# gaspardol/MonteCarloPredictiveCoding

Measured on AMD Instinct MI355X. Metric: Langevin inference steps/sec (whole node), MNIST MCPC 784-256-256-30, batch 6000, higher is better.
Workload: dtype f32

## Files before the change

### montecarlopredictivecoding_amd/csrc/mcpc_api.hip

```cpp
#include <hip/hip_runtime.h>
#include <dlfcn.h>
#include <rccl/rccl.h>

#include <algorithm>
#include <cmath>
#include <cstdio>
#include <cstring>
#include <string>
#include <vector>

#include "mcpc_build.h"
#include "mcpc_kernels.h"
#include "mcpc_moments.h"
#include "mcpc_plan.h"

using namespace mcpc;

#define HIP_TRY(expr)                                                                            \
    do {                                                                                         \
        hipError_t _e = (expr);                                                                  \
        if (_e != hipSuccess) return fail(MCPC_EHIP, "%s failed: %s (%s:%d)", #expr, hipGetErrorString(_e), __FILE__, __LINE__); \
    } while (0)

static inline int grid_for(size_t n, int block = 256) { return (int)std::min<size_t>((n + block - 1) / block, 4096); }

struct mcpc_engine : EnginePlan {
    mcpc_net_desc d{};
    ncclComm_t comm = nullptr;
    int comm_ranks = 0;
    float* x[kMaxLatent]{};
    float* m[kMaxLatent]{};
    float* v[kMaxLatent]{};
    float* e0sum = nullptr;
    float* mu1 = nullptr;
    float* ypad = nullptr;
    float* ytile = nullptr;
    uint32_t* ybits = nullptr;
    int* y_binary = nullptr;
    int ywords = 0;
    bool target_bound = false;
    const float* inputs = nullptr;
    hipStream_t aux = nullptr;
    hipEvent_t ev_steps[kMaxRingParts] = {}, ev_flush[kMaxRingParts] = {};
    hipStream_t spacer = nullptr;
    hipStream_t aux3 = nullptr;
    hipEvent_t ev_fork = nullptr, ev_join = nullptr;
    bool flush_pending[kMaxRingParts] = {};
    float* spill_a[kMaxLatent]{};
    float* spill_e[kMaxLatent]{};
    float* spill_eo = nullptr;
    float* slab = nullptr;
    size_t slab_floats = 0;
    double* epart = nullptr;
    size_t epart_rows = 0;
    float* adam_coef = nullptr;
    size_t adam_cap = 0;
    float* adam_host[2] = {nullptr, nullptr};
    size_t adam_host_cap[2] = {0, 0};
    hipEvent_t adam_ev[2] = {nullptr, nullptr};
    int adam_next = 0;
    struct Retired { void* p; hipEvent_t ev; };
    std::vector<Retired> retired;
    bool spill_ready = false;
    int* err = nullptr;
    int* wexp = nullptr;
    unsigned* spillmax = nullptr;
    float* lw_fx[kMaxLatent]{};
    float* lw_err[kMaxLatent]{};
    float* lw_err_o = nullptr;
    LwJob* lw_jobs = nullptr;
    unsigned long long* clk = nullptr;
    float* dummy = nullptr;
    int* rr_tab = nullptr;
    std::string last_step;
    std::string last_flush[kMaxLatent + 1];
    bool profiling = false;
    std::vector<std::pair<hipEvent_t, hipEvent_t>> events;
    size_t events_used = 0;
    double prof_steps = 0;
#ifdef MCPC_STAMPS
    unsigned long long* dbg = nullptr;
#endif
};

namespace {

struct Rccl {
    void* so = nullptr;
    decltype(&ncclGetUniqueId) GetUniqueId = nullptr;
    decltype(&ncclCommInitRank) CommInitRank = nullptr;
    decltype(&ncclAllReduce) AllReduce = nullptr;
    decltype(&ncclCommDestroy) CommDestroy = nullptr;
    decltype(&ncclGetErrorString) GetErrorString = nullptr;
};
Rccl g_rccl;

int rccl_load() {
    if (g_rccl.so) return MCPC_OK;
    void* so = dlopen("librccl.so.1", RTLD_NOW | RTLD_LOCAL);
    if (!so) so = dlopen("librccl.so", RTLD_NOW | RTLD_LOCAL);
    if (!so) return fail(MCPC_EHIP, "librccl.so.1 could not be loaded: %s", dlerror());
    Rccl r;
    r.GetUniqueId = (decltype(r.GetUniqueId))dlsym(so, "ncclGetUniqueId");
    r.CommInitRank = (decltype(r.CommInitRank))dlsym(so, "ncclCommInitRank");
    r.AllReduce = (decltype(r.AllReduce))dlsym(so, "ncclAllReduce");
    r.CommDestroy = (decltype(r.CommDestroy))dlsym(so, "ncclCommDestroy");
    r.GetErrorString = (decltype(r.GetErrorString))dlsym(so, "ncclGetErrorString");
    if (!r.GetUniqueId || !r.CommInitRank || !r.AllReduce || !r.CommDestroy || !r.GetErrorString) {
        dlclose(so);
        return fail(MCPC_EHIP, "librccl.so.1 lacks an entry point this library needs");
    }
    r.so = so;
    g_rccl = r;
    return MCPC_OK;
}

int free_all(mcpc_engine* e) {
    if (e->comm && g_rccl.CommDestroy) { (void)g_rccl.CommDestroy(e->comm); e->comm = nullptr; e->comm_ranks = 0; }
    auto F = [](auto*& p) { if (p) { (void)hipFree((void*)p); p = nullptr; } };
    for (int l = 0; l < kMaxLatent; ++l) { F(e->x[l]); F(e->m[l]); F(e->v[l]); F(e->spill_a[l]); F(e->spill_e[l]); }
    F(e->e0sum); F(e->mu1); F(e->ypad); F(e->ytile); F(e->ybits); F(e->y_binary); F(e->spill_eo); F(e->slab); F(e->epart); F(e->adam_coef); F(e->main.dev); F(e->err); F(e->wexp); F(e->spillmax); F(e->clk); F(e->dummy); F(e->u.plan.dev);
    for (int l = 0; l < kMaxLatent; ++l) { F(e->lw_fx[l]); F(e->lw_err[l]); }
    F(e->lw_err_o); F(e->lw_jobs);
    for (auto& ln : e->lin) { F(ln.Wf); F(ln.Wb); F(ln.bias_pad); F(ln.G); F(ln.Gb); }
    for (auto& ev : e->events) { (void)hipEventDestroy(ev.first); (void)hipEventDestroy(ev.second); }
    for (int h = 0; h < kMaxRingParts; ++h) { if (e->ev_steps[h]) (void)hipEventDestroy(e->ev_steps[h]); if (e->ev_flush[h]) (void)hipEventDestroy(e->ev_flush[h]); e->ev_steps[h] = e->ev_flush[h] = nullptr; }
    if (e->aux) { (void)hipStreamDestroy(e->aux); e->aux = nullptr; }
    if (e->aux3) { (void)hipStreamDestroy(e->aux3); e->aux3 = nullptr; }
    if (e->spacer) { (void)hipStreamDestroy(e->spacer); e->spacer = nullptr; }
    if (e->ev_fork) { (void)hipEventDestroy(e->ev_fork); e->ev_fork = nullptr; }
    if (e->ev_join) { (void)hipEventDestroy(e->ev_join); e->ev_join = nullptr; }
    F(e->rr_tab);
    for (auto& q : e->retired) { (void)hipFree(q.p); if (q.ev) (void)hipEventDestroy(q.ev); }
    e->retired.clear();
    for (int i = 0; i < 2; ++i) {
        if (e->adam_host[i]) { (void)hipHostFree(e->adam_host[i]); e->adam_host[i] = nullptr; }
        if (e->adam_ev[i]) { (void)hipEventDestroy(e->adam_ev[i]); e->adam_ev[i] = nullptr; }
    }
    e->events.clear();
    return 0;
}

template <typename T>
int dmalloc(T*& p, size_t count) {
    void* q = nullptr;
    hipError_t err = hipMalloc(&q, std::max<size_t>(count, 1) * sizeof(T));
    if (err != hipSuccess) return fail(MCPC_ENOMEM, "hipMalloc of %zu bytes failed: %s", count * sizeof(T), hipGetErrorString(err));
#ifdef MCPC_POISON_ALLOC
    if (hipMemset(q, 0xFF, std::max<size_t>(count, 1) * sizeof(T)) != hipSuccess) return fail(MCPC_EHIP, "hipMemset (poison) failed");
#endif
    p = (T*)q;
    return 0;
}

void retire(mcpc_engine* e, void* p, hipStream_t stream) {
    hipEvent_t ev = nullptr;
    if (hipEventCreateWithFlags(&ev, hipEventDisableTiming) != hipSuccess || hipEventRecord(ev, stream) != hipSuccess) {
        if (ev) (void)hipEventDestroy(ev);
        ev = nullptr;
    }
    e->retired.push_back({p, ev});
}
void free_completed_retired(mcpc_engine* e) {
    size_t keep = 0;
    for (size_t i = 0; i < e->retired.size(); ++i) {
        auto& q = e->retired[i];
        if (q.ev && hipEventQuery(q.ev) == hipSuccess) { (void)hipFree(q.p); (void)hipEventDestroy(q.ev); }
        else e->retired[keep++] = q;
    }
    e->retired.resize(keep);
    (void)hipGetLastError();
}
#ifdef MCPC_STAMPS
void print_u_table(const StepPlan& u) {
    static const char* tn[6] = {"FWD", "HEADF", "HEADB", "BWD", "ENERGY", "NOP"};
    for (int w = 0; w < kUWaves; ++w) {
        fprintf(stderr, "[u-table] wave %d:", w);
        for (int i = 0; i < u.n_phases; ++i) {
            const KPhase& k = u.table[(size_t)w * u.n_phases + i];
            fprintf(stderr, " %s%s(l%d t%d+%d kb%d)", (k.flags & PHF_SYNC) ? "|" : "", tn[k.type], k.layer, k.tile0, k.ntiles, (k.flags & PHF_WS_GEMM) ? k.nkb : 0);
        }
        fprintf(stderr, "\n");
    }
}
#endif

template <typename T>
int upload(T*& dev, const std::vector<T>& host, const char* what) {
    if (const int rc = dmalloc(dev, host.size())) return rc;
    if (hipMemcpy(dev, host.data(), host.size() * sizeof(T), hipMemcpyHostToDevice) != hipSuccess) return fail(MCPC_EHIP, "hipMemcpy of %s failed", what);
    return 0;
}

int upload_table(mcpc_engine* e, StepPlan& p) {
    for (KPhase& k : p.table)
        if (k.a_lin >= 1) k.A = (k.type == PH_FWD || k.type == PH_HEADF) ? e->lin[k.a_lin].Wf : e->lin[k.a_lin].Wb;
    return upload(p.dev, p.table, "the phase table");
}

hipError_t allow_lds(const void* fn, int bytes) { return hipFuncSetAttribute(fn, hipFuncAttributeMaxDynamicSharedMemorySize, bytes); }
int upload_rounds(mcpc_engine* e) {
    if (const int rc = upload(e->rr_tab, e->rr_host, "the round-schedule tables")) return rc;
    if (allow_lds((const void*)mcpc_steps_ws2_kernel<1, true>, e->main.lds_bytes) != hipSuccess) return fail(MCPC_EHIP, "hipFuncSetAttribute failed for the round schedule");
    return 0;
}

void set_window(const mcpc_engine* e, const mcpc_run_desc* r, KParams& P, int t0, int n) {
    P.t0 = t0; P.n_steps = n;
    const size_t s0 = (size_t)(t0 - r->t_begin);
    P.adam_coef = r->xopt_kind == MCPC_XOPT_ADAM ? e->adam_coef + 2 * s0 : nullptr;
    if (r->noise_mode == MCPC_NOISE_EXTERNAL)
        for (int l = 0; l < e->L; ++l) P.layer[l].ext_noise = r->ext_noise[l] + s0 * e->d.batch * e->d.sizes[l];
}

int launch_lw_steps(mcpc_engine* e, const mcpc_run_desc* r, const KParams& P, int t0, int n, hipStream_t stream) {
    LwParams Q{};
    Q.P = P;
    for (int l = 0; l < e->L; ++l) { Q.fx[l] = e->lw_fx[l]; Q.err[l] = e->lw_err[l]; }
    Q.err_o = e->lw_err_o;
    const dim3 gf(e->Bpad / kLwChains, e->lw_nf), gb(e->Bpad / kLwChains, e->lw_nb);
    for (int t = t0; t < t0 + n; ++t) {
        Q.t = t;
        Q.slot = (t >= P.acc_begin && t < P.acc_end) ? t - P.spill_t0 : -1;
        Q.rec_idx = -1;
        if (P.rec_count > 0 && t >= P.rec_begin) {
            const int k = (t - P.rec_begin) / P.rec_stride;
            if (k < P.rec_count && P.rec_begin + k * P.rec_stride == t) Q.rec_idx = k;
        }
        Q.do_energy = (P.energy_mode == MCPC_ENERGY_ALL || (P.energy_mode == MCPC_ENERGY_LAST && t == P.T - 1)) ? 1 : 0;
        Q.erow = P.energy_mode == MCPC_ENERGY_ALL ? t : 0;
        set_window(e, r, Q.P, t, 1);
        Q.jobs = e->lw_jobs;
        hipLaunchKernelGGL(mcpc_lw_fwd_kernel, gf, dim3(kLwThreads), 0, stream, Q);
        Q.jobs = e->lw_jobs + e->lw_nf;
        hipLaunchKernelGGL(mcpc_lw_bwd_kernel, gb, dim3(kLwThreads), 0, stream, Q);
    }
    HIP_TRY(hipGetLastError());
    return 0;
}

}

extern "C" {

int mcpc_abi_version(void) { return MCPC_ABI_VERSION; }

const char* mcpc_build_info(void) {
    static const bool exp = MCPC_TIMING_BUILD != 0 || std::strstr(MCPC_BUILD_FLAGS, "MCPC_EXP") != nullptr ||
                            std::strstr(MCPC_BUILD_FLAGS, "MCPC_HEB_EXP") != nullptr;
    static char buf[1024];
    static const int n = std::snprintf(buf, sizeof buf, "libmcpc abi=%d arch=gfx950 csrc=%s commit=%s exp=%d stamps=%d flags=[%s]",
                                       MCPC_ABI_VERSION, MCPC_BUILD_CSRC_SHA, MCPC_BUILD_COMMIT, exp ? 1 : 0, MCPC_STAMPS_BUILD, MCPC_BUILD_FLAGS);
    (void)n;
    return buf;
}
const char* mcpc_last_error(void) { return g_err.c_str(); }

int mcpc_create(const mcpc_net_desc* d, mcpc_engine** out) {
    if (!d || !out) return fail(MCPC_EINVAL, "null argument");
    *out = nullptr;
    if (const int rc = check_net_desc(d)) return rc;
    int ndev = 0;
    HIP_TRY(hipGetDeviceCount(&ndev));
    if (d->device < 0 || d->device >= ndev) return fail(MCPC_EINVAL, "device %d not present (%d devices)", d->device, ndev);
    HIP_TRY(hipSetDevice(d->device));
    int n_cu = 256;
    if (hipDeviceGetAttribute(&n_cu, hipDeviceAttributeMultiprocessorCount, d->device) != hipSuccess || n_cu <= 0) n_cu = 256;
    size_t free_b = 0, total_b = 0;
    if (d->spill_budget_bytes <= 0 && hipMemGetInfo(&free_b, &total_b) != hipSuccess) total_b = 0;

    mcpc_engine* e = new mcpc_engine();
    e->d = *d;
    e->d.tuning = nullptr;
    int rc = parse_tuning(d->tuning, e->knobs);
    if (!rc) rc = plan_engine(*d, n_cu, total_b, *e);
    if (rc) { delete e; return rc; }
    auto bail = [&](int code) { free_all(e); delete e; return code; };
    auto zeroed = [&](auto*& p, size_t count) -> int {
        if (const int rc2 = dmalloc(p, count)) return rc2;
        return hipMemset(p, 0, count * sizeof(*p)) == hipSuccess ? 0 : fail(MCPC_EHIP, "hipMemset failed");
    };
    for (int l = 0; l < e->L; ++l) {
        const size_t n = (size_t)e->Bpad * e->npad[l];
        if ((rc = zeroed(e->x[l], n)) || (rc = dmalloc(e->m[l], n)) || (rc = dmalloc(e->v[l], n))) return bail(rc);
    }
    if ((rc = zeroed(e->e0sum, (size_t)e->Bpad * e->npad[0])) || (rc = dmalloc(e->mu1, (size_t)e->Bpad * e->npad[0]))) return bail(rc);
    if (e->has_head) {
        if ((rc = zeroed(e->ypad, (size_t)e->Bpad * e->out_pad)) || (rc = dmalloc(e->ytile, (size_t)e->Bpad * e->out_pad))) return bail(rc);
        e->ywords = (e->out_pad + 31) / 32;
        if ((rc = dmalloc(e->ybits, (size_t)e->Bpad * e->ywords)) || (rc = zeroed(e->y_binary, 3))) return bail(rc);
    }
    const int nlin = e->L + (e->has_head ? 1 : 0);
    for (int j = 0; j < nlin; ++j) {
        Lin& ln = e->lin[j];
        if ((rc = zeroed(ln.G, (size_t)ln.out_pad * ln.g_ld)) || (rc = zeroed(ln.Gb, (size_t)ln.out_pad))) return bail(rc);
        if (j >= 1) {
            const size_t pkf = (size_t)(ln.out_pad / 16) * kblocks(ln.in_pad) * kFragBlock * 4;
            const size_t pkb = (size_t)(ln.in_pad / 16) * kblocks(ln.out_pad) * kFragBlock * 4;
            if ((rc = dmalloc(ln.Wf, pkf)) || (rc = dmalloc(ln.Wb, pkb)) || (rc = dmalloc(ln.bias_pad, (size_t)ln.out_pad))) return bail(rc);
        }
    }
    if (e->lw) {
        for (int l = 0; l < e->L; ++l) {
            const size_t n = (size_t)e->Bpad * e->npad[l];
            if ((rc = dmalloc(e->lw_fx[l], n))) return bail(rc);
            if (l >= 1 && (rc = dmalloc(e->lw_err[l], n))) return bail(rc);
        }
        if (e->has_head && (rc = dmalloc(e->lw_err_o, (size_t)e->Bpad * e->out_pad))) return bail(rc);
        if ((rc = upload(e->lw_jobs, e->lw_table, "the layer-wise job table"))) return bail(rc);
    } else if ((rc = upload_table(e, e->main))) return bail(rc);
    if (e->u.on && (rc = upload_table(e, e->u.plan))) return bail(rc);
#ifdef MCPC_STAMPS
    if (e->u.on) print_u_table(e->u.plan);
#endif
    if ((rc = zeroed(e->err, 1)) || (rc = zeroed(e->spillmax, (size_t)kMaxRingParts * kSpillTensors)) || (rc = zeroed(e->wexp, kMaxLatent + 1)) ||
        (rc = zeroed(e->clk, 2)) || (rc = zeroed(e->dummy, 1024)))
        return bail(rc);
    const void* kfn = e->ws == 2 ? (const void*)mcpc_steps_ws2_kernel<1> : (const void*)mcpc_steps_kernel<1, 4>;
    const hipError_t herr = e->lw ? hipSuccess : allow_lds(kfn, e->main.lds_bytes);
    if (herr != hipSuccess) return bail(fail(MCPC_EHIP, "hipFuncSetAttribute(%d bytes LDS) failed: %s", e->main.lds_bytes, hipGetErrorString(herr)));
    if (e->rr && (rc = upload_rounds(e))) return bail(rc);
    if (e->u.on && (allow_lds((const void*)mcpc_steps_u_kernel<false>, e->u.plan.lds_bytes) != hipSuccess ||
                    allow_lds((const void*)mcpc_steps_u_kernel<true>, e->u.plan.lds_bytes) != hipSuccess))
        return bail(fail(MCPC_EHIP, "hipFuncSetAttribute failed for the unified-wave kernel (%d bytes LDS)", e->u.plan.lds_bytes));
    *out = e;
    return MCPC_OK;
}

int mcpc_destroy(mcpc_engine* e) {
    if (!e) return MCPC_OK;
    (void)hipSetDevice(e->d.device);
    (void)hipDeviceSynchronize();
    free_all(e);
    delete e;
    return MCPC_OK;
}

int mcpc_bind_params(mcpc_engine* e, int j, const float* W, const float* bias) {
    if (!e) return fail(MCPC_EINVAL, "null engine");
    const int nlin = e->L + (e->has_head ? 1 : 0);
    if (j < 0 || j >= nlin) return fail(MCPC_EINVAL, "Linear index %d out of range 0..%d", j, nlin - 1);
    if (!W) return fail(MCPC_EINVAL, "null weight pointer for Linear %d", j);
    e->lin[j].W = W;
    e->lin[j].bias = bias;
    e->lin[j].bound = true;
    return MCPC_OK;
}

int mcpc_params_changed(mcpc_engine* e, void* stream_) {
    if (!e) return fail(MCPC_EINVAL, "null engine");
    hipStream_t stream = (hipStream_t)stream_;
    HIP_TRY(hipSetDevice(e->d.device));
    const int nlin = e->L + (e->has_head ? 1 : 0);
    for (int j = 0; j < nlin; ++j)
        if (!e->lin[j].bound) return fail(MCPC_ESTATE, "Linear %d has no bound parameters", j);
    for (int j = 1; j < nlin; ++j) {
        Lin& ln = e->lin[j];
        const size_t total = (size_t)ln.out_pad * ln.in_pad;
        const int grid = std::max(grid_for(total), (ln.out_pad + 255) / 256);
        hipLaunchKernelGGL(mcpc_wexp_kernel, dim3(1), dim3(1024), 0, stream, ln.W, (size_t)ln.n_out * ln.n_in, e->wexp + j);
        hipLaunchKernelGGL(mcpc_pack_kernel, dim3(grid), dim3(256), 0, stream, ln.W, ln.bias, ln.Wf, ln.Wb, ln.bias_pad,
                           ln.n_out, ln.n_in, ln.out_pad / 16, ln.in_pad / 16, (const int*)(e->wexp + j));
    }
    HIP_TRY(hipGetLastError());
    return MCPC_OK;
}

int mcpc_bind_inputs(mcpc_engine* e, const float* inputs, void* ) {
    if (!e) return fail(MCPC_EINVAL, "null engine");
    e->inputs = inputs;
    return MCPC_OK;
}

int mcpc_bind_target(mcpc_engine* e, const float* target, void* stream_) {
    if (!e) return fail(MCPC_EINVAL, "null engine");
    if (!e->has_head) return fail(MCPC_EINVAL, "network has no read-out: no target to bind");
    if (!target) return fail(MCPC_EINVAL, "null target");
    HIP_TRY(hipSetDevice(e->d.device));
    const size_t total = (size_t)e->Bpad * e->out_pad;
    hipLaunchKernelGGL(mcpc_pad_kernel, dim3(grid_for(total)), dim3(256), 0, (hipStream_t)stream_, target, e->ypad,
                       e->d.batch, e->d.n_out, e->Bpad, e->out_pad);
    hipLaunchKernelGGL(mcpc_tile_major_kernel, dim3(grid_for(total / 4)), dim3(256), 0, (hipStream_t)stream_, e->ypad, e->ytile, e->Bpad, e->out_pad);
    HIP_TRY(hipMemsetAsync(e->y_binary, 0xff, sizeof(int), (hipStream_t)stream_));
    HIP_TRY(hipMemsetAsync(e->y_binary + 2, 0xff, sizeof(int), (hipStream_t)stream_));
    hipLaunchKernelGGL(mcpc_pack_target_bits_kernel, dim3(grid_for((size_t)e->Bpad * e->ywords)), dim3(256), 0, (hipStream_t)stream_,
                       e->ypad, e->ybits, e->y_binary, e->Bpad, e->out_pad, e->ywords);
    HIP_TRY(hipGetLastError());
    e->target_bound = true;
    return MCPC_OK;
}

int mcpc_load_state(mcpc_engine* e, const float* const* x, void* stream_) {
    if (!e || !x) return fail(MCPC_EINVAL, "null argument");
    HIP_TRY(hipSetDevice(e->d.device));
    for (int l = 0; l < e->L; ++l) {
        if (!x[l]) return fail(MCPC_EINVAL, "null state pointer for layer %d", l);
        const size_t total = (size_t)e->Bpad * e->npad[l];
        hipLaunchKernelGGL(mcpc_pad_kernel, dim3(grid_for(total)), dim3(256), 0, (hipStream_t)stream_, x[l], e->x[l],
                           e->d.batch, e->d.sizes[l], e->Bpad, e->npad[l]);
    }
    HIP_TRY(hipGetLastError());
    return MCPC_OK;
}

int mcpc_store_state(mcpc_engine* e, float* const* x, void* stream_) {
    if (!e || !x) return fail(MCPC_EINVAL, "null argument");
    HIP_TRY(hipSetDevice(e->d.device));
    for (int l = 0; l < e->L; ++l) {
        if (!x[l]) return fail(MCPC_EINVAL, "null state pointer for layer %d", l);
        const size_t total = (size_t)e->d.batch * e->d.sizes[l];
        hipLaunchKernelGGL(mcpc_unpad_kernel, dim3(grid_for(total)), dim3(256), 0, (hipStream_t)stream_, e->x[l], x[l],
                           e->d.batch, e->d.sizes[l], e->npad[l]);
    }
    HIP_TRY(hipGetLastError());
    return MCPC_OK;
}

int mcpc_store_adam_state(mcpc_engine* e, float* const* m, float* const* v, void* stream_) {
    if (!e || !m || !v) return fail(MCPC_EINVAL, "null argument");
    HIP_TRY(hipSetDevice(e->d.device));
    for (int l = 0; l < e->L; ++l) {
        if (!m[l] || !v[l]) return fail(MCPC_EINVAL, "null Adam state pointer for layer %d", l);
        const size_t total = (size_t)e->d.batch * e->d.sizes[l];
        hipLaunchKernelGGL(mcpc_unpad_adam_kernel, dim3(grid_for(total)), dim3(256), 0, (hipStream_t)stream_, e->m[l], m[l],
                           e->d.batch, e->d.sizes[l], e->npad[l]);
        hipLaunchKernelGGL(mcpc_unpad_adam_kernel, dim3(grid_for(total)), dim3(256), 0, (hipStream_t)stream_, e->v[l], v[l],
                           e->d.batch, e->d.sizes[l], e->npad[l]);
    }
    HIP_TRY(hipGetLastError());
    return MCPC_OK;
}

}

namespace {

struct HebPlan {
    bool tiled = false, swapped = false;
    int ra = 0;
    int te[2] = {0, 0}, n_mt[2] = {0, 0};
    int n_nt = 1;
    int wave_tiles = 0;
    int ksplit = 1, rps = 0;
    int ksplit_cap = 1;
};

HebPlan plan_hebbian(const mcpc_engine* e, int ne, int na, int rows) {
    HebPlan h;
    const int et = ne / 16, at = na / 16;
    const bool wide = heb_wide(et, at);
    const bool narrow_in = heb_narrow_in(et, at);
    h.tiled = wide || narrow_in;
    h.swapped = narrow_in;
    if (wide) {
        h.ra = at >= 16 ? 2 : 1;
        h.n_nt = at / (8 * h.ra);
        if (et <= 8) { h.te[0] = 8; h.n_mt[0] = 1; }
        else if (et <= 16) { h.te[0] = 16; h.n_mt[0] = 1; }
        else {
            const int b17 = et % 16, a16 = (et - 17 * b17) / 16;
            if (et - 17 * b17 >= 0) { h.te[0] = 17; h.n_mt[0] = b17; h.te[1] = 16; h.n_mt[1] = a16; }
            else { h.te[0] = 17; h.n_mt[0] = (et + 16) / 17; }
            if (h.n_mt[0] == 0) { h.te[0] = h.te[1]; h.n_mt[0] = h.n_mt[1]; h.te[1] = 0; h.n_mt[1] = 0; }
        }
    } else if (narrow_in) {
        h.ra = 2; h.n_nt = 1; h.te[0] = at; h.n_mt[0] = 1;
    }
    if (h.tiled) {
        int want = e->knobs.dw_ksplit > 0 ? e->knobs.dw_ksplit : std::max(1, rows / (48 * kHebKB));
        if (e->knobs.dw_ksplit <= 0) {
            const int cols = std::max(1, (h.n_mt[0] + h.n_mt[1]) * h.n_nt);
            want = std::max(want, std::min(rows / (8 * kHebKB), (256 + cols - 1) / cols));
        }
        want = std::min(want, std::max(1, rows / kHebKB));
        h.ksplit_cap = want;
        h.rps = ((rows + want - 1) / want + kHebKB - 1) / kHebKB * kHebKB;
        h.ksplit = (rows + h.rps - 1) / h.rps;
    } else {
        h.wave_tiles = ((ne + 63) / 64) * ((na + 63) / 64);
        int ksplit = std::max(1, std::min(4096 / h.wave_tiles, rows / 64));
        h.ksplit_cap = ksplit;
        h.rps = ((rows + ksplit - 1) / ksplit + 15) / 16 * 16;
        h.ksplit = (rows + h.rps - 1) / h.rps;
    }
    return h;
}

template <int TE, int RA, bool SW = false>
int launch_heb(const HebArgs& a, hipStream_t stream) {
    constexpr int lds_bytes = 2 * kHebKB * (heb_lds_stride(16 * TE) + heb_lds_stride(16 * 8 * RA)) * (int)sizeof(float);
    static bool attr_set[16] = {false};
    int dev = 0;
    (void)hipGetDevice(&dev);
    if (dev >= 0 && dev < 16 && !attr_set[dev]) {
        if (hipFuncSetAttribute((const void*)mcpc_heb_kernel<TE, RA, SW>, hipFuncAttributeMaxDynamicSharedMemorySize, lds_bytes) != hipSuccess)
            return fail(MCPC_EHIP, "hipFuncSetAttribute failed for the Hebbian kernel");
        attr_set[dev] = true;
    }
    hipLaunchKernelGGL((mcpc_heb_kernel<TE, RA, SW>), dim3(a.n_mt * a.n_nt * a.ksplit), dim3(kHebThreads), lds_bytes, stream, a);
    return 0;
}

template <int TE, int RA, bool SW = false>
int launch_heb7(const HebArgs& a, hipStream_t stream) {
    constexpr int lds_bytes = 2 * 2 * 16 * TE * kHeb7LD * 2 + 16 * TE * (int)sizeof(float) + 8 * 2 * 272 * (int)sizeof(float);
    static bool attr_set[16] = {false};
    int dev = 0;
    (void)hipGetDevice(&dev);
    if (dev >= 0 && dev < 16 && !attr_set[dev]) {
        if (hipFuncSetAttribute((const void*)mcpc_heb7_kernel<TE, RA, SW>, hipFuncAttributeMaxDynamicSharedMemorySize, lds_bytes) != hipSuccess)
            return fail(MCPC_EHIP, "hipFuncSetAttribute failed for the Hebbian kernel");
        attr_set[dev] = true;
    }
    hipLaunchKernelGGL((mcpc_heb7_kernel<TE, RA, SW>), dim3(a.n_mt * a.n_nt * a.ksplit), dim3(kHebThreads), lds_bytes, stream, a);
    return 0;
}

int ensure_spill(mcpc_engine* e, hipStream_t stream) {
    if (e->spill_ready) return 0;
    int rc;
    if (e->half_slots < e->slots && !e->aux) {
        int lo = 0, hi = 0;
        (void)hipDeviceGetStreamPriorityRange(&lo, &hi);
        if (!e->spacer) (void)hipStreamCreateWithFlags(&e->spacer, hipStreamNonBlocking);
        if (hipStreamCreateWithPriority(&e->aux, hipStreamNonBlocking, lo) != hipSuccess) return fail(MCPC_EHIP, "hipStreamCreateWithPriority failed");
        if (e->knobs.flush_streams >= 2 &&
            (hipStreamCreateWithPriority(&e->aux3, hipStreamNonBlocking, lo) != hipSuccess ||
             hipEventCreateWithFlags(&e->ev_fork, hipEventDisableTiming) != hipSuccess ||
             hipEventCreateWithFlags(&e->ev_join, hipEventDisableTiming) != hipSuccess))
            return fail(MCPC_EHIP, "second flush stream could not be created");
        for (int h = 0; h < kMaxRingParts; ++h)
            if (hipEventCreateWithFlags(&e->ev_steps[h], hipEventDisableTiming) != hipSuccess ||
                hipEventCreateWithFlags(&e->ev_flush[h], hipEventDisableTiming) != hipSuccess)
                return fail(MCPC_EHIP, "hipEventCreate failed");
    }
    for (int l = 0; l < e->L; ++l) {
        const size_t n = (size_t)e->slots * e->Bpad * e->npad[l];
        if (!e->spill_a[l] && (rc = dmalloc(e->spill_a[l], n))) return rc;
        if (l >= 1 && !e->spill_e[l] && (rc = dmalloc(e->spill_e[l], n))) return rc;
    }
    if (e->has_head && !e->spill_eo && (rc = dmalloc(e->spill_eo, (size_t)e->slots * e->Bpad * e->out_pad))) return rc;
    if (e->nwg_live * e->ct < e->Bpad && e->ws == 2) {
        const size_t live = (size_t)e->nwg_live * 16, dead = (size_t)e->Bpad - live;
        auto zero_tail = [&](float* base, int npad) {
            return hipMemset2DAsync(base + live * npad, (size_t)e->Bpad * npad * sizeof(float), 0, dead * npad * sizeof(float), (size_t)e->slots, stream) == hipSuccess;
        };
        bool ok = true;
        for (int l = 0; l < e->L; ++l) { ok = ok && zero_tail(e->spill_a[l], e->npad[l]); if (l >= 1) ok = ok && zero_tail(e->spill_e[l], e->npad[l]); }
        if (e->has_head) ok = ok && zero_tail(e->spill_eo, e->out_pad);
        if (!ok) return fail(MCPC_EHIP, "hipMemset2D of the spill ring's padding rows failed");
    }
    const int nlin = e->L + (e->has_head ? 1 : 0);
    const int max_rows = e->half_slots * e->Bpad;
    size_t total = 0;
    for (int j = 1; j < nlin; ++j) {
        Lin& ln = e->lin[j];
        const HebPlan h = plan_hebbian(e, ln.out_pad, ln.in_pad, max_rows);
        ln.slab_off = total;
        ln.slab_floats = (size_t)h.ksplit_cap * ((size_t)ln.out_pad * ln.in_pad + ln.out_pad);
        total += ln.slab_floats;
    }
    if (!e->slab && (rc = dmalloc(e->slab, total))) return rc;
    e->slab_floats = total;
    e->spill_ready = true;
    return 0;
}

static inline int spill_id_a_host(int l) { return l; }
int flush_spill(mcpc_engine* e, int n_slots, int slot0, hipStream_t stream, int part) {
    const unsigned* const smax = e->spillmax + (size_t)part * kSpillTensors;
    const int rows = n_slots * e->Bpad;
    const int nlin = e->L + (e->has_head ? 1 : 0);
    ReduceJobs jobs{};
    unsigned max_blocks = 1;
    hipStream_t const main_stream = stream;
    const bool two = e->aux3 != nullptr && stream == e->aux;
    double load[2] = {0.0, 0.0};
    if (two) { HIP_TRY(hipEventRecord(e->ev_fork, main_stream)); HIP_TRY(hipStreamWaitEvent(e->aux3, e->ev_fork, 0)); }
    auto next_stream = [&](double cost) {
        const int k = (two && load[1] < load[0]) ? 1 : 0;
        load[k] += cost;
        return k ? e->aux3 : main_stream;
    };
    for (int j = 1; j < nlin; ++j) {
        Lin& ln = e->lin[j];
        const int ne = ln.out_pad, na = ln.in_pad;
        const float* E = (j < e->L ? e->spill_e[j] : e->spill_eo) + (size_t)slot0 * e->Bpad * ne;
        const float* A = e->spill_a[j - 1] + (size_t)slot0 * e->Bpad * na;
        const HebPlan h = plan_hebbian(e, ne, na, rows);
        std::string plan;
        auto name_launch = [&](const char* kern, int te, int ra, bool sw, int n_mt, int n_nt) {
            char buf[64];
            snprintf(buf, sizeof buf, "%s%s<%d,%d%s>x%d", plan.empty() ? "" : "+", kern, te, ra, sw ? ",T" : "", n_mt);
            plan += buf;
            if (n_nt > 1) plan += "*" + std::to_string(n_nt);
        };
        const char* const heb_name = e->knobs.heb_fp32 ? "heb" : "heb7";
        const int e_id = j < e->L ? kMaxLatent + j : kSpillIdEo;
        float* slab = e->slab + ln.slab_off;
        float* slab_b = slab + (size_t)h.ksplit * ne * na;
        if ((size_t)h.ksplit * ((size_t)ne * na + ne) > ln.slab_floats)
            return fail(MCPC_ESTATE, "internal: Hebbian slabs of Linear %d (%d splits) exceed their allocation", j, h.ksplit);
        if (h.swapped) {
            stream = next_stream((double)ne * na);
            HebArgs a{A, E, slab, slab_b, rows, na, ne, h.rps, 1, 1, h.ksplit, 0, smax + spill_id_a_host(j - 1), smax + e_id};
            name_launch(heb_name, h.te[0], 2, true, 1, 1);
            int rc = 0;
            if (!e->knobs.heb_fp32) {
                if (h.te[0] == 1) rc = launch_heb7<1, 2, true>(a, stream);
                else if (h.te[0] == 2) rc = launch_heb7<2, 2, true>(a, stream);
                else rc = launch_heb7<4, 2, true>(a, stream);
            } else
            if (h.te[0] == 1) rc = launch_heb<1, 2, true>(a, stream);
            else if (h.te[0] == 2) rc = launch_heb<2, 2, true>(a, stream);
            else rc = launch_heb<4, 2, true>(a, stream);
            if (rc) return rc;
        } else if (h.tiled) {
            int col = 0;
            for (int part = 0; part < 2; ++part) {
                if (h.n_mt[part] == 0) continue;
                HebArgs a{E, A, slab, slab_b, rows, ne, na, h.rps, h.n_mt[part], h.n_nt, h.ksplit, col, smax + e_id, smax + spill_id_a_host(j - 1)};
                stream = next_stream((double)h.n_mt[part] * h.te[part] * 16 * na);
                int rc = 0;
                const int te = h.te[part];
                const bool resplit = te == 17 && h.ra == 2 && !e->knobs.heb_fp32 && e->knobs.heb171;
                if (!resplit) name_launch(heb_name, te, h.ra, false, h.n_mt[part], h.n_nt);
                if (!e->knobs.heb_fp32) {
                    if (te == 17 && h.ra == 2 && !e->knobs.heb171) rc = launch_heb7<17, 2>(a, stream);
                    else if (te == 17 && h.ra == 2) {
                        HebArgs a1 = a;
                        a1.n_nt = 2 * a.n_nt;
                        name_launch(heb_name, 17, 1, false, a1.n_mt, a1.n_nt);
                        rc = launch_heb7<17, 1>(a1, stream);
                    }
                    else if (te == 16 && h.ra == 2) rc = launch_heb7<16, 2>(a, stream);
                    else if (te == 8 && h.ra == 2) rc = launch_heb7<8, 2>(a, stream);
                    else if (te == 17) rc = launch_heb7<17, 1>(a, stream);
                    else if (te == 16) rc = launch_heb7<16, 1>(a, stream);
                    else rc = launch_heb7<8, 1>(a, stream);
                } else
                if (te == 17 && h.ra == 2) rc = launch_heb<17, 2>(a, stream);
                else if (te == 16 && h.ra == 2) rc = launch_heb<16, 2>(a, stream);
                else if (te == 8 && h.ra == 2) rc = launch_heb<8, 2>(a, stream);
                else if (te == 17) rc = launch_heb<17, 1>(a, stream);
                else if (te == 16) rc = launch_heb<16, 1>(a, stream);
                else rc = launch_heb<8, 1>(a, stream);
                if (rc) return rc;
                col += h.n_mt[part] * te * 16;
            }
        } else {
            stream = next_stream((double)ne * na);
            hipLaunchKernelGGL(mcpc_dw_kernel, dim3((h.wave_tiles + 3) / 4, h.ksplit), dim3(256), 0, stream, E, A, slab, slab_b,
                               rows, ne, na, h.rps);
            plan = "dw tiles=" + std::to_string(h.wave_tiles);
        }
        e->last_flush[j] = plan + " ksplit=" + std::to_string(h.ksplit) + " rps=" + std::to_string(h.rps) + (ln.spill_tm ? " tm" : " rm");
        const float sign = j < e->L ? -1.0f : 1.0f;
        jobs.job[jobs.n_jobs++] = ReduceJob{slab, ln.G, ne * na, h.ksplit, sign, h.swapped ? ne : 0, h.swapped ? na : 0};
        jobs.job[jobs.n_jobs++] = ReduceJob{slab_b, ln.Gb, ne, h.ksplit, sign, 0, 0};
        max_blocks = std::max(max_blocks, (unsigned)std::min<size_t>(((size_t)ne * na + 255) / 256, 2048));
    }
    stream = main_stream;
    if (two) { HIP_TRY(hipEventRecord(e->ev_join, e->aux3)); HIP_TRY(hipStreamWaitEvent(main_stream, e->ev_join, 0)); }
    if (jobs.n_jobs > 0)
        hipLaunchKernelGGL(mcpc_reduce_jobs_kernel, dim3(max_blocks, jobs.n_jobs), dim3(256), 0, stream, jobs);
    HIP_TRY(hipGetLastError());
    return 0;
}

}

namespace {

int check_run(const mcpc_engine* e, const mcpc_run_desc* r) {
    const int nlin = e->L + (e->has_head ? 1 : 0);
    for (int j = 0; j < nlin; ++j)
        if (!e->lin[j].bound) return fail(MCPC_ESTATE, "Linear %d has no bound parameters (mcpc_bind_params + mcpc_params_changed first)", j);
    if (r->T < 1 || r->t_begin < 0 || r->n_steps < 1 || r->t_begin + r->n_steps > r->T)
        return fail(MCPC_EINVAL, "bad step range: T=%d t_begin=%d n_steps=%d", r->T, r->t_begin, r->n_steps);
    if (r->loss_kind < 0 || r->loss_kind > 2) return fail(MCPC_EINVAL, "loss_kind=%d", r->loss_kind);
    if (r->loss_kind != MCPC_LOSS_NONE) {
        if (!e->has_head) return fail(MCPC_EINVAL, "a loss needs a read-out Linear (n_out > 0)");
        if (!e->target_bound) return fail(MCPC_ESTATE, "loss requested but no target bound");
        if (r->loss_kind == MCPC_LOSS_GAUSSIAN && !(r->loss_var > 0.0)) return fail(MCPC_EINVAL, "loss_var must be positive");
        if (r->mask_start < 0 || r->mask_start >= e->d.n_out) return fail(MCPC_EINVAL, "mask_start=%d outside 0..%d", r->mask_start, e->d.n_out - 1);
    }
    if (r->xopt_kind != MCPC_XOPT_SGD && r->xopt_kind != MCPC_XOPT_ADAM) return fail(MCPC_EINVAL, "xopt_kind=%d", r->xopt_kind);
    if (!(r->lr > 0.0)) return fail(MCPC_EINVAL, "lr must be positive");
    if (r->noise_mode < 0 || r->noise_mode > 2) return fail(MCPC_EINVAL, "noise_mode=%d", r->noise_mode);
    if (r->noise_mode != MCPC_NOISE_NONE && r->xopt_kind != MCPC_XOPT_SGD)
        return fail(MCPC_EINVAL, "the fused Langevin kick is defined for SGD on x only (reference utils/model.py:35-44 steps the same optimizer)");
    if (r->noise_mode != MCPC_NOISE_NONE && !(r->noise_var >= 0.0)) return fail(MCPC_EINVAL, "noise_var must be >= 0");
    if (r->noise_mode == MCPC_NOISE_EXTERNAL)
        for (int l = 0; l < e->L; ++l)
            if (!r->ext_noise[l]) return fail(MCPC_EINVAL, "ext_noise[%d] is null", l);
    if (!r->update_x)
        for (int l = 0; l < e->L; ++l)
            if (!r->xgrad[l]) return fail(MCPC_EINVAL, "update_x=0 needs xgrad[%d]", l);
    if (r->energy_mode < 0 || r->energy_mode > 2) return fail(MCPC_EINVAL, "energy_mode=%d", r->energy_mode);
    if (r->energy_mode != MCPC_ENERGY_NONE && !r->energies_out) return fail(MCPC_EINVAL, "energies_out is null");
    if (r->rec_count < 0 || (r->rec_count > 0 && r->rec_stride < 1)) return fail(MCPC_EINVAL, "bad record schedule");
    return 0;
}

size_t energy_slots(const mcpc_engine* e) { return e->lw ? (size_t)e->nwg_live : e->ws == 2 ? (size_t)e->Bpad / 16 : (size_t)e->nwg; }

int prepare_run(mcpc_engine* e, const mcpc_run_desc* r, bool run_accumulates, hipStream_t stream) {
    if (r->xopt_kind == MCPC_XOPT_ADAM) {
        const size_t need = (size_t)r->n_steps * 2;
        if (need > e->adam_cap) {
            if (e->adam_coef) retire(e, e->adam_coef, stream);
            e->adam_coef = nullptr;
            size_t cap = 1024;
            while (cap < need) cap *= 2;
            int rc = dmalloc(e->adam_coef, cap);
            if (rc) return rc;
            e->adam_cap = cap;
        }
        const int hb = e->adam_next; e->adam_next ^= 1;
        if (!e->adam_ev[hb]) HIP_TRY(hipEventCreateWithFlags(&e->adam_ev[hb], hipEventDisableTiming));
        else HIP_TRY(hipEventSynchronize(e->adam_ev[hb]));
        if (need > e->adam_host_cap[hb]) {
            if (e->adam_host[hb]) HIP_TRY(hipHostFree(e->adam_host[hb]));
            e->adam_host[hb] = nullptr;
            void* q = nullptr;
            HIP_TRY(hipHostMalloc(&q, e->adam_cap * sizeof(float), hipHostMallocDefault));
            e->adam_host[hb] = (float*)q; e->adam_host_cap[hb] = e->adam_cap;
        }
        float* tab = e->adam_host[hb];
        for (int s = 0; s < r->n_steps; ++s) {
            const double step = (double)(r->adam_step0 + s + 1);
            const double bc1 = 1.0 - std::pow(r->beta1, step);
            const double bc2 = 1.0 - std::pow(r->beta2, step);
            tab[2 * s] = (float)(-(r->lr / bc1));
            tab[2 * s + 1] = (float)std::sqrt(bc2);
        }
        HIP_TRY(hipMemcpyAsync(e->adam_coef, tab, need * sizeof(float), hipMemcpyHostToDevice, stream));
        HIP_TRY(hipEventRecord(e->adam_ev[hb], stream));
        if (r->adam_step0 == 0)
            for (int l = 0; l < e->L; ++l) {
                HIP_TRY(hipMemsetAsync(e->m[l], 0, (size_t)e->Bpad * e->npad[l] * 4, stream));
                HIP_TRY(hipMemsetAsync(e->v[l], 0, (size_t)e->Bpad * e->npad[l] * 4, stream));
            }
    }
    const size_t erows = r->energy_mode == MCPC_ENERGY_ALL ? (size_t)r->T : 1, eslots = energy_slots(e);
    if (r->energy_mode != MCPC_ENERGY_NONE && erows > e->epart_rows) {
        if (e->epart) retire(e, e->epart, stream);
        e->epart = nullptr;
        const size_t cap = std::max(erows, e->epart_rows + e->epart_rows / 2);
        int rc = dmalloc(e->epart, cap * eslots * (kMaxLatent + 1));
        if (rc) return rc;
        HIP_TRY(hipMemsetAsync(e->epart, 0, cap * eslots * (kMaxLatent + 1) * sizeof(double), stream));
        e->epart_rows = cap;
    }
    {
        const Lin& l0 = e->lin[0];
        const size_t total = (size_t)e->Bpad * e->npad[0];
        hipLaunchKernelGGL(mcpc_mu1_kernel, dim3(grid_for(total)), dim3(256), 0, stream, e->inputs, l0.W, l0.bias, e->mu1,
                           e->d.batch, e->d.n_in, e->d.sizes[0], e->Bpad, e->npad[0]);
    }
    if (e->lw)
        for (int l = 0; l < e->L; ++l) {
            const size_t total4 = (size_t)e->Bpad * e->npad[l] / 4;
            hipLaunchKernelGGL(mcpc_lw_act_kernel, dim3(grid_for(total4)), dim3(256), 0, stream, (const float*)e->x[l], e->lw_fx[l], total4, e->d.acts[l]);
        }
    if (run_accumulates) { const int rc = ensure_spill(e, stream); if (rc) return rc; }
    if (r->acc_reset && run_accumulates) {
        const int nlin = e->L + (e->has_head ? 1 : 0);
        for (int j = 0; j < nlin; ++j) {
            HIP_TRY(hipMemsetAsync(e->lin[j].G, 0, (size_t)e->lin[j].out_pad * e->lin[j].g_ld * 4, stream));
            HIP_TRY(hipMemsetAsync(e->lin[j].Gb, 0, (size_t)e->lin[j].out_pad * 4, stream));
        }
        HIP_TRY(hipMemsetAsync(e->e0sum, 0, (size_t)e->Bpad * e->npad[0] * 4, stream));
    }
    return 0;
}

bool lean_ok(const mcpc_engine* e) {
    int widest = e->out_pad;
    for (int l = 0; l < e->L; ++l) widest = std::max(widest, e->npad[l]);
    return e->Bpad < (1 << 24) && (uint64_t)e->Bpad * (uint64_t)widest * 4u < (1ull << 32) && !e->knobs.no_lean;
}

bool use_unified(const mcpc_engine* e, const mcpc_run_desc* r) {
    return e->u.on && (e->u.prefer || (e->has_head && r->loss_kind == MCPC_LOSS_NONE)) && e->ws == 2 && r->update_x && lean_ok(e) &&
           ((r->xopt_kind == MCPC_XOPT_SGD && r->noise_mode != MCPC_NOISE_EXTERNAL) ||
            (r->xopt_kind == MCPC_XOPT_ADAM && r->noise_mode == MCPC_NOISE_NONE));
}

KParams run_params(const mcpc_engine* e, const mcpc_run_desc* r, const StepPlan& sp) {
    KParams P{};
    const int nlin = e->L + (e->has_head ? 1 : 0);
    for (int l = 0; l < e->L; ++l) {
        KLayer& K = P.layer[l];
        K.x = e->x[l]; K.m = e->m[l]; K.v = e->v[l];
        K.xgrad = r->update_x ? nullptr : r->xgrad[l];
        K.rec = r->rec_count > 0 ? r->rec_x[l] : nullptr;
        K.spill_e = l == 0 ? e->e0sum : e->spill_e[l];
        K.spill_a = e->spill_a[l];
        K.spill_e_tm = (l >= 1 && e->lin[l].spill_tm) ? 1 : 0;
        K.spill_a_tm = (l + 1 < nlin && e->lin[l + 1].spill_tm) ? 1 : 0;
        K.ext_noise = nullptr;
        if (l >= 1) {
            K.Wf = (const f32x4*)e->lin[l].Wf; K.Wb = (const f32x4*)e->lin[l].Wb; K.bias = e->lin[l].bias_pad;
        }
        K.n = e->d.sizes[l]; K.npad = e->npad[l]; K.ntiles = e->npad[l] / 16;
        K.act = e->d.acts[l]; K.ecoef = e->d.ecoef[l];
        K.lds_a = sp.lds_a[l]; K.lds_e = sp.lds_e[l]; K.ld = e->npad[l] + kLdPad;
        K.lds_x = sp.lds_x[l]; K.lds_bias = sp.lds_bias[l];
    }
    if (e->has_head) {
        KHead& H = P.head;
        const Lin& ln = e->lin[e->L];
        H.Wf = (const f32x4*)ln.Wf; H.Wb = (const f32x4*)ln.Wb; H.bias = ln.bias_pad;
        H.ybits = e->ybits; H.y_binary = e->knobs.no_ybits ? e->y_binary + 1 : e->y_binary; H.y_bounded = e->y_binary + 2; H.ywords = e->ywords;
        H.y = e->ypad; H.ytile = e->ytile; H.rec_out = r->rec_count > 0 ? r->rec_out : nullptr; H.spill_e = e->spill_eo;
        H.spill_tm = e->lin[e->L].spill_tm ? 1 : 0;
        H.n = e->d.n_out; H.npad = e->out_pad; H.ntiles = e->out_pad / 16;
        H.loss_kind = r->loss_kind;
        H.inv_var = r->loss_kind == MCPC_LOSS_GAUSSIAN ? (float)(1.0 / r->loss_var) : 1.0f;
        H.mask_start = r->loss_kind == MCPC_LOSS_NONE ? 0 : r->mask_start;
        H.lds_eo = sp.lds_eo; H.ld = sp.head_ld;
        H.lds_bias = sp.lds_hbias; H.lds_yw = sp.lds_yw;
    }
    P.mu1 = e->mu1; P.epart = e->epart; P.epart_slots = (int)energy_slots(e);
    P.phases = sp.dev; P.n_phases = sp.n_phases; P.wexp = e->wexp; P.spillmax = nullptr; P.lds_spillmax = sp.lds_spillmax; P.lds_rowexp = sp.lds_rowexp; P.g_first = sp.g_first;
    P.stagger_cycles = e->knobs.stagger;
    P.L = e->L; P.has_head = e->has_head; P.B = e->d.batch; P.Bpad = e->Bpad; P.T = r->T;
    P.xopt = r->xopt_kind; P.update_x = r->update_x ? 1 : 0;
    P.lr = (float)r->lr; P.beta2 = (float)r->beta2;
    P.omb1 = (float)(1.0 - r->beta1); P.omb2 = (float)(1.0 - r->beta2); P.eps = (float)r->eps;
    P.noise_mode = r->update_x ? r->noise_mode : MCPC_NOISE_NONE;
    P.noise_scale = (float)std::sqrt(r->noise_var * r->lr);
    P.seed = r->seed; P.step_base = r->step_base; P.chain_base = r->chain_base;
    P.acc_begin = std::max(r->acc_begin, 0); P.acc_end = std::min(r->acc_end, r->T);
    P.energy_mode = r->energy_mode;
    P.rec_begin = r->rec_begin; P.rec_stride = std::max(r->rec_stride, 1); P.rec_count = r->rec_count;
    P.lds_red = sp.lds_red;
    P.lds_ws_sync = sp.lds_ws_sync;
    P.ws_prio = e->knobs.ws_prio;
    P.lean_ok = lean_ok(e);
    P.err = e->err; P.dummy = e->dummy; P.lds_floats = sp.lds_bytes / 4; P.lds_zero = sp.lds_zero;
    P.clk = e->profiling ? e->clk : nullptr;
    P.xl = sp.xl ? 1 : 0;
    P.spill_sys = e->slot_bytes > ((size_t)8 << 20) ? 1 : 0;
    return P;
}

#ifdef MCPC_STAMPS
int report_stamps(mcpc_engine* e, bool use_u, int t, int n, hipStream_t stream) {
    static const char* names_ws2[16] = {"G top", "G wait deps", "G HEADB gemm", "G gemm", "G prefetch next", "G store+publish",
                                        "(launch, s_memtime)", "(launch, 100 MHz)", "E other", "E loads", "E wait block", "E epilogue FWD", "E epilogue HEADF", "E epilogue BWD", "-", "-"};
    static const char* names[16] = {"FWD prologue", "FWD gemm", "FWD epilogue", "HEADF prologue", "HEADF gemm", "HEADF epilogue",
                                    "HEADB prologue", "HEADB gemm", "HEADB (acc->b)", "BWD prologue", "BWD gemm", "BWD epilogue",
                                    "energy", "barrier", "-", "-"};
    HIP_TRY(hipStreamSynchronize(stream));
    std::vector<unsigned long long> h((size_t)e->nwg * e->nw * 16);
    HIP_TRY(hipMemcpy(h.data(), e->dbg, h.size() * 8, hipMemcpyDeviceToHost));
#ifdef MCPC_STAMPS_ENTRY
    static const char* what[5] = {"", "G wait (deps)", "G total", "E wait for block", "E total"};
    static const char* tname[5] = {"FWD", "HEADF", "HEADB", "BWD", "ENERGY"};
    const std::vector<KPhase>& tab = e->main.table;
    const bool want_g = MCPC_STAMPS_ENTRY <= 2;
    fprintf(stderr, "[stamps] launch t0=%d n=%d: %s per table entry, cycles per step (mean / max over the %s waves)\n", t, n,
            what[MCPC_STAMPS_ENTRY], want_g ? "G" : "E");
    double tot = 0;
    for (int i = 0; i < 16 && i < e->main.n_phases; ++i) {
        double sum = 0, mx = 0; size_t cnt = 0;
        for (size_t w = 0; w < (size_t)e->nwg * e->nw; ++w) {
            const bool is_g = (int)(w % e->nw) < e->nw / 2;
            if (is_g != want_g) continue;
            const double v = (double)h[w * 16 + i];
            sum += v; mx = std::max(mx, v); ++cnt;
        }
        tot += sum / cnt / n;
        fprintf(stderr, "[stamps]   entry %2d %-6s layer %d tiles %2d nkb %2d  mean %8.0f  max %8.0f\n", i, tname[tab[i].type], tab[i].layer,
                tab[i].ntiles, tab[i].nkb, sum / cnt / n, mx / n);
    }
    fprintf(stderr, "[stamps]   sum over entries: %.0f cycles per step\n", tot);
#else
    double tot = 0, sum[16] = {0}, mx[16] = {0};
    for (size_t w = 0; w < (size_t)e->nwg * e->nw; ++w)
        for (int i = 0; i < 16; ++i) { sum[i] += (double)h[w * 16 + i]; mx[i] = std::max(mx[i], (double)h[w * 16 + i]); }
    static const char* names_u[16] = {"top of entry", "barrier", "gemm", "prefetch next", "epilogue", "-", "-", "presplit", "gemm fwd nt=1", "gemm fwd nt=2", "gemm fwd nt=3", "gemm fwd nt=4", "gemm bwd nt=1", "gemm bwd nt=2", "gemm bwd nt=3", "gemm bwd nt=4"};
    if (e->ws == 2 && !use_u) {
        fprintf(stderr, "[stamps] shader clock during the launch = %.3f GHz (s_memtime ticks per 100 MHz wall-clock tick)\n", sum[6] / sum[7] * 0.1);
        sum[6] = sum[7] = 0;
    }
    for (int i = 0; i < 16; ++i) tot += sum[i];
    fprintf(stderr, "[stamps] launch t0=%d n=%d: mean cycles/step/wave = %.0f\n", t, n, tot / (e->nwg * e->nw) / n);
    for (int i = 0; i < 16; ++i)
        fprintf(stderr, "[stamps]   %-18s %5.1f%%  mean %8.0f  max %8.0f cycles/step\n", (use_u ? names_u : e->ws == 2 ? names_ws2 : names)[i], 100.0 * sum[i] / tot,
                sum[i] / (e->nwg * e->nw) / n, mx[i] / n);
#endif
    return 0;
}
#endif

}

extern "C" {

int mcpc_run(mcpc_engine* e, const mcpc_run_desc* r, void* stream_) {
    if (!e || !r) return fail(MCPC_EINVAL, "null argument");
    hipStream_t stream = (hipStream_t)stream_;
    HIP_TRY(hipSetDevice(e->d.device));
    if (const int rc = check_run(e, r)) return rc;
    const int acc_b = std::max(r->acc_begin, 0), acc_e = std::min(r->acc_end, r->T);
    if (!e->retired.empty()) free_completed_retired(e);
    const bool run_accumulates = acc_b < acc_e && r->t_begin < acc_e && r->t_begin + r->n_steps > acc_b;
    if (const int rc = prepare_run(e, r, run_accumulates, stream)) return rc;
    const size_t eslots = energy_slots(e);
    const bool use_u = use_unified(e, r);
    const StepPlan& sp = use_u ? e->u.plan : e->main;
    KParams P = run_params(e, r, sp);
#ifdef MCPC_STAMPS
    if (!e->dbg) { int rc = dmalloc(e->dbg, (size_t)e->nwg * 2 * kMaxWaves * 16); if (rc) return rc; }
    P.dbg = e->dbg;
#endif

    int t = r->t_begin;
    const int end = r->t_begin + r->n_steps;
    const bool overlap = e->aux != nullptr;
    int half = 0;
    const int n_parts = std::max(1, e->slots / std::max(1, e->half_slots));
    constexpr size_t kMaxProfBrackets = 1 << 16;
    bool bracket_open = false;
    auto prof_begin = [&]() -> int {
        bracket_open = false;
        if (!e->profiling) return 0;
        if (e->events_used >= kMaxProfBrackets) return 0;
        bracket_open = true;
        if (e->events_used == e->events.size()) {
            hipEvent_t a, b;
            if (hipEventCreate(&a) != hipSuccess || hipEventCreate(&b) != hipSuccess) return fail(MCPC_EHIP, "hipEventCreate failed");
            e->events.emplace_back(a, b);
        }
        return hipEventRecord(e->events[e->events_used].first, stream) == hipSuccess ? 0 : fail(MCPC_EHIP, "hipEventRecord failed");
    };
    auto prof_end = [&](double steps) -> int {
        if (!e->profiling || !bracket_open) return 0;
        if (hipEventRecord(e->events[e->events_used].second, stream) != hipSuccess) return fail(MCPC_EHIP, "hipEventRecord failed");
        ++e->events_used; e->prof_steps += steps;
        return 0;
    };
    bool rr_ok = e->rr && r->update_x;
#ifdef MCPC_STAMPS
    rr_ok = false;
#endif
    unsigned launched = 0;
    auto run_round_cycle = [&](const KParams& base, int t0, int q) -> int {
        launched |= 2u;
        KParams Q = base;
        set_window(e, r, Q, t0, q);
        Q.spill_t0 = t0; Q.rr_q = q;
        for (int i = 0; i < e->rr_k; ++i) {
            Q.wg_list = e->rr_tab + e->rr_off[i]; Q.wg_rel = Q.wg_list + e->rr_count[i];
            { const int rc = prof_begin(); if (rc) return rc; }
            if (use_u) hipLaunchKernelGGL((mcpc_steps_u_kernel<true>), dim3(e->rr_count[i]), dim3(kUThreads), sp.lds_bytes, stream, Q);
            else hipLaunchKernelGGL((mcpc_steps_ws2_kernel<1, true>), dim3(e->rr_count[i]), dim3(kWs2Threads), sp.lds_bytes, stream, Q);
            { const int rc = prof_end((double)q * e->rr_count[i] / e->nwg_live); if (rc) return rc; }
        }
        HIP_TRY(hipGetLastError());
        return 0;
    };
    while (t < end) {
        const bool in_acc = t >= acc_b && t < acc_e;
        int n;
        if (in_acc) {
            const int rem = std::min(end, acc_e) - t;
            n = std::min(rem, e->half_slots);
            const int tail = e->knobs.flush_tail;
            if (overlap && tail > 0 && rem <= e->half_slots && rem >= 2 * tail && std::min(end, acc_e) == acc_e) n = rem - tail;
        }
        else n = (t < acc_b ? std::min(end, acc_b) : end) - t;
        n = std::min(n, ((1 << 24) - 2) / std::max(std::max(e->main.n_phases, e->u.plan.n_phases), 1));
        int rr_q = 0;
        if (rr_ok && in_acc) {
            rr_q = n / e->rr_m;
            if (rr_q >= 1) n = rr_q * e->rr_m;
        } else if (rr_ok) {
            while (n >= e->rr_m) {
                const int q = std::min(std::max(1, e->knobs.rr_qmax), n / e->rr_m);
                const int rc = run_round_cycle(P, t, q);
                if (rc) return rc;
                t += q * e->rr_m; n -= q * e->rr_m;
            }
            if (n == 0) continue;
        }
        const int slot0 = in_acc && overlap ? half * e->half_slots : 0;
        set_window(e, r, P, t, n);
        P.spill_t0 = t;
        if (in_acc) {
            for (int l = 0; l < e->L; ++l) {
                const size_t off = (size_t)slot0 * e->Bpad * e->npad[l];
                P.layer[l].spill_a = e->spill_a[l] + off;
                if (l >= 1) P.layer[l].spill_e = e->spill_e[l] + off;
            }
            if (e->has_head) P.head.spill_e = e->spill_eo + (size_t)slot0 * e->Bpad * e->out_pad;
            if (overlap && e->flush_pending[half]) { HIP_TRY(hipStreamWaitEvent(stream, e->ev_flush[half], 0)); e->flush_pending[half] = false; }
            P.spillmax = e->spillmax + (size_t)(overlap ? half : 0) * kSpillTensors;
            HIP_TRY(hipMemsetAsync(P.spillmax, 0, kSpillTensors * sizeof(unsigned), stream));
        } else {
            P.spillmax = nullptr;
        }
        if (rr_q >= 1) {
            const int rc = run_round_cycle(P, t, rr_q);
            if (rc) return rc;
        } else {
            { const int rc = prof_begin(); if (rc) return rc; }
            launched |= 1u;
            if (e->lw) { const int rc = launch_lw_steps(e, r, P, t, n, stream); if (rc) return rc; }
            else if (use_u) hipLaunchKernelGGL((mcpc_steps_u_kernel<false>), dim3(e->nwg_live), dim3(kUThreads), sp.lds_bytes, stream, P);
            else if (e->ws == 2) hipLaunchKernelGGL((mcpc_steps_ws2_kernel<1>), dim3(e->nwg_live), dim3(kWs2Threads), sp.lds_bytes, stream, P);
            else hipLaunchKernelGGL((mcpc_steps_kernel<1, 4>), dim3(e->nwg), dim3(256), sp.lds_bytes, stream, P);
            { const int rc = prof_end((double)n); if (rc) return rc; }
        }
        HIP_TRY(hipGetLastError());
#ifdef MCPC_STAMPS
        if (const int rc = report_stamps(e, use_u, t, n, stream)) return rc;
#endif
        if (in_acc) {
            if (overlap) {
                HIP_TRY(hipEventRecord(e->ev_steps[half], stream));
                HIP_TRY(hipStreamWaitEvent(e->aux, e->ev_steps[half], 0));
                int rc = flush_spill(e, n, slot0, e->aux, half);
                if (rc) return rc;
                HIP_TRY(hipEventRecord(e->ev_flush[half], e->aux));
                e->flush_pending[half] = true;
                half = (half + 1) % n_parts;
            } else {
                int rc = flush_spill(e, n, 0, stream, 0);
                if (rc) return rc;
            }
        }
        t += n;
    }
    {
        std::string name;
        if (launched & 2u) name = use_u ? e->u_rr_name : e->rr_name;
        if (launched & 1u) {
            if (!name.empty()) name += " + ";
            name += plain_kernel_name(*e, use_u);
        }
        e->last_step = name;
    }
    for (int h = 0; h < kMaxRingParts; ++h)
        if (overlap && e->flush_pending[h]) { HIP_TRY(hipStreamWaitEvent(stream, e->ev_flush[h], 0)); e->flush_pending[h] = false; }
    if (run_accumulates) {
        Lin& l0 = e->lin[0];
        hipLaunchKernelGGL(mcpc_dw0_kernel, dim3(l0.n_out, e->inputs != nullptr ? l0.n_in + 1 : 1), dim3(256), 0, stream, e->e0sum,
                           e->inputs, l0.G, l0.Gb, e->d.batch, l0.n_out, e->npad[0], l0.n_in, l0.g_ld);
        HIP_TRY(hipMemsetAsync(e->e0sum, 0, (size_t)e->Bpad * e->npad[0] * 4, stream));
    }
    if (r->energy_mode == MCPC_ENERGY_ALL) {
        hipLaunchKernelGGL(mcpc_energy_reduce_kernel, dim3((r->n_steps + 3) / 4), dim3(256), 0, stream,
                           e->epart + (size_t)r->t_begin * eslots * (kMaxLatent + 1),
                           r->energies_out + (size_t)r->t_begin * kEnergyCols, r->n_steps, (int)eslots, e->L);
    } else if (r->energy_mode == MCPC_ENERGY_LAST && end == r->T) {
        hipLaunchKernelGGL(mcpc_energy_reduce_kernel, dim3(1), dim3(256), 0, stream, e->epart, r->energies_out, 1, (int)eslots, e->L);
    }
    HIP_TRY(hipGetLastError());
    return MCPC_OK;
}

int mcpc_read_param_grads(mcpc_engine* e, int j, float* dW, float* db, float scale, int accumulate, void* stream_) {
    if (!e) return fail(MCPC_EINVAL, "null engine");
    const int nlin = e->L + (e->has_head ? 1 : 0);
    if (j < 0 || j >= nlin) return fail(MCPC_EINVAL, "Linear index %d out of range", j);
    if (!dW) return fail(MCPC_EINVAL, "null dW");
    HIP_TRY(hipSetDevice(e->d.device));
    const Lin& ln = e->lin[j];
    hipStream_t stream = (hipStream_t)stream_;
    hipLaunchKernelGGL(mcpc_export_grad_kernel, dim3(grid_for((size_t)ln.n_out * ln.n_in)), dim3(256), 0, stream, ln.G, dW,
                       ln.n_out, ln.n_in, ln.g_ld, scale, accumulate);
    if (db)
        hipLaunchKernelGGL(mcpc_export_grad_kernel, dim3(grid_for((size_t)ln.n_out)), dim3(256), 0, stream, ln.Gb, db,
                           ln.n_out, 1, 1, scale, accumulate);
    HIP_TRY(hipGetLastError());
    return MCPC_OK;
}

int mcpc_comm_unique_id(void* id_out) {
    static_assert(sizeof(ncclUniqueId) == MCPC_COMM_ID_BYTES, "ncclUniqueId is 128 bytes");
    if (!id_out) return fail(MCPC_EINVAL, "null id buffer");
    if (const int rc = rccl_load()) return rc;
    ncclUniqueId id;
    const ncclResult_t r = g_rccl.GetUniqueId(&id);
    if (r != ncclSuccess) return fail(MCPC_EHIP, "ncclGetUniqueId: %s", g_rccl.GetErrorString(r));
    std::memcpy(id_out, &id, sizeof(id));
    return MCPC_OK;
}

int mcpc_comm_init(mcpc_engine* e, int n_ranks, int rank, const void* id_in) {
    if (!e || !id_in) return fail(MCPC_EINVAL, "null argument");
    if (n_ranks < 1 || rank < 0 || rank >= n_ranks) return fail(MCPC_EINVAL, "rank %d of %d", rank, n_ranks);
    if (e->comm) return fail(MCPC_ESTATE, "the engine already has a communicator (mcpc_comm_destroy first)");
    if (const int rc = rccl_load()) return rc;
    HIP_TRY(hipSetDevice(e->d.device));
    ncclUniqueId id;
    std::memcpy(&id, id_in, sizeof(id));
    const ncclResult_t r = g_rccl.CommInitRank(&e->comm, n_ranks, id, rank);
    if (r != ncclSuccess) { e->comm = nullptr; return fail(MCPC_EHIP, "ncclCommInitRank(%d of %d): %s", rank, n_ranks, g_rccl.GetErrorString(r)); }
    e->comm_ranks = n_ranks;
    return MCPC_OK;
}

int mcpc_allreduce_grads(mcpc_engine* e, float* flat, int64_t n_floats, void* stream_) {
    if (!e || !flat) return fail(MCPC_EINVAL, "null argument");
    if (!e->comm) return fail(MCPC_ESTATE, "mcpc_allreduce_grads before mcpc_comm_init");
    if (n_floats != mcpc_param_count(e)) return fail(MCPC_EINVAL, "bucket of %lld floats, the engine's parameters have %lld", (long long)n_floats, (long long)mcpc_param_count(e));
    HIP_TRY(hipSetDevice(e->d.device));
    const ncclResult_t r = g_rccl.AllReduce(flat, flat, (size_t)n_floats, ncclFloat, ncclSum, e->comm, (hipStream_t)stream_);
    if (r != ncclSuccess) return fail(MCPC_EHIP, "ncclAllReduce: %s", g_rccl.GetErrorString(r));
    return MCPC_OK;
}

int mcpc_comm_destroy(mcpc_engine* e) {
    if (!e) return fail(MCPC_EINVAL, "null engine");
    if (e->comm) {
        (void)hipSetDevice(e->d.device);
        const ncclResult_t r = g_rccl.CommDestroy(e->comm);
        e->comm = nullptr; e->comm_ranks = 0;
        if (r != ncclSuccess) return fail(MCPC_EHIP, "ncclCommDestroy: %s", g_rccl.GetErrorString(r));
    }
    return MCPC_OK;
}

int64_t mcpc_param_count(const mcpc_engine* e) {
    if (!e) return 0;
    const int nlin = e->L + (e->has_head ? 1 : 0);
    int64_t n = 0;
    for (int j = 0; j < nlin; ++j) n += (int64_t)e->lin[j].n_out * e->lin[j].n_in + (e->lin[j].bias ? e->lin[j].n_out : 0);
    return n;
}

int mcpc_read_param_grads_flat(mcpc_engine* e, float* flat, int64_t n_floats, float scale, void* stream_) {
    if (!e || !flat) return fail(MCPC_EINVAL, "null argument");
    if (n_floats != mcpc_param_count(e)) return fail(MCPC_EINVAL, "flat buffer holds %lld floats, parameters need %lld", (long long)n_floats, (long long)mcpc_param_count(e));
    const int nlin = e->L + (e->has_head ? 1 : 0);
    int64_t off = 0;
    for (int j = 0; j < nlin; ++j) {
        const Lin& ln = e->lin[j];
        float* dW = flat + off; off += (int64_t)ln.n_out * ln.n_in;
        float* db = nullptr;
        if (ln.bias) { db = flat + off; off += ln.n_out; }
        int rc = mcpc_read_param_grads(e, j, dW, db, scale, 0, stream_);
        if (rc) return rc;
    }
    return MCPC_OK;
}

int mcpc_philox_normals(int device, uint64_t seed, uint64_t step, int layer, uint64_t chain_base, int batch, int n_units,
                        float* out, int raw, void* stream_) {
    if (!out || batch < 1 || n_units < 1 || layer < 0 || layer > 255) return fail(MCPC_EINVAL, "bad argument");
    HIP_TRY(hipSetDevice(device));
    const size_t total = (size_t)batch * ((n_units + 3) / 4);
    hipLaunchKernelGGL(mcpc_philox_kernel, dim3(grid_for(total)), dim3(256), 0, (hipStream_t)stream_, seed, step, layer, chain_base,
                       batch, n_units, out, raw);
    HIP_TRY(hipGetLastError());
    return MCPC_OK;
}

int mcpc_moments_accumulate(int device, const float* rec, int64_t row_elems, int32_t first, int32_t stride, int32_t n, int32_t transform,
                            double* sum, double* sumsq, int accumulate, void* stream_) {
    if (!sum) return fail(MCPC_EINVAL, "moments: sum is null");
    if (row_elems < 1) return fail(MCPC_EINVAL, "moments: row_elems=%lld, must be at least 1", (long long)row_elems);
    if (stride < 1) return fail(MCPC_EINVAL, "moments: stride=%d, must be at least 1", stride);
    if (first < 0) return fail(MCPC_EINVAL, "moments: first=%d, must not be negative", first);
    if (n < 0) return fail(MCPC_EINVAL, "moments: n=%d, must not be negative", n);
    if (transform != MCPC_MOM_IDENTITY && transform != MCPC_MOM_SIGMOID) return fail(MCPC_EINVAL, "moments: unknown transform %d", transform);
    if (n > 0 && !rec) return fail(MCPC_EINVAL, "moments: rec is null with n=%d", n);
    if (n == 0 && accumulate) return MCPC_OK;
    HIP_TRY(hipSetDevice(device));
    const float* r0 = n > 0 ? rec + (int64_t)first * row_elems : rec;
    const int64_t row_step = (int64_t)stride * row_elems;
    const uintptr_t align = (uintptr_t)r0 | (uintptr_t)sum | (uintptr_t)sumsq;
    if (row_elems % 4 == 0 && align % 16 == 0)
        mom_dispatch<4>(transform, r0, row_elems, row_step, n, sum, sumsq, accumulate, (hipStream_t)stream_);
    else
        mom_dispatch<1>(transform, r0, row_elems, row_step, n, sum, sumsq, accumulate, (hipStream_t)stream_);
    HIP_TRY(hipGetLastError());
    return MCPC_OK;
}

int mcpc_query(const mcpc_engine* e, int32_t* lds_bytes, int32_t* chains_per_wg, int32_t* n_workgroups, int32_t* spill_slots) {
    if (!e) return fail(MCPC_EINVAL, "null engine");
    if (lds_bytes) *lds_bytes = e->main.lds_bytes;
    if (chains_per_wg) *chains_per_wg = e->lw ? kLwChains : e->ct;
    if (n_workgroups) *n_workgroups = e->nwg_live;
    if (spill_slots) *spill_slots = e->slots;
    return MCPC_OK;
}

const char* mcpc_step_kernel_name(const mcpc_engine* e) { return e ? step_kernel_name(*e) : ""; }

const char* mcpc_last_step_kernel_name(const mcpc_engine* e) {
    return e ? e->last_step.c_str() : "";
}

const char* mcpc_last_flush_plan(const mcpc_engine* e, int j) {
    if (!e || j < 0 || j >= e->L + (e->has_head ? 1 : 0)) return "";
    return e->last_flush[j].c_str();
}

int mcpc_sync_check(mcpc_engine* e, void* stream_) {
    if (!e) return fail(MCPC_EINVAL, "null engine");
    HIP_TRY(hipSetDevice(e->d.device));
    HIP_TRY(hipStreamSynchronize((hipStream_t)stream_));
    int flag = 0;
    HIP_TRY(hipMemcpy(&flag, e->err, sizeof(int), hipMemcpyDeviceToHost));
    if (flag != 0) {
        (void)hipMemset(e->err, 0, sizeof(int));
        return fail(MCPC_ESTATE, "the step kernel reported error word 0x%x (a workgroup-internal progress wait ran out): results of the last run are invalid", flag);
    }
    return MCPC_OK;
}

int mcpc_last_shader_clock_ghz(mcpc_engine* e, float* ghz) {
    if (!e || !ghz) return fail(MCPC_EINVAL, "null argument");
    HIP_TRY(hipSetDevice(e->d.device));
    unsigned long long h[2] = {0, 0};
    HIP_TRY(hipMemcpy(h, e->clk, sizeof h, hipMemcpyDeviceToHost));
    *ghz = h[1] ? (float)((double)h[0] / (double)h[1] * 0.1) : 0.f;
    return MCPC_OK;
}

}
namespace {
__global__ __launch_bounds__(256) void mcpc_poison_lds_kernel(uint32_t word, int* seen) {
    extern __shared__ uint32_t poison_lds[];
    for (int i = threadIdx.x; i < 160 * 1024 / 4; i += 256) poison_lds[i] = word;
    __syncthreads();
    if (threadIdx.x == 0) {
        uint32_t hw, xcc;
        asm volatile("s_getreg_b32 %0, hwreg(HW_REG_HW_ID)" : "=s"(hw));
        asm volatile("s_getreg_b32 %0, hwreg(HW_REG_XCC_ID)" : "=s"(xcc));
        const int cu = (int)((hw >> 8) & 0xff);
        atomicAdd(&seen[(xcc & 7) * 256 + cu], 1);
        const unsigned long long t_end = wall_clock64() + 2000;
        while (wall_clock64() < t_end) __builtin_amdgcn_s_sleep(32);
    }
    __syncthreads();
    if (poison_lds[(threadIdx.x * 97) % (160 * 1024 / 4)] != word) atomicAdd(&seen[8 * 256], 1);
}
}
extern "C" {

int mcpc_debug_poison_lds(int device, uint32_t word, void* stream_) {
    HIP_TRY(hipSetDevice(device));
    int n_cu = 256;
    if (hipDeviceGetAttribute(&n_cu, hipDeviceAttributeMultiprocessorCount, device) != hipSuccess || n_cu <= 0) n_cu = 256;
    static bool attr_set[16] = {false};
    if (device >= 0 && device < 16 && !attr_set[device]) {
        HIP_TRY(hipFuncSetAttribute((const void*)mcpc_poison_lds_kernel, hipFuncAttributeMaxDynamicSharedMemorySize, 160 * 1024));
        attr_set[device] = true;
    }
    int* seen = nullptr;
    HIP_TRY(hipMalloc((void**)&seen, (8 * 256 + 1) * sizeof(int)));
    hipStream_t stream = (hipStream_t)stream_;
    int rc = MCPC_OK;
    for (int pass = 0; pass < 2 && rc == MCPC_OK; ++pass) {
        if (hipMemsetAsync(seen, 0, (8 * 256 + 1) * sizeof(int), stream) != hipSuccess) { rc = fail(MCPC_EHIP, "hipMemsetAsync failed"); break; }
        hipLaunchKernelGGL(mcpc_poison_lds_kernel, dim3(4 * n_cu), dim3(256), 160 * 1024, stream, word, seen);
        if (hipGetLastError() != hipSuccess || hipStreamSynchronize(stream) != hipSuccess) rc = fail(MCPC_EHIP, "the LDS poison kernel failed");
    }
    if (rc == MCPC_OK) {
        std::vector<int> h(8 * 256 + 1);
        if (hipMemcpy(h.data(), seen, h.size() * sizeof(int), hipMemcpyDeviceToHost) != hipSuccess) rc = fail(MCPC_EHIP, "hipMemcpy failed");
        else {
            int visited = 0;
            for (int i = 0; i < 8 * 256; ++i) visited += h[i] > 0;
            if (visited < n_cu) rc = fail(MCPC_ESTATE, "LDS poison reached %d of %d compute units", visited, n_cu);
            else if (h[8 * 256] != 0) rc = fail(MCPC_ESTATE, "LDS poison read-back mismatch");
        }
    }
    (void)hipFree(seen);
    return rc;
}

int mcpc_debug_lw_jobs(int32_t n_latent, const int32_t* sizes, int32_t n_out, int32_t* fwd, int32_t* bwd, int32_t cap,
                       int32_t* n_fwd, int32_t* n_bwd, int32_t* tile) {
    if (n_latent < 1 || n_latent > kMaxLatent || !sizes || n_out < 0) return fail(MCPC_EINVAL, "bad network");
    int npad[kMaxLatent];
    for (int l = 0; l < n_latent; ++l) { if (sizes[l] < 1) return fail(MCPC_EINVAL, "sizes[%d]=%d", l, sizes[l]); npad[l] = pad16(sizes[l]); }
    std::vector<LwJob> f, b;
    lw_job_table(n_latent, npad, pad16(n_out), f, b);
    for (int i = 0; i < (int)f.size() && i < cap && fwd; ++i) { fwd[2 * i] = f[i].layer; fwd[2 * i + 1] = f[i].ut0; }
    for (int i = 0; i < (int)b.size() && i < cap && bwd; ++i) { bwd[2 * i] = b[i].layer; bwd[2 * i + 1] = b[i].ut0; }
    if (n_fwd) *n_fwd = (int32_t)f.size();
    if (n_bwd) *n_bwd = (int32_t)b.size();
    if (tile) { tile[0] = kLwChains; tile[1] = kLwUnitTiles; }
    return MCPC_OK;
}

int mcpc_debug_plan(const mcpc_net_desc* d, int32_t n_cu, int64_t total_mem, char* out, int64_t cap, int64_t* needed) {
    if (!d || n_cu < 1 || total_mem < 0 || cap < 0 || (cap > 0 && !out)) return fail(MCPC_EINVAL, "bad argument");
    if (const int rc = check_net_desc(d)) return rc;
    EnginePlan plan;
    if (const int rc = parse_tuning(d->tuning, plan.knobs)) return rc;
    if (const int rc = plan_engine(*d, n_cu, (size_t)total_mem, plan)) return rc;
    const std::string s = plan_json(plan);
    if (needed) *needed = (int64_t)s.size() + 1;
    if (cap > 0) { const size_t n = std::min<size_t>(s.size(), (size_t)cap - 1); std::memcpy(out, s.data(), n); out[n] = 0; }
    return MCPC_OK;
}

int mcpc_set_profiling(mcpc_engine* e, int enable) {
    if (!e) return fail(MCPC_EINVAL, "null engine");
    HIP_TRY(hipSetDevice(e->d.device));
    e->profiling = enable != 0;
    e->events_used = 0;
    e->prof_steps = 0;
    if (enable) HIP_TRY(hipMemset(e->clk, 0, 2 * sizeof(unsigned long long)));
    return MCPC_OK;
}

namespace {
int sum_events(const std::vector<std::pair<hipEvent_t, hipEvent_t>>& ev, size_t used, float* total) {
    *total = 0.f;
    for (size_t i = 0; i < used; ++i) {
        HIP_TRY(hipEventSynchronize(ev[i].second));
        float t = 0.f;
        HIP_TRY(hipEventElapsedTime(&t, ev[i].first, ev[i].second));
        *total += t;
    }
    return 0;
}
}

int mcpc_last_step_kernel_ms(mcpc_engine* e, float* ms, int32_t* n_launches, int64_t* n_steps) {
    if (!e || !ms) return fail(MCPC_EINVAL, "null argument");
    HIP_TRY(hipSetDevice(e->d.device));
    const int rc = sum_events(e->events, e->events_used, ms);
    if (rc) return rc;
    if (n_launches) *n_launches = (int32_t)e->events_used;
    if (n_steps) *n_steps = (int64_t)std::llround(e->prof_steps);
    return MCPC_OK;
}

}
```

### montecarlopredictivecoding_amd/csrc/mcpc_plan.h

```cpp
#pragma once

#include <algorithm>
#include <cstdarg>
#include <cstdio>
#include <cstdlib>
#include <string>
#include <vector>

#include "mcpc_kernels.h"

namespace mcpc {

inline thread_local std::string g_err;

inline int fail(int code, const char* fmt, ...) {
    char buf[1024];
    va_list ap;
    va_start(ap, fmt);
    vsnprintf(buf, sizeof buf, fmt, ap);
    va_end(ap);
    g_err = buf;
    return code;
}

inline int pad16(int n) { return (n + 15) / 16 * 16; }
inline int kblocks(int k_pad) { return (k_pad + kKB - 1) / kKB; }
inline bool heb_wide(int et, int at) { return et >= 8 && at % 8 == 0 && (at <= 16 || at % 16 == 0); }
inline bool heb_narrow_in(int et, int at) { return !heb_wide(et, at) && et == 16 && (at == 1 || at == 2 || at == 4); }
constexpr int kLdsLimit = 160 * 1024;

struct Lin {
    const float* W = nullptr;
    const float* bias = nullptr;
    bool bound = false;
    int n_out = 0, n_in = 0, out_pad = 0, in_pad = 0;
    float* Wf = nullptr;
    float* Wb = nullptr;
    float* bias_pad = nullptr;
    float* G = nullptr;
    float* Gb = nullptr;
    int g_ld = 0;
    bool spill_tm = false;
    size_t slab_off = 0;
    size_t slab_floats = 0;
};

constexpr int kMaxRingParts = 8;
struct Knobs {
    int ws = -1;
    int wide = 0;
    int no_overlap = 0;
    int slot_cap = 384;
    int spill_gb = 0;
    int cu_slack = 0;
    int flush_streams = 2;
    int flush_tail = 0;
    int ring_parts = 3;
    int dw_ksplit = 0;
    int ws_prio = 0;
    int stagger = 0;
    int no_lean = 0;
    int no_ybits = 0;
    int overlay16 = 0;
    int no_xl = 0;
    int rr = 1;
    int rr_qmax = 100;
    int heb171 = 0;
    int heb_fp32 = 0;
    int u_row = 5000;
    int u_gemm0 = 1200;
    int u_kb = 200;
    int u_kbt = 68;
    int u_eh = 3000, u_eb = 1300, u_ef = 500;
};

inline int parse_tuning(const char* str, Knobs& k) {
    if (!str) return 0;
    std::string s(str);
    size_t pos = 0;
    while (pos < s.size()) {
        size_t end = s.find_first_of(",;", pos);
        if (end == std::string::npos) end = s.size();
        std::string item = s.substr(pos, end - pos);
        pos = end + 1;
        while (!item.empty() && item.front() == ' ') item.erase(item.begin());
        while (!item.empty() && item.back() == ' ') item.pop_back();
        if (item.empty()) continue;
        const size_t eq = item.find('=');
        const std::string key = item.substr(0, eq);
        const int val = eq == std::string::npos ? 1 : atoi(item.c_str() + eq + 1);
        struct { const char* name; int* dst; } table[] = {
            {"ws", &k.ws}, {"wide", &k.wide}, {"no_overlap", &k.no_overlap},
            {"slot_cap", &k.slot_cap}, {"spill_gb", &k.spill_gb}, {"cu_slack", &k.cu_slack}, {"ring_parts", &k.ring_parts}, {"flush_tail", &k.flush_tail}, {"flush_streams", &k.flush_streams}, {"dw_ksplit", &k.dw_ksplit},
            {"ws_prio", &k.ws_prio}, {"stagger", &k.stagger}, {"no_lean", &k.no_lean}, {"no_ybits", &k.no_ybits}, {"overlay16", &k.overlay16}, {"heb_fp32", &k.heb_fp32}, {"heb171", &k.heb171}, {"rr", &k.rr}, {"rr_qmax", &k.rr_qmax}, {"no_xl", &k.no_xl},
            {"u_row", &k.u_row}, {"u_gemm0", &k.u_gemm0}, {"u_kb", &k.u_kb}, {"u_kbt", &k.u_kbt}, {"u_eh", &k.u_eh}, {"u_eb", &k.u_eb}, {"u_ef", &k.u_ef}};
        bool found = false;
        for (auto& t : table)
            if (key == t.name) { *t.dst = val; found = true; }
        if (!found) return fail(MCPC_EINVAL, "unknown tuning key '%s' in mcpc_net_desc::tuning", key.c_str());
    }
    if (k.ws != -1 && k.ws != 0 && k.ws != 2 && k.ws != 3 && k.ws != 4)
        return fail(MCPC_EINVAL, "tuning ws=%d: 0 (barrier kernel), 2 (in-place kernel), 3 (unified-wave kernel) or 4 (layer-wise kernels)", k.ws);
    if (k.ws == 4) {
        const Knobs dflt;
        const struct { const char* name; bool set; } lds_only[] = {
            {"no_lean", k.no_lean != 0}, {"no_xl", k.no_xl != 0}, {"overlay16", k.overlay16 != 0}, {"rr", k.rr != dflt.rr},
            {"u_row", k.u_row != dflt.u_row}, {"u_gemm0", k.u_gemm0 != dflt.u_gemm0}, {"u_kb", k.u_kb != dflt.u_kb}, {"u_kbt", k.u_kbt != dflt.u_kbt},
            {"u_eh", k.u_eh != dflt.u_eh}, {"u_eb", k.u_eb != dflt.u_eb}, {"u_ef", k.u_ef != dflt.u_ef}};
        for (auto& t : lds_only)
            if (t.set) return fail(MCPC_EINVAL, "tuning ws=4 (layer-wise kernels) together with %s, a knob of the LDS-resident kernels", t.name);
    }
    if (k.slot_cap < 2) k.slot_cap = 2;
    if (k.cu_slack < 0) k.cu_slack = 0;
    if (k.ring_parts < 2 || k.ring_parts > kMaxRingParts) return fail(MCPC_EINVAL, "tuning ring_parts=%d: 2..%d", k.ring_parts, kMaxRingParts);
    return 0;
}

struct LdsRegion { const char* name; int layer; int off, floats; };
struct StepPlan {
    int lds_a[kMaxLatent]{}, lds_e[kMaxLatent]{}, lds_x[kMaxLatent]{}, lds_bias[kMaxLatent]{};
    int lds_eo = 0, lds_red = 0, lds_ws_sync = 0, lds_spillmax = 0, lds_rowexp = 0, lds_hbias = 0, lds_yw = 0, lds_bytes = 0;
    int lds_zero = 0;
    int head_ld = kChunkTiles * 16 + kLdPad;
    bool xl = false;
    int g_first = -1;
    int ws2_chunk = 0, ws2_ring = 0;
    bool ws2_overlay = true;
    std::vector<LdsRegion> regions;
    std::vector<KPhase> table;
    int n_phases = 0;
    KPhase* dev = nullptr;
    int take(const char* name, int layer, int& off, int floats) { regions.push_back({name, layer, off, floats}); off += floats; return off - floats; }
};

struct UPlan {
    bool ok = false;
    bool on = false;
    bool prefer = false;
    StepPlan plan;
};

struct EnginePlan {
    Knobs knobs;
    int L = 0, Bpad = 0, nwg = 0, has_head = 0;
    int nwg_live = 0;
    static constexpr int ct = 16;
    int nw = kWaves;
    int ws = 0;
    bool lw = false;
    int npad[kMaxLatent]{};
    int out_pad = 0;
    Lin lin[kMaxLatent + 1];
    StepPlan main;
    UPlan u;
    std::vector<LwJob> lw_table;
    int lw_nf = 0, lw_nb = 0;
    bool rr = false;
    int rr_k = 0, rr_m = 0;
    std::vector<int> rr_count, rr_off;
    std::vector<int> rr_host;
    std::string rr_name;
    std::string u_rr_name;
    int slots = 0, half_slots = 0;
    size_t slot_bytes = 0;
};

static const char* const kLwName = "mcpc::mcpc_lw_fwd_kernel + mcpc::mcpc_lw_bwd_kernel";

inline KPhase blank_phase() { KPhase k{}; k.dep_e = -1; k.dep_g = -1; k.dep_se = -1; k.b_row = -1; k.o_row = -1; return k; }
inline void set_gemm(KPhase& k, int a_lin, int kw) { k.a_lin = a_lin; k.kw = kw; k.nkb = kblocks(kw); k.a_tile_stride = k.nkb * kFragBlock; }

inline int plan_lds(const EnginePlan& e, StepPlan& p) {
    p = StepPlan{};
    int buf[2] = {0, 0};
    const int CT = e.ct;
    for (int l = 0; l < e.L; ++l) buf[l & 1] = std::max(buf[l & 1], CT * (e.npad[l] + kLdPad));
    const int eo_floats = e.has_head ? CT * (kChunkTiles * 16 + kLdPad) : 0;
    const int eo_buf = ((e.L - 1) & 1) ^ 1;
    buf[eo_buf] = std::max(buf[eo_buf], eo_floats);
    int off = 0;
    const int base[2] = {p.take("buf", 0, off, buf[0]), p.take("buf", 1, off, buf[1])};
    for (int l = 0; l < e.L; ++l) p.lds_a[l] = base[l & 1];
    p.lds_eo = base[eo_buf];
    for (int l = 1; l < e.L; ++l) p.lds_e[l] = p.take("e", l, off, CT * (e.npad[l] + kLdPad));
    p.lds_red = p.take("red", -1, off, 2 * (kMaxLatent + 1) * kMaxWaves);
    p.lds_zero = p.take("zero", -1, off, 16);
    p.lds_spillmax = p.take("spillmax", -1, off, kSpillTensors);
    p.lds_bytes = off * (int)sizeof(float);
    if (p.lds_bytes > kLdsLimit)
        return fail(MCPC_ENOMEM, "network needs %d bytes of LDS per workgroup (> 163840): latent widths too large for the fused kernel", p.lds_bytes);
    return 0;
}

inline void take_xl(const EnginePlan& e, StepPlan& p, int& off, bool with_yw) {
    for (int l = 0; l < e.L; ++l) p.lds_x[l] = p.take("x", l, off, e.ct * (e.npad[l] + kLdPad));
    for (int l = 0; l < e.L; ++l) p.lds_bias[l] = p.take("bias", l, off, l >= 1 ? e.npad[l] : e.ct * (e.npad[0] + kLdPad));
    if (e.has_head) p.lds_hbias = p.take("hbias", -1, off, e.out_pad);
    if (e.has_head && with_yw) p.lds_yw = p.take("yw", -1, off, (e.ct * ((e.out_pad + 31) / 32) + 3) / 4 * 4);
    p.xl = true;
}

inline int plan_lds_ws2(const EnginePlan& e, StepPlan& p) {
    p = StepPlan{};
    const int CT = e.ct, L = e.L;
    int off = 0;
    for (int l = 0; l < L; ++l) p.lds_a[l] = p.take("fx", l, off, CT * (e.npad[l] + kLdPad));
    p.lds_red = p.take("red", -1, off, 2 * (kMaxLatent + 1) * kMaxWaves);
    p.lds_ws_sync = p.take("ws_sync", -1, off, 16);
    int e_sum = 0;
    for (int l = 1; l < L; ++l) e_sum += CT * (e.npad[l] + kLdPad);
    int ring_floats = 0;
    if (e.has_head) {
        const int ht = std::max(e.out_pad / 16, 1);
        const int span = kWs2Pairs * ws2_nt<1>();
        auto ring_of = [&](int hc, int nb) { return nb * CT * (hc * 16 + kLdPad); };
        constexpr int tail = 16 + kSpillTensors + kRowExpFloats;
        auto fits = [&](int hc, int nb) { return (off + tail + std::max(ring_of(hc, nb), e_sum)) * (int)sizeof(float) <= kLdsLimit; };
        auto fits_apart = [&](int hc, int nb) { return (off + tail + ring_of(hc, nb) + e_sum) * (int)sizeof(float) <= kLdsLimit; };
        const int tq = kKB / 16, hb = (ht + tq - 1) / tq;
        int hcb_fit = 0;
        for (int hcb = std::min(span / tq, hb); hcb >= 1; --hcb)
            if (fits(hcb * tq, 2)) { hcb_fit = hcb; break; }
        if (!hcb_fit) return fail(MCPC_ENOMEM, "in-place schedule does not fit the LDS");
        const int nch = (hb + hcb_fit - 1) / hcb_fit;
        const int hc = tq * ((hb + nch - 1) / nch);
        const int nb = (nch >= 3 && fits(hc, 3)) ? 3 : 2;
        p.ws2_chunk = hc; p.ws2_ring = nb; ring_floats = ring_of(hc, nb);
        if (L >= 2 && fits_apart(hc, nb) && !e.knobs.overlay16) p.ws2_overlay = false;
    }
    int e_off = off;
    for (int l = 1; l < L; ++l) p.lds_e[l] = p.take("e", l, e_off, CT * (e.npad[l] + kLdPad));
    p.lds_eo = p.ws2_overlay ? off : e_off;
    if (ring_floats) p.regions.push_back({"ring", -1, p.lds_eo, ring_floats});
    off += p.ws2_overlay ? std::max(ring_floats, e_sum) : ring_floats + e_sum;
    p.lds_zero = p.take("zero", -1, off, 16);
    p.lds_spillmax = p.take("spillmax", -1, off, kSpillTensors);
    p.lds_rowexp = p.take("rowexp", -1, off, kRowExpFloats);
    if (!e.knobs.no_xl) {
        StepPlan with = p;
        int end = off;
        take_xl(e, with, end, true);
        if (end * (int)sizeof(float) <= kLdsLimit) { p = with; off = end; }
    }
    p.lds_bytes = off * (int)sizeof(float);
    if (p.lds_bytes > kLdsLimit) return fail(MCPC_ENOMEM, "in-place schedule does not fit the LDS (%d bytes)", p.lds_bytes);
    return 0;
}

inline void build_phases_ws2(const EnginePlan& e, StepPlan& p) {
    const int L = e.L;
    const int span = kWs2Pairs * ws2_nt<1>();
    auto tiles = [&](int l) { return e.npad[l] / 16; };
    enum { REF_LAST_BWD = -1000, REF_LAST_FWD = -2000, REF_LAST_HB = -3000, REF_LAST_BWD_GEMM = -4000, REF_LAST_BWD_ANY = -5000 };
    auto fwd_entries = [&](int l, std::vector<KPhase>& out) {
        for (int base = 0; base < tiles(l); base += span) {
            KPhase k = blank_phase();
            k.type = PH_FWD; k.layer = l; k.tile0 = base; k.ntiles = std::min(span, tiles(l) - base);
            if (l == 0) {
                k.flags = PHF_MU1 | PHF_WS_EPI;
            } else {
                set_gemm(k, l, 16 * tiles(l - 1));
                k.b_lds = p.lds_a[l - 1]; k.ldb = e.npad[l - 1] + kLdPad;
                k.out_lds = p.lds_e[l]; k.out_ld = e.npad[l] + kLdPad;
                k.b_row = rowexp_fx(l - 1); k.o_row = rowexp_e(l);
                k.flags = PHF_WS_GEMM | PHF_WS_EPI; k.dep_e = REF_LAST_BWD - (l - 1);
                if (e.has_head && p.ws2_overlay) k.dep_g = REF_LAST_HB;
                else if (e.has_head) {
                    k.dep_g = REF_LAST_BWD_GEMM; k.dep_se = REF_LAST_BWD_ANY;
                }
            }
            out.push_back(k);
        }
    };
    std::vector<KPhase> fill, after;
    if (e.has_head && !p.ws2_overlay) {
        if (L >= 2) fwd_entries(1, fill);
        fwd_entries(0, fill);
        for (int l = 2; l < L; ++l) fwd_entries(l, fill);
    } else {
        for (int l = L - 1; l >= 0; --l) fwd_entries(l, (l >= 1 && e.has_head) ? after : fill);
    }
    std::vector<KPhase>& ph = p.table;
    size_t nf = 0;
    if (e.has_head) {
        const int hc = p.ws2_chunk, R = p.ws2_ring;
        const int ht = e.out_pad / 16;
        const int nch = (ht + hc - 1) / hc;
        const int tq = kKB / 16, hb = (ht + tq - 1) / tq;
        std::vector<int> c_start(nch + 1, 0);
        for (int c = 0; c < nch; ++c) c_start[c + 1] = std::min(ht, c_start[c] + tq * (hb / nch + (c < hb % nch ? 1 : 0)));
        const int chunk_floats = e.ct * (hc * 16 + kLdPad);
        int e_sum = 0;
        for (int l = 1; l < L; ++l) e_sum += e.ct * (e.npad[l] + kLdPad);
        std::vector<int> idx_f(nch, -1), idx_b(nch, -1);
        auto add_f = [&](int c) {
            KPhase f = blank_phase();
            f.type = PH_HEADF; f.layer = L - 1; f.tile0 = c_start[c]; f.ntiles = c_start[c + 1] - c_start[c]; f.rot = c & (kWs2Pairs - 1);
            set_gemm(f, L, 16 * tiles(L - 1));
            f.b_lds = p.lds_a[L - 1]; f.ldb = e.npad[L - 1] + kLdPad;
            f.out_lds = p.lds_eo + (c % R) * chunk_floats; f.out_ld = hc * 16 + kLdPad;
            f.b_row = rowexp_fx(L - 1); f.o_row = rowexp_ring(c % R);
            f.flags = PHF_WS_GEMM | PHF_WS_EPI; f.dep_e = REF_LAST_BWD - (L - 1);
            if (c >= R) f.dep_g = idx_b[c - R];
            else if (p.ws2_overlay && (c % R) * chunk_floats < e_sum) { f.dep_g = REF_LAST_BWD_GEMM; f.dep_se = REF_LAST_BWD_ANY; }
            idx_f[c] = (int)ph.size(); ph.push_back(f);
        };
        auto add_b = [&](int c) {
            KPhase b = blank_phase();
            b.type = PH_HEADB; b.layer = L - 1; b.tile0 = 0; b.ntiles = tiles(L - 1);
            b.a_lin = L; b.a_tile_stride = kblocks(e.out_pad) * kFragBlock; b.a_off0 = (c_start[c] / tq) * kFragBlock;
            b.kw = 16 * (c_start[c + 1] - c_start[c]); b.nkb = (c_start[c + 1] - c_start[c] + tq - 1) / tq;
            b.b_lds = p.lds_eo + (c % R) * chunk_floats; b.ldb = hc * 16 + kLdPad;
            b.b_row = rowexp_ring(c % R);
            b.flags = PHF_WS_GEMM; b.dep_e = idx_f[c];
            idx_b[c] = (int)ph.size(); ph.push_back(b);
            if (nf < fill.size()) ph.push_back(fill[nf++]);
        };
        for (int c = 0; c < nch; ++c) {
            add_f(c);
            if (c >= R - 1) add_b(c - (R - 1));
        }
        for (int c = std::max(nch - (R - 1), 0); c < nch; ++c) add_b(c);
    }
    while (nf < fill.size()) ph.push_back(fill[nf++]);
    for (auto it = after.rbegin(); it != after.rend(); ++it) ph.push_back(*it);
    for (int base = 0; base < tiles(L - 1); base += span) {
        KPhase k = blank_phase();
        k.type = PH_BWD; k.layer = L - 1; k.tile0 = base; k.ntiles = std::min(span, tiles(L - 1) - base);
        k.flags = PHF_WS_EPI | (e.has_head ? PHF_WS2_HANDOFF : 0);
        k.sign = e.has_head ? 1.0f : 0.0f;
        k.out_lds = p.lds_a[L - 1]; k.out_ld = e.npad[L - 1] + kLdPad;
        k.o_row = rowexp_fx(L - 1);
        ph.push_back(k);
    }
    for (int l = 1; l <= L - 1; ++l)
        for (int base = 0; base < tiles(l - 1); base += span) {
            KPhase k = blank_phase();
            k.type = PH_BWD; k.layer = l - 1; k.tile0 = base; k.ntiles = std::min(span, tiles(l - 1) - base);
            set_gemm(k, l, 16 * tiles(l));
            k.b_lds = p.lds_e[l]; k.ldb = e.npad[l] + kLdPad; k.sign = -1.0f;
            k.out_lds = p.lds_a[l - 1]; k.out_ld = e.npad[l - 1] + kLdPad;
            k.b_row = rowexp_e(l); k.o_row = rowexp_fx(l - 1);
            k.flags = PHF_WS_GEMM | PHF_WS_EPI; k.dep_e = REF_LAST_FWD - l;
            ph.push_back(k);
        }
    { KPhase k = blank_phase(); k.type = PH_ENERGY; k.flags = PHF_WS_EPI; ph.push_back(k); }
    std::vector<int> last_fwd(L, -1), last_bwd(L, -1);
    int last_hb = -1, last_bwd_gemm = -1, last_bwd_any = -1;
    for (size_t i = 0; i < ph.size(); ++i) {
        if (ph[i].type == PH_FWD) last_fwd[ph[i].layer] = (int)i;
        if (ph[i].type == PH_BWD) { last_bwd[ph[i].layer] = (int)i; last_bwd_any = (int)i; if (ph[i].flags & PHF_WS_GEMM) last_bwd_gemm = (int)i; }
        if (ph[i].type == PH_HEADB) last_hb = (int)i;
    }
    auto resolve = [&](int d) {
        if (d == REF_LAST_BWD_ANY) return last_bwd_any;
        if (d == REF_LAST_BWD_GEMM) return last_bwd_gemm;
        if (d == REF_LAST_HB) return last_hb;
        if (d <= REF_LAST_FWD && d > REF_LAST_HB) return last_fwd[REF_LAST_FWD - d];
        if (d <= REF_LAST_BWD && d > REF_LAST_FWD) return last_bwd[REF_LAST_BWD - d];
        return d;
    };
    for (auto& k : ph) { k.dep_e = resolve(k.dep_e); k.dep_g = resolve(k.dep_g); k.dep_se = resolve(k.dep_se); }
    auto g_works = [&](const KPhase& k) { return (k.flags & (PHF_WS_GEMM | PHF_WS2_HANDOFF)) != 0; };
    p.g_first = -1;
    for (size_t i = 0; i < ph.size(); ++i) if (g_works(ph[i])) { p.g_first = (int)i; break; }
    for (size_t i = 0; i < ph.size(); ++i) {
        ph[i].next_g = p.g_first;
        for (size_t d = 1; d <= ph.size(); ++d) {
            const size_t j = (i + d) % ph.size();
            if (g_works(ph[j])) { ph[i].next_g = (int)j; break; }
        }
    }
    p.n_phases = (int)ph.size();
}

inline void plan_lds_u(const EnginePlan& e, UPlan& u) {
    u.ok = false;
    const int CT = e.ct, L = e.L;
    for (int yw_in_lds = 1; yw_in_lds >= 0 && !u.ok; --yw_in_lds) {
        StepPlan& p = u.plan = StepPlan{};
        int off = 0;
        for (int l = 0; l < L; ++l) p.lds_a[l] = p.take("fx", l, off, CT * (e.npad[l] + kLdPad));
        for (int l = 1; l < L; ++l) p.lds_e[l] = p.take("e", l, off, CT * (e.npad[l] + kLdPad));
        p.lds_red = p.take("red", -1, off, 2 * (kMaxLatent + 1) * kMaxWaves);
        p.lds_ws_sync = off;
        p.lds_eo = p.take("eo", -1, off, e.has_head ? CT * (e.out_pad + kLdPad) : 0);
        p.head_ld = e.out_pad + kLdPad;
        p.lds_zero = p.take("zero", -1, off, 16);
        p.lds_spillmax = p.take("spillmax", -1, off, kSpillTensors);
        p.lds_rowexp = p.take("rowexp", -1, off, (rowexp_ring(0) + 1) * 16);
        p.lds_yw = -1;
        take_xl(e, p, off, yw_in_lds != 0);
        p.g_first = 0;
        p.lds_bytes = off * (int)sizeof(float);
        u.ok = p.lds_bytes <= kLdsLimit;
    }
}
// ... 404 lines not shown
```

### montecarlopredictivecoding_amd/csrc/mcpc_steps_ws2.h

```cpp
#pragma once

namespace mcpc {

#ifdef MCPC_EXP_NOGEMM
#define MCPC_EXP_GEMM_GATE && P.n_steps < 0
#else
#define MCPC_EXP_GEMM_GATE
#endif

#ifndef MCPC_WS2_PAIRS
#define MCPC_WS2_PAIRS 4
#endif
constexpr int kWs2Pairs = MCPC_WS2_PAIRS;
#ifndef MCPC_WS2_SPAN
#define MCPC_WS2_SPAN 16
#endif
#ifndef MCPC_WS2_WAVES_PER_EU
#define MCPC_WS2_WAVES_PER_EU 2
#endif
constexpr int kWs2NT = MCPC_WS2_SPAN / kWs2Pairs;
#ifndef MCPC_WS2_NT16
#define MCPC_WS2_NT16 kWs2NT
#endif
template <int CTT> constexpr int ws2_nt() { return MCPC_WS2_NT16; }
constexpr int kWs2Threads = 2 * kWs2Pairs * 64;
static_assert(kWs2Pairs == 4 || kWs2Pairs == 8, "4 or 8 pairs");

#ifdef MCPC_STAMPS_ENTRY
#define STAMP_ENTRY_ADD(p_, d_)                                                                      \
    do {                                                                                             \
        const unsigned long long dd_ = (d_);                                                         \
        switch (p_) {                                                                                \
            case 0: st_sum[0] += dd_; break; case 1: st_sum[1] += dd_; break; case 2: st_sum[2] += dd_; break;     \
            case 3: st_sum[3] += dd_; break; case 4: st_sum[4] += dd_; break; case 5: st_sum[5] += dd_; break;     \
            case 6: st_sum[6] += dd_; break; case 7: st_sum[7] += dd_; break; case 8: st_sum[8] += dd_; break;     \
            case 9: st_sum[9] += dd_; break; case 10: st_sum[10] += dd_; break; case 11: st_sum[11] += dd_; break; \
            case 12: st_sum[12] += dd_; break; case 13: st_sum[13] += dd_; break; case 14: st_sum[14] += dd_; break; \
            default: st_sum[15] += dd_; break;                                                       \
        }                                                                                            \
    } while (0)
#undef STAMP
#define STAMP(i) do {} while (0)
#endif

struct alignas(16) Ws2Sync {
    int prog_e[kWs2Pairs];
    int prog_g[kWs2Pairs];
};

typedef int i32x4_t __attribute__((ext_vector_type(4)));
__device__ __forceinline__ int ws2_min_all(const int* p) {
    if constexpr (kWs2Pairs == 4) {
        const i32x4_t v = *reinterpret_cast<const volatile i32x4_t*>(p);
        return min(min(v.x, v.y), min(v.z, v.w));
    } else {
        int m = ws_ld(p);
#pragma unroll
        for (int i = 1; i < kWs2Pairs; ++i) m = min(m, ws_ld(p + i));
        return m;
    }
}
__device__ __forceinline__ void ws2_wait_all(const int* p, int need, int* err, int& dead) {
    if (__builtin_expect(ws2_min_all(p) < need, 0)) {
        if (!dead) {
            int spin = 0;
            bool ok = false;
#pragma clang loop unroll(disable)
            do {
                if (MCPC_WS_SLEEP > 0) __builtin_amdgcn_s_sleep(MCPC_WS_SLEEP);
                ok = ws2_min_all(p) >= need;
            } while (!ok && ++spin < kWsSpinLimit);
            if (!ok) { if ((threadIdx.x & 63) == 0) atomicOr(err, 1); dead = 1; }
        }
    }
    MCPC_WS_FENCE(__ATOMIC_ACQUIRE);
}

__device__ __forceinline__ int ws2_need(int base, int n_ent, int p, int dep) {
    return (dep > p ? base - n_ent : base) + dep + 1;
}

template <int NT>
__device__ __forceinline__ void ws2_prefetch(const KPhase& ph, int k, int lane, const void* dummy, int& nt_out, int (&aoff)[NT],
                                             frag_t (&pre0)[NT]) {
    const int kk = (k + ph.rot) & (kWs2Pairs - 1);
    int nt = (ph.ntiles - kk + kWs2Pairs - 1) / kWs2Pairs;
    nt = nt < 0 ? 0 : (nt > NT ? NT : nt);
    if (!(ph.flags & PHF_WS_GEMM) || ph.nkb <= 0) nt = 0;
    nt_out = nt;
    const bool valid = nt > 0;
    const gu32x4* const A = valid ? (const gu32x4*)ph.A : (const gu32x4*)dummy;
#pragma unroll
    for (int i = 0; i < NT; ++i) {
        const int ii = i < nt ? i : 0;
        const int off = valid ? (ph.tile0 + kk + kWs2Pairs * ii) * ph.a_tile_stride + ph.a_off0 : 0;
        aoff[i] = off;
        pre0[i] = load_frag(A, off, lane);
    }
}

template <int ACT>
__device__ __forceinline__ void ws2_fill_fx(const KLayer& Ly, float* lds, int chain0, int tid, int ct_rows, bool keep_x,
                                            float* lds_rowexp = nullptr, int row_id = 0) {
    const int qpr = Ly.npad / 4;
    for (int idx = tid; idx < ct_rows * qpr; idx += kWs2Threads) {
        const int r = idx / qpr, u0 = 4 * (idx - r * qpr);
        const f32x4 x = ld4s(Ly.x + (size_t)(chain0 + r) * Ly.npad + u0);
        f32x4 fx;
        fx.x = actf<ACT>(x.x); fx.y = actf<ACT>(x.y); fx.z = actf<ACT>(x.z); fx.w = actf<ACT>(x.w);
        st4(lds + Ly.lds_a + r * Ly.ld + u0, fx);
        if (keep_x) st4(lds + Ly.lds_x + r * Ly.ld + u0, x);
        if (lds_rowexp != nullptr && r < 16) rowexp_track(lds_rowexp, row_id, r, absmax4(0.f, fx), 0u);
    }
}

__device__ __forceinline__ void ws2_fill_constants(const KParams& P, float* lds, int chain0, int tid, int ct_rows) {
    for (int l = 1; l < P.L; ++l) {
        const KLayer& Ly = P.layer[l];
        for (int i = tid; i < Ly.npad / 4; i += kWs2Threads) st4(lds + Ly.lds_bias + 4 * i, ld4(Ly.bias + 4 * i));
    }
    {
        const KLayer& Ly = P.layer[0];
        const int qpr = Ly.npad / 4;
        for (int idx = tid; idx < ct_rows * qpr; idx += kWs2Threads) {
            const int r = idx / qpr, u0 = 4 * (idx - r * qpr);
            st4(lds + Ly.lds_bias + r * Ly.ld + u0, ld4(P.mu1 + (size_t)(chain0 + r) * Ly.npad + u0));
        }
    }
    if (P.has_head) {
        const KHead& H = P.head;
        for (int i = tid; i < H.npad / 4; i += kWs2Threads) st4(lds + H.lds_bias + 4 * i, ld4(H.bias + 4 * i));
        if (H.lds_yw >= 0) {
            uint32_t* const yw = reinterpret_cast<uint32_t*>(lds + H.lds_yw);
            for (int idx = tid; idx < ct_rows * H.ywords; idx += kWs2Threads) {
                const int r = idx / H.ywords, w = idx - r * H.ywords;
                yw[idx] = H.ybits[(size_t)(chain0 + r) * H.ywords + w];
            }
        }
    }
}

__device__ __forceinline__ int vreg(int s) { int v; asm volatile("v_mov_b32 %0, %1" : "=v"(v) : "s"(s)); return v; }
__device__ __forceinline__ float vreg(float s) { float v; asm volatile("v_mov_b32 %0, %1" : "=v"(v) : "s"(s)); return v; }
__device__ __forceinline__ float* vreg(float* s) {
    const uint64_t u = (uint64_t)s;
    const uint32_t lo = (uint32_t)vreg((int)(uint32_t)u), hi = (uint32_t)vreg((int)(uint32_t)(u >> 32));
    return (float*)(((uint64_t)hi << 32) | lo);
}

template <int CTT, int NW, int NTW>
__device__ __forceinline__ float ws2_headf_epilogue(const KParams& P, const KPhase& ph, float* lds, int nt, int wave, int lane,
                                                    int chain0, const f32x4 (&acc)[NTW][CTT], const f32x4 (&pa)[NTW][CTT],
                                                    const f32x4 (&pb)[NTW][CTT], int slot, int rec_idx, bool do_energy) {
    const KHead& H = P.head;
    const int c = lane & 15, q = lane >> 4;
    const int kind = H.loss_kind;
    const int npad = vreg(H.npad), n = vreg(H.n), ld = vreg(ph.out_ld), B = vreg(P.B), mask_start = vreg(H.mask_start);
    const float inv_var = vreg(H.inv_var);
    const int eo_off = vreg(ph.out_lds), tile0x16 = vreg(16 * ph.tile0);
    float* const spill = slot >= 0 ? vreg(H.spill_e + (size_t)slot * P.Bpad * H.npad) : nullptr;
    const int spill_tm = vreg(H.spill_tm);
    float* const rec = (rec_idx >= 0 && H.rec_out != nullptr) ? H.rec_out + (size_t)rec_idx * P.B * H.n : nullptr;
    float lsum = 0.f;
    float omx = 0.f;
#pragma unroll
    for (int i = 0; i < NTW; ++i) {
        if (i >= nt) continue;
        const int u0 = tile0x16 + 16 * (wave + NW * i) + 4 * q;
#pragma unroll
        for (int ct = 0; ct < CTT; ++ct) {
            const int cl = 16 * ct + c, chain = chain0 + cl;
            const bool live = chain < B;
            const f32x4 o = acc[i][ct] + pb[i][ct];
            f32x4 e = splat(0.f);
            if (kind != MCPC_LOSS_NONE) {
                const f32x4 y = pa[i][ct];
                const float ov[4] = {o.x, o.y, o.z, o.w}, yv[4] = {y.x, y.y, y.z, y.w};
                float ev[4];
                if (kind == MCPC_LOSS_GAUSSIAN) {
#pragma unroll
                    for (int r = 0; r < 4; ++r) {
                        const bool on = live && (u0 + r) >= mask_start && (u0 + r) < n;
                        const float dlt = ov[r] - yv[r];
                        ev[r] = on ? inv_var * dlt : 0.f;
                        lsum += on ? 0.5f * inv_var * dlt * dlt : 0.f;
                    }
                } else if (do_energy) {
#pragma unroll
                    for (int r = 0; r < 4; ++r) {
                        const bool on = live && (u0 + r) >= mask_start && (u0 + r) < n;
                        float sg, bc;
                        sigmoid_bce_f(ov[r], yv[r], sg, bc);
                        ev[r] = on ? sg - yv[r] : 0.f;
                        lsum += on ? bc : 0.f;
                    }
                } else {
#pragma unroll
                    for (int r = 0; r < 4; ++r) {
                        const bool on = live && (u0 + r) >= mask_start && (u0 + r) < n;
                        ev[r] = on ? sigmoid_f(ov[r]) - yv[r] : 0.f;
                    }
                }
                e.x = ev[0]; e.y = ev[1]; e.z = ev[2]; e.w = ev[3];
            }
            st4(lds + eo_off + cl * ld + (u0 - tile0x16), e);
            if (slot >= 0) { st4s(spill + spill_offset(spill_tm, (size_t)chain, u0, npad), e); omx = absmax4(omx, e); }
            if (rec != nullptr && live) st_unpadded(rec, chain, H.n, u0, o);
        }
    }
    if (slot >= 0) spill_track(lds + P.lds_spillmax, kSpillIdEo, omx, lane);
    return lsum;
}

template <int CTT, bool MIX = false>
__global__ __launch_bounds__(kWs2Threads, MCPC_WS2_WAVES_PER_EU) void mcpc_steps_ws2_kernel(const KParams P) {
    extern __shared__ __attribute__((aligned(16))) float lds[];
#define WS2_BLOCK blockIdx.x
#define WS2_NBLOCKS gridDim.x
#include "mcpc_steps_ws2_body.inc"
#undef WS2_BLOCK
#undef WS2_NBLOCKS
}

}
```

### montecarlopredictivecoding_amd/csrc/mcpc_steps_ws2_body.inc

```
    constexpr int NW = kWs2Pairs, NTW = ws2_nt<CTT>();
    const int tid = threadIdx.x;
    const int lane = tid & 63;
    const int wave8 = __builtin_amdgcn_readfirstlane(tid >> 6);
    const bool is_g = wave8 < kWs2Pairs;
    const int k = wave8 & (kWs2Pairs - 1);
    const int c = lane & 15, q = lane >> 4;
    const int unit = MIX ? P.wg_list[WS2_BLOCK] : (int)WS2_BLOCK;
    const int chain0 = unit * (16 * CTT);
    const int t_first = MIX ? P.t0 + P.wg_rel[WS2_BLOCK] * P.rr_q : P.t0;
    const int L = P.L;
    const int n_ent = P.n_phases;
    Ws2Sync* sync = reinterpret_cast<Ws2Sync*>(lds + P.lds_ws_sync);
    int dead = 0;
    for (int i = tid; i < P.lds_floats / 4; i += kWs2Threads) st4(lds + 4 * i, splat(0.f));
    __syncthreads();
    if (tid < 2 * kWs2Pairs) reinterpret_cast<int*>(sync)[tid] = 0;
    const int upd_mode = (P.update_x && P.xopt == MCPC_XOPT_SGD)
                             ? (P.noise_mode == MCPC_NOISE_PHILOX ? 2 : (P.noise_mode == MCPC_NOISE_NONE ? 1 : 0)) : 0;
    const bool lean_adam = P.update_x && P.xopt == MCPC_XOPT_ADAM && P.noise_mode == MCPC_NOISE_NONE;
    const bool lean = (upd_mode != 0 || lean_adam) && chain0 < P.B && P.lean_ok;
    const bool xl = CTT == 1 && lean && P.xl != 0;
#ifdef MCPC_EXP_NOLEAN
    const bool rowexp = false;
#else
    const bool rowexp = CTT == 1 && lean;
#endif
    float* const rx = rowexp ? lds + P.lds_rowexp : nullptr;
    for (int l = 0; l < L; ++l) {
        const KLayer& Ly = P.layer[l];
        if (Ly.act == MCPC_ACT_RELU) ws2_fill_fx<MCPC_ACT_RELU>(Ly, lds, chain0, tid, 16 * CTT, xl, rx, rowexp_fx(l));
        else if (Ly.act == MCPC_ACT_TANH) ws2_fill_fx<MCPC_ACT_TANH>(Ly, lds, chain0, tid, 16 * CTT, xl, rx, rowexp_fx(l));
        else ws2_fill_fx<MCPC_ACT_IDENTITY>(Ly, lds, chain0, tid, 16 * CTT, xl, rx, rowexp_fx(l));
    }
    if (xl) ws2_fill_constants(P, lds, chain0, tid, 16 * CTT);
    __syncthreads();

    if (is_g) {
        if (P.ws_prio == 2) __builtin_amdgcn_s_setprio(2);
        int p = P.g_first;
        if (p < 0) return;
        const bool y_bounded = P.has_head && *P.head.y_bounded != 0;
        KPhase ph_next = load_phase(P.phases, p);
        int nt_next, aoff[NTW];
        frag_t pre0[NTW];
#pragma unroll
        for (int i = 0; i < NTW; ++i) { pre0[i] = frag_zero(); aoff[i] = 0; }
        ws2_prefetch(ph_next, k, lane, P.dummy, nt_next, aoff, pre0);
        STAMP_DECL
#ifdef MCPC_STAMPS
        const unsigned long long clk_m0 = mcpc_stamp(), clk_r0 = wall_clock64();
#endif
        for (int s = 0; s < P.n_steps; ++s) {
            const int base = s * n_ent;
            f32x4 accb[NTW][CTT];
#pragma unroll
            for (int i = 0; i < NTW; ++i)
#pragma unroll
                for (int ct = 0; ct < CTT; ++ct) accb[i][ct] = splat(0.f);
            int accb_run = kRunNone, accb_aexp = 0;
#pragma unroll 1
            for (;;) {
                const KPhase ph = ph_next;
                const int nt = nt_next;
                const int p_next = ph.next_g;
                const bool wraps = p_next <= p;
                const bool has_next = !wraps || (s + 1 < P.n_steps);
                if (has_next) ph_next = load_phase(P.phases, p_next);
                const bool handoff = (ph.flags & PHF_WS2_HANDOFF) != 0;
                const bool is_headb = ph.type == PH_HEADB;
                const bool works = true;
                const bool stores = !is_headb;
                f32x4 acc[NTW][CTT];
#pragma unroll
                for (int i = 0; i < NTW; ++i)
#pragma unroll
                    for (int ct = 0; ct < CTT; ++ct) acc[i][ct] = splat(0.f);
                STAMP(0);
#ifdef MCPC_STAMPS_ENTRY
                const unsigned long long ge0 = mcpc_stamp();
                unsigned long long gwait = 0;
#endif
                if (works) {
                    if (ph.dep_e >= 0) ws2_wait_all(sync->prog_e, ws2_need(base, n_ent, p, ph.dep_e), P.err, dead);
#ifdef MCPC_STAMPS_ENTRY
                    gwait = mcpc_stamp() - ge0;
#endif
                    STAMP(1);
                    if (is_headb) {
                        if (nt > 0 MCPC_EXP_GEMM_GATE) {
                            const int hb_exp = headb_fixed_exp(P.head.loss_kind, y_bounded);
                            const bool hb_word = hb_exp == kScaleAuto && rowexp && ph.b_row >= 0;
                            const int fixed_b = hb_word ? rowexp_read(rx, ph.b_row, c) : hb_exp;
                            GemmScale gs{load_wexp(P.wexp, ph.a_lin), GS_ACCUM, fixed_b, accb_run,
                                         P.head.npad <= kShortK * kKB ? 1 : 0, (hb_exp == kScaleAuto && !hb_word) ? 1 : 0};
                            gemm_tiles<NTW, CTT, NW>(accb, ph.A, aoff, nt, ph.nkb, ph.kw, lds + ph.b_lds, ph.ldb, lane, pre0, lds + P.lds_zero, gs);
                            accb_run = gs.run; accb_aexp = gs.a_exp;
                        }
                        STAMP(2);
                    } else {
                        if (handoff) {
#pragma unroll
                            for (int i = 0; i < NTW; ++i)
#pragma unroll
                                for (int ct = 0; ct < CTT; ++ct) acc[i][ct] = accb[i][ct];
                            if (accb_run != kRunNone) gemm_unscale<NTW, CTT>(acc, accb_aexp, accb_run);
                        }
                        if (nt > 0 && ph.nkb > 0 MCPC_EXP_GEMM_GATE) {
                            const bool has_word = rowexp && ph.b_row >= 0;
                            const int fixed_b = has_word ? rowexp_read(rx, ph.b_row, c) : kScaleAuto;
                            GemmScale gs{load_wexp(P.wexp, ph.a_lin), GS_FRESH, fixed_b, kRunNone, -1, has_word ? 0 : 1};
                            gemm_tiles<NTW, CTT, NW>(acc, ph.A, aoff, nt, ph.nkb, ph.kw, lds + ph.b_lds, ph.ldb, lane, pre0, lds + P.lds_zero, gs);
                        }
                        STAMP(3);
                    }
                }
                ws2_prefetch(ph_next, k, lane, P.dummy, nt_next, aoff, pre0);
                STAMP(4);
                if (stores) {
#ifdef MCPC_STAMPS_ENTRY
                    const unsigned long long gw0 = mcpc_stamp();
#endif
                    if (ph.dep_g >= 0) ws2_wait_all(sync->prog_g, ws2_need(base, n_ent, p, ph.dep_g), P.err, dead);
                    if (ph.dep_se >= 0) ws2_wait_all(sync->prog_e, ws2_need(base, n_ent, p, ph.dep_se), P.err, dead);
#ifdef MCPC_STAMPS_ENTRY
                    gwait += mcpc_stamp() - gw0;
#endif
                    const int kk = (k + ph.rot) & (NW - 1);
                    int ntw = (ph.ntiles - kk + NW - 1) / NW;
                    ntw = ntw < 0 ? 0 : (ntw > NTW ? NTW : ntw);
                    float* const out = lds + ph.out_lds;
                    const int col0 = (ph.type == PH_HEADF) ? 0 : 16 * ph.tile0;
#pragma unroll
                    for (int i = 0; i < NTW; ++i) {
                        if (i >= ntw) continue;
                        const int col = col0 + 16 * (kk + NW * i) + 4 * q;
#pragma unroll
                        for (int ct = 0; ct < CTT; ++ct) st4(out + (16 * ct + c) * ph.out_ld + col, acc[i][ct]);
                    }
                }
                if (lane == 0) ws_publish(&sync->prog_g[k], base + p + 1);
                STAMP(5);
#ifdef MCPC_STAMPS_ENTRY
                if (MCPC_STAMPS_ENTRY == 1) STAMP_ENTRY_ADD(p, gwait);
                else if (MCPC_STAMPS_ENTRY == 2) STAMP_ENTRY_ADD(p, mcpc_stamp() - ge0);
#endif
                p = p_next;
                if (wraps) break;
            }
        }
#if defined(MCPC_STAMPS) && !defined(MCPC_STAMPS_ENTRY)
        st_sum[6] = mcpc_stamp() - clk_m0;
        st_sum[7] = wall_clock64() - clk_r0;
#endif
#ifdef MCPC_STAMPS
        if (lane == 0 && P.dbg != nullptr)
            for (int i = 0; i < 16; ++i) P.dbg[((size_t)WS2_BLOCK * (2 * kWs2Pairs) + wave8) * 16 + i] = st_sum[i];
#endif
        return;
    }

    if (P.ws_prio == 1) __builtin_amdgcn_s_setprio(2);
    const bool clk_wave = P.clk != nullptr && WS2_BLOCK == 0 && k == 0;
    unsigned long long clk_c0 = 0, clk_w0 = 0;
    if (clk_wave) { clk_c0 = __builtin_amdgcn_s_memtime(); clk_w0 = __builtin_amdgcn_s_memrealtime(); }
    LeanLane<CTT> LL;
    LL.c = c; LL.q = q;
#pragma unroll
    for (int ct = 0; ct < CTT; ++ct) {
        LL.chain[ct] = (uint32_t)(chain0 + 16 * ct + c); LL.lrow[ct] = (uint32_t)(16 * ct + c);
        const bool live = chain0 + 16 * ct + c < P.B;
        LL.livem[ct] = live ? ~0u : 0u;
    }
    const bool ybin = lean && P.has_head && *P.head.y_binary != 0;
    const bool e0_in_regs = lean && P.layer[0].ntiles <= NW;
    bool e0_dirty = false;
    f32x4 e0acc[CTT];
#pragma unroll
    for (int ct = 0; ct < CTT; ++ct) e0acc[ct] = splat(0.f);
    if (e0_in_regs && t_first + P.n_steps > P.acc_begin && t_first < P.acc_end) lean_load_e0<CTT>(P, k, LL, e0acc);
    STAMP_DECL
    for (int s = 0; s < P.n_steps; ++s) {
        const int t = t_first + s;
        const int s_tab = MIX ? t - P.t0 : s;
        const int base = s * n_ent;
        const bool do_energy = (P.energy_mode == MCPC_ENERGY_ALL) || (P.energy_mode == MCPC_ENERGY_LAST && t == P.T - 1);
        const int slot = (t >= P.acc_begin && t < P.acc_end) ? (t - P.spill_t0) : -1;
        int rec_idx = -1;
        if (P.rec_count > 0 && t >= P.rec_begin) {
            const int kk = (t - P.rec_begin) / P.rec_stride;
            if (kk < P.rec_count && P.rec_begin + kk * P.rec_stride == t) rec_idx = kk;
        }
        float* red = lds + P.lds_red + (s & 1) * (kMaxLatent + 1) * kMaxWaves;
        float en_acc = 0.f;
#pragma unroll 1
        for (int p = 0; p < n_ent; ++p) {
            const KPhase ph = load_phase(P.phases, p);
#ifdef MCPC_STAMPS_ENTRY
            const unsigned long long ee0 = mcpc_stamp();
            unsigned long long ewait = 0;
#endif
            if (ph.type == PH_ENERGY) {
                if (do_energy && lane <= kMaxLatent) red[lane * kMaxWaves + k] = en_acc;
                if (lane == 0) ws_publish(&sync->prog_e[k], base + p + 1);
                if (do_energy && k == 0) {
                    ws2_wait_all(sync->prog_e + 0, base + p + 1, P.err, dead);
                    if (lane <= kMaxLatent) {
                        double v = 0.0;
                        const bool used = (lane < L) || (lane == kMaxLatent && P.has_head);
                        if (used) {
#pragma unroll
                            for (int w = 0; w < kWs2Pairs; ++w) v += (double)red[lane * kMaxWaves + w];
                        }
                        const int erow = (P.energy_mode == MCPC_ENERGY_ALL) ? t : 0;
                        double* const ep = P.epart + ((size_t)erow * P.epart_slots + (size_t)unit * CTT) * (kMaxLatent + 1) + lane;
                        ep[0] = v;
                        if (CTT == 2) ep[kMaxLatent + 1] = 0.0;
                    }
                }
                continue;
            }
            if (!(ph.flags & PHF_WS_EPI)) {
                if (lane == 0) ws_publish(&sync->prog_e[k], base + p + 1);
                continue;
            }
            const int kk = (k + ph.rot) & (NW - 1);
            int nt = (ph.ntiles - kk + NW - 1) / NW;
            nt = nt < 0 ? 0 : (nt > NTW ? NTW : nt);
#ifndef MCPC_EXP_NOLEAN
            if (lean) {
                const int act = P.layer[ph.layer].act;
                const int* const pg = &sync->prog_g[k];
                const int need = base + p + 1;
#ifdef MCPC_STAMPS_ENTRY
                if (((ph.flags & PHF_WS_GEMM) && ph.nkb > 0) || (ph.flags & PHF_WS2_HANDOFF)) {
                    const unsigned long long ew0 = mcpc_stamp();
                    ws_wait_one(pg, need, P.err, dead);
                    ewait = mcpc_stamp() - ew0;
                }
#endif
#ifdef MCPC_EXP_NOEPI
                if (P.n_steps < 0)
#endif
                if (ph.type == PH_FWD) {
                    float esum;
                    if (ph.layer == 0 && slot >= 0) e0_dirty = true;
                    if constexpr (CTT == 1) {
                        if (xl) {
                            if (act == MCPC_ACT_RELU) esum = lean_fwd<CTT, NW, NTW, MCPC_ACT_RELU, true>(P, ph, lds, nt, kk, LL, slot, rec_idx, pg, need, P.err, dead, e0acc, e0_in_regs, rx, (unsigned)(s + 1));
                            else if (act == MCPC_ACT_TANH) esum = lean_fwd<CTT, NW, NTW, MCPC_ACT_TANH, true>(P, ph, lds, nt, kk, LL, slot, rec_idx, pg, need, P.err, dead, e0acc, e0_in_regs, rx, (unsigned)(s + 1));
                            else esum = lean_fwd<CTT, NW, NTW, MCPC_ACT_IDENTITY, true>(P, ph, lds, nt, kk, LL, slot, rec_idx, pg, need, P.err, dead, e0acc, e0_in_regs, rx, (unsigned)(s + 1));
                        }
                    }
                    if (!xl) {
                    if (act == MCPC_ACT_RELU) esum = lean_fwd<CTT, NW, NTW, MCPC_ACT_RELU>(P, ph, lds, nt, kk, LL, slot, rec_idx, pg, need, P.err, dead, e0acc, e0_in_regs, rx, (unsigned)(s + 1));
                    else if (act == MCPC_ACT_TANH) esum = lean_fwd<CTT, NW, NTW, MCPC_ACT_TANH>(P, ph, lds, nt, kk, LL, slot, rec_idx, pg, need, P.err, dead, e0acc, e0_in_regs, rx, (unsigned)(s + 1));
                    else esum = lean_fwd<CTT, NW, NTW, MCPC_ACT_IDENTITY>(P, ph, lds, nt, kk, LL, slot, rec_idx, pg, need, P.err, dead, e0acc, e0_in_regs, rx, (unsigned)(s + 1));
                    }
                    if (do_energy) { esum = wave_sum(esum); if (lane == ph.layer) en_acc += esum; }
                } else if (ph.type == PH_HEADF) {
                    float lsum;
                    bool done = false;
                    if constexpr (CTT == 1) {
                        if (xl) {
                            if (ybin) lsum = lean_headf<CTT, NW, NTW, true, true>(P, ph, lds, nt, kk, LL, slot, rec_idx, do_energy, pg, need, P.err, dead, true, rx);
                            else lsum = lean_headf<CTT, NW, NTW, true, false>(P, ph, lds, nt, kk, LL, slot, rec_idx, do_energy, pg, need, P.err, dead, false, rx);
                            done = true;
                        }
                    }
                    if (!done) lsum = lean_headf<CTT, NW, NTW>(P, ph, lds, nt, kk, LL, slot, rec_idx, do_energy, pg, need, P.err, dead, ybin, rx);
                    if (do_energy) { lsum = wave_sum(lsum); if (lane == kMaxLatent) en_acc += lsum; }
                } else if (ph.type == PH_BWD) {
                    bool done = false;
                    if constexpr (CTT == 1) {
                        if (xl) {
                            done = true;
                            if (lean_adam) {
                                if (act == MCPC_ACT_RELU) lean_bwd<CTT, NW, NTW, MCPC_ACT_RELU, false, true, true>(P, ph, lds, nt, kk, LL, t, pg, need, P.err, dead, s_tab, rx, (unsigned)(s + 1));
                                else if (act == MCPC_ACT_TANH) lean_bwd<CTT, NW, NTW, MCPC_ACT_TANH, false, true, true>(P, ph, lds, nt, kk, LL, t, pg, need, P.err, dead, s_tab, rx, (unsigned)(s + 1));
                                else lean_bwd<CTT, NW, NTW, MCPC_ACT_IDENTITY, false, true, true>(P, ph, lds, nt, kk, LL, t, pg, need, P.err, dead, s_tab, rx, (unsigned)(s + 1));
                            } else if (upd_mode == 2) {
                                if (act == MCPC_ACT_RELU) lean_bwd<CTT, NW, NTW, MCPC_ACT_RELU, true, false, true>(P, ph, lds, nt, kk, LL, t, pg, need, P.err, dead, 0, rx, (unsigned)(s + 1));
                                else if (act == MCPC_ACT_TANH) lean_bwd<CTT, NW, NTW, MCPC_ACT_TANH, true, false, true>(P, ph, lds, nt, kk, LL, t, pg, need, P.err, dead, 0, rx, (unsigned)(s + 1));
                                else lean_bwd<CTT, NW, NTW, MCPC_ACT_IDENTITY, true, false, true>(P, ph, lds, nt, kk, LL, t, pg, need, P.err, dead, 0, rx, (unsigned)(s + 1));
                            } else {
                                if (act == MCPC_ACT_RELU) lean_bwd<CTT, NW, NTW, MCPC_ACT_RELU, false, false, true>(P, ph, lds, nt, kk, LL, t, pg, need, P.err, dead, 0, rx, (unsigned)(s + 1));
                                else if (act == MCPC_ACT_TANH) lean_bwd<CTT, NW, NTW, MCPC_ACT_TANH, false, false, true>(P, ph, lds, nt, kk, LL, t, pg, need, P.err, dead, 0, rx, (unsigned)(s + 1));
                                else lean_bwd<CTT, NW, NTW, MCPC_ACT_IDENTITY, false, false, true>(P, ph, lds, nt, kk, LL, t, pg, need, P.err, dead, 0, rx, (unsigned)(s + 1));
                            }
                        }
                    }
                    if (done) {
                    } else if (lean_adam) {
                        if (act == MCPC_ACT_RELU) lean_bwd<CTT, NW, NTW, MCPC_ACT_RELU, false, true>(P, ph, lds, nt, kk, LL, t, pg, need, P.err, dead, s_tab, rx, (unsigned)(s + 1));
                        else if (act == MCPC_ACT_TANH) lean_bwd<CTT, NW, NTW, MCPC_ACT_TANH, false, true>(P, ph, lds, nt, kk, LL, t, pg, need, P.err, dead, s_tab, rx, (unsigned)(s + 1));
                        else lean_bwd<CTT, NW, NTW, MCPC_ACT_IDENTITY, false, true>(P, ph, lds, nt, kk, LL, t, pg, need, P.err, dead, s_tab, rx, (unsigned)(s + 1));
                    } else if (upd_mode == 2) {
                        if (act == MCPC_ACT_RELU) lean_bwd<CTT, NW, NTW, MCPC_ACT_RELU, true>(P, ph, lds, nt, kk, LL, t, pg, need, P.err, dead, 0, rx, (unsigned)(s + 1));
                        else if (act == MCPC_ACT_TANH) lean_bwd<CTT, NW, NTW, MCPC_ACT_TANH, true>(P, ph, lds, nt, kk, LL, t, pg, need, P.err, dead, 0, rx, (unsigned)(s + 1));
                        else lean_bwd<CTT, NW, NTW, MCPC_ACT_IDENTITY, true>(P, ph, lds, nt, kk, LL, t, pg, need, P.err, dead, 0, rx, (unsigned)(s + 1));
                    } else {
                        if (act == MCPC_ACT_RELU) lean_bwd<CTT, NW, NTW, MCPC_ACT_RELU, false>(P, ph, lds, nt, kk, LL, t, pg, need, P.err, dead, 0, rx, (unsigned)(s + 1));
                        else if (act == MCPC_ACT_TANH) lean_bwd<CTT, NW, NTW, MCPC_ACT_TANH, false>(P, ph, lds, nt, kk, LL, t, pg, need, P.err, dead, 0, rx, (unsigned)(s + 1));
                        else lean_bwd<CTT, NW, NTW, MCPC_ACT_IDENTITY, false>(P, ph, lds, nt, kk, LL, t, pg, need, P.err, dead, 0, rx, (unsigned)(s + 1));
                    }
                }
                if (lane == 0) ws_publish(&sync->prog_e[k], base + p + 1);
#ifdef MCPC_STAMPS_ENTRY
                if (MCPC_STAMPS_ENTRY == 3) STAMP_ENTRY_ADD(p, ewait);
                else if (MCPC_STAMPS_ENTRY == 4) STAMP_ENTRY_ADD(p, mcpc_stamp() - ee0);
#endif
                continue;
            }
#endif
            f32x4 acc[NTW][CTT], pa[NTW][CTT], pb[NTW][CTT];
#pragma unroll
            for (int i = 0; i < NTW; ++i)
#pragma unroll
                for (int ct = 0; ct < CTT; ++ct) { acc[i][ct] = splat(0.f); pa[i][ct] = splat(0.f); pb[i][ct] = splat(0.f); }
            const KLayer& Ly = P.layer[ph.layer];
            STAMP(8);
            issue_epilogue_loads<CTT, NW, NTW>(P, ph, lds, nt, kk, lane, chain0, pa, pb);
            STAMP(9);
            const bool from_g = ((ph.flags & PHF_WS_GEMM) && ph.nkb > 0) || (ph.flags & PHF_WS2_HANDOFF);
            if (from_g) {
#ifdef MCPC_STAMPS_ENTRY
                const unsigned long long ew0 = mcpc_stamp();
#endif
                ws_wait_one(&sync->prog_g[k], base + p + 1, P.err, dead);
#ifdef MCPC_STAMPS_ENTRY
                ewait = mcpc_stamp() - ew0;
#endif
                STAMP(10);
                const float* const src = lds + ph.out_lds;
                const int col0 = (ph.type == PH_HEADF) ? 0 : 16 * ph.tile0;
#pragma unroll
                for (int i = 0; i < NTW; ++i) {
                    const int col = col0 + 16 * (kk + NW * (i < nt ? i : 0)) + 4 * q;
#pragma unroll
                    for (int ct = 0; ct < CTT; ++ct) acc[i][ct] = ld4(src + (16 * ct + c) * ph.out_ld + col);
                }
            }
#ifdef MCPC_EXP_NOEPI
            if (P.n_steps < 0)
#endif
            if (ph.type == PH_FWD) {
                float esum;
                if (Ly.act == MCPC_ACT_RELU) esum = fwd_epilogue<CTT, NW, NTW, MCPC_ACT_RELU, false>(P, ph, lds, nt, kk, lane, chain0, acc, pa, pb, slot, rec_idx);
                else if (Ly.act == MCPC_ACT_TANH) esum = fwd_epilogue<CTT, NW, NTW, MCPC_ACT_TANH, false>(P, ph, lds, nt, kk, lane, chain0, acc, pa, pb, slot, rec_idx);
                else esum = fwd_epilogue<CTT, NW, NTW, MCPC_ACT_IDENTITY, false>(P, ph, lds, nt, kk, lane, chain0, acc, pa, pb, slot, rec_idx);
                if (do_energy) { esum = wave_sum(esum); if (lane == ph.layer) en_acc += esum; }
            } else if (ph.type == PH_HEADF) {
                float lsum = ws2_headf_epilogue<CTT, NW, NTW>(P, ph, lds, nt, kk, lane, chain0, acc, pa, pb, slot, rec_idx, do_energy);
                if (do_energy) { lsum = wave_sum(lsum); if (lane == kMaxLatent) en_acc += lsum; }
            } else if (ph.type == PH_BWD) {
                if (Ly.act == MCPC_ACT_RELU) bwd_epilogue_mode<CTT, NW, NTW, MCPC_ACT_RELU, true>(P, ph, nt, kk, lane, chain0, acc, pa, pb, s_tab, t, upd_mode, lds);
                else if (Ly.act == MCPC_ACT_TANH) bwd_epilogue_mode<CTT, NW, NTW, MCPC_ACT_TANH, true>(P, ph, nt, kk, lane, chain0, acc, pa, pb, s_tab, t, upd_mode, lds);
                else bwd_epilogue_mode<CTT, NW, NTW, MCPC_ACT_IDENTITY, true>(P, ph, nt, kk, lane, chain0, acc, pa, pb, s_tab, t, upd_mode, lds);
            }
            if (lane == 0) ws_publish(&sync->prog_e[k], base + p + 1);
            if (ph.type == PH_FWD) STAMP(11); else if (ph.type == PH_HEADF) STAMP(12); else STAMP(13);
#ifdef MCPC_STAMPS_ENTRY
            if (MCPC_STAMPS_ENTRY == 3) STAMP_ENTRY_ADD(p, ewait);
            else if (MCPC_STAMPS_ENTRY == 4) STAMP_ENTRY_ADD(p, mcpc_stamp() - ee0);
#endif
        }
    }
    if constexpr (CTT == 1) {
        if (xl) lean_store_x<CTT, NW>(P, lds, k, LL);
    }
    spill_max_publish(P.spillmax, lds + P.lds_spillmax, lane);
    if (clk_wave && lane == 0) {
        atomicAdd(P.clk, __builtin_amdgcn_s_memtime() - clk_c0);
        atomicAdd(P.clk + 1, __builtin_amdgcn_s_memrealtime() - clk_w0);
    }
    if (e0_in_regs && e0_dirty) lean_flush_e0<CTT>(P, k, LL, e0acc);
#ifdef MCPC_STAMPS
    if (lane == 0 && P.dbg != nullptr)
        for (int i = 0; i < 16; ++i) P.dbg[((size_t)WS2_BLOCK * 8 + wave8) * 16 + i] = st_sum[i];
#endif
```

### montecarlopredictivecoding_amd/csrc/mcpc_ws2_lean.h

```cpp
#pragma once

namespace mcpc {

typedef const char __attribute__((address_space(1)))* gbytes_t;
typedef char __attribute__((address_space(1)))* gbytes_w_t;

__device__ __forceinline__ f32x4 gld4(const float* base, uint32_t boff) {
    return *reinterpret_cast<const gf32x4*>((gbytes_t)base + boff);
}
__device__ __forceinline__ f32x4 gld4s(const float* base, uint32_t boff) {
    return __builtin_nontemporal_load(reinterpret_cast<const gf32x4*>((gbytes_t)base + boff));
}
__device__ __forceinline__ void gst4s(float* base, uint32_t boff, f32x4 v) {
    __builtin_nontemporal_store(v, reinterpret_cast<gf32x4*>((gbytes_w_t)base + boff));
}
__device__ __forceinline__ uint32_t mul24(uint32_t a, uint32_t b) { return __umul24(a, b); }

#ifndef MCPC_SPILL_AUX
#define MCPC_SPILL_AUX -1
#endif
typedef unsigned int u32x4_t __attribute__((ext_vector_type(4)));
__device__ __forceinline__ void spill_st4(float* base, uint32_t image_bytes, uint32_t boff, f32x4 v, bool sys = true) {
#ifdef MCPC_EXP_NOSPILL
    (void)base; (void)image_bytes; (void)boff; (void)v; (void)sys;
#elif MCPC_SPILL_AUX < 0
    if (sys) {
        gst4s(base, boff, v); (void)image_bytes;
    } else {
        const __amdgpu_buffer_rsrc_t rsrc = __builtin_amdgcn_make_buffer_rsrc(base, 0, (int)image_bytes, 0x00020000);
        __builtin_amdgcn_raw_buffer_store_b128(__builtin_bit_cast(u32x4_t, v), rsrc, (int)boff, 0, 0);
    }
#else
    const __amdgpu_buffer_rsrc_t rsrc = __builtin_amdgcn_make_buffer_rsrc(base, 0, (int)image_bytes, 0x00020000);
    if (sys) __builtin_amdgcn_raw_buffer_store_b128(__builtin_bit_cast(u32x4_t, v), rsrc, (int)boff, 0, MCPC_SPILL_AUX);
    else __builtin_amdgcn_raw_buffer_store_b128(__builtin_bit_cast(u32x4_t, v), rsrc, (int)boff, 0, 0);
#endif
}

template <int CTT>
struct LeanLane {
    int c, q;
    uint32_t chain[CTT];
    uint32_t lrow[CTT];
    uint32_t livem[CTT];
};
__device__ __forceinline__ f32x4 mask4(f32x4 v, uint32_t m) {
    f32x4 r;
    r.x = __uint_as_float(__float_as_uint(v.x) & m); r.y = __uint_as_float(__float_as_uint(v.y) & m);
    r.z = __uint_as_float(__float_as_uint(v.z) & m); r.w = __uint_as_float(__float_as_uint(v.w) & m);
    return r;
}

template <int ACT> __device__ __forceinline__ f32x4 act4(f32x4 x) {
    f32x4 r;
    r.x = actf<ACT>(x.x); r.y = actf<ACT>(x.y); r.z = actf<ACT>(x.z); r.w = actf<ACT>(x.w);
    return r;
}

template <int CTT, int NW, int NTW, int ACT, bool XL = false, bool REG = false>
__device__ __forceinline__ float lean_fwd(const KParams& P, const KPhase& ph, float* lds, int nt, int kk, const LeanLane<CTT>& L,
                                          int slot, int rec_idx, const int* prog_g, int need, int* err, int& dead,
                                          f32x4 (&e0acc)[CTT], bool e0_in_regs, float* rx = nullptr, unsigned row_gen = 0u,
                                          const f32x4 (*racc)[CTT] = nullptr) {
    if (nt <= 0) return 0.f;
    const int tstep = REG ? ph.rot : NW;
    const KLayer& Ly = P.layer[ph.layer];
    const int l = ph.layer;
    const bool has_gemm = (ph.flags & PHF_WS_GEMM) && ph.nkb > 0;
    const uint32_t npad4 = 4u * (uint32_t)Ly.npad;
    uint32_t rowb[CTT], lrowb[CTT], orowb[CTT];
#pragma unroll
    for (int ct = 0; ct < CTT; ++ct) {
        rowb[ct] = mul24(L.chain[ct], npad4) + 16u * L.q;
        lrowb[ct] = mul24(L.lrow[ct], 4u * (uint32_t)Ly.ld) + 16u * L.q;
        orowb[ct] = mul24(L.lrow[ct], 4u * (uint32_t)ph.out_ld) + 16u * L.q;
    }
    f32x4 xv[NTW][CTT], bv[NTW][CTT];
    const float* const bsrc = l == 0 ? P.mu1 : Ly.bias;
#pragma unroll
    for (int i = 0; i < NTW; ++i) {
        const uint32_t tb = 64u * (uint32_t)(ph.tile0 + kk + tstep * (i < nt ? i : 0));
#pragma unroll
        for (int ct = 0; ct < CTT; ++ct) {
            if constexpr (XL) {
                xv[i][ct] = *reinterpret_cast<const f32x4*>(reinterpret_cast<const char*>(lds + Ly.lds_x) + lrowb[ct] + tb);
                bv[i][ct] = *reinterpret_cast<const f32x4*>(reinterpret_cast<const char*>(lds + Ly.lds_bias) + (l == 0 ? lrowb[ct] : 16u * L.q) + tb);
                (void)bsrc;
            } else {
#if defined(MCPC_EXP_NOX) || defined(MCPC_EXP_NOELOAD)
            xv[i][ct] = splat(0.5f);
#else
            xv[i][ct] = gld4s(Ly.x, rowb[ct] + tb);
#endif
#ifdef MCPC_EXP_NOELOAD
            bv[i][ct] = splat(0.25f); (void)bsrc;
#else
            bv[i][ct] = gld4(bsrc, (l == 0 ? rowb[ct] : 16u * L.q) + tb);
#endif
            }
        }
    }
    f32x4 av[NTW][CTT];
    if constexpr (REG) {
#pragma unroll
        for (int i = 0; i < NTW; ++i)
#pragma unroll
            for (int ct = 0; ct < CTT; ++ct) av[i][ct] = racc[i][ct];
        (void)has_gemm; (void)prog_g; (void)need; (void)err; (void)dead; (void)orowb;
    } else if (has_gemm) {
        ws_wait_one(prog_g, need, err, dead);
        const char* const src = reinterpret_cast<const char*>(lds + ph.out_lds);
#pragma unroll
        for (int i = 0; i < NTW; ++i) {
            const uint32_t tb = 64u * (uint32_t)(ph.tile0 + kk + tstep * (i < nt ? i : 0));
#pragma unroll
            for (int ct = 0; ct < CTT; ++ct) av[i][ct] = *reinterpret_cast<const f32x4*>(src + orowb[ct] + tb);
        }
    } else {
#pragma unroll
        for (int i = 0; i < NTW; ++i)
#pragma unroll
            for (int ct = 0; ct < CTT; ++ct) av[i][ct] = splat(0.f);
    }
    const float ecoef = Ly.ecoef;
    char* const e_lds = reinterpret_cast<char*>(lds + Ly.lds_e);
    float* const spill_a = slot >= 0 ? Ly.spill_a + (size_t)slot * P.Bpad * Ly.npad : nullptr;
    float* const spill_e = slot >= 0 ? (l > 0 ? Ly.spill_e + (size_t)slot * P.Bpad * Ly.npad : Ly.spill_e) : nullptr;
    float* const rec = (rec_idx >= 0 && Ly.rec != nullptr) ? Ly.rec + (size_t)rec_idx * P.B * Ly.n : nullptr;
    const uint32_t img_bytes = (uint32_t)P.Bpad * npad4;
    const bool sys = P.spill_sys != 0;
    float esum = 0.f;
    float amx = 0.f, emx = 0.f;
    float rmx = 0.f;
#pragma unroll
    for (int i = 0; i < NTW; ++i) {
        if (i >= nt) continue;
        const int tile = ph.tile0 + kk + tstep * i;
        const uint32_t tb = 64u * (uint32_t)tile;
#pragma unroll
        for (int ct = 0; ct < CTT; ++ct) {
            const f32x4 x = xv[i][ct];
            const f32x4 d = x - (av[i][ct] + bv[i][ct]);
            const f32x4 e = d * ecoef;
            if (l > 0) { *reinterpret_cast<f32x4*>(e_lds + lrowb[ct] + tb) = e; rmx = absmax4(rmx, e); }
            if (slot >= 0) {
#ifdef MCPC_EXP_SPILL_LINEAR
                const uint32_t sb = mul24(L.chain[ct] - (uint32_t)L.c, npad4) + 1024u * (uint32_t)tile + 16u * (uint32_t)(L.c + 16 * L.q);
#else
                const uint32_t sb = rowb[ct] + tb;
#endif
                const uint32_t sb_tm = mul24(L.chain[ct] - (uint32_t)L.c, npad4) + 1024u * (uint32_t)tile + 16u * (uint32_t)(L.c + 16 * L.q);
                spill_st4(spill_a, img_bytes, Ly.spill_a_tm ? sb_tm : sb, mask4(act4<ACT>(x), L.livem[ct]), sys);
                amx = absmax4(amx, mask4(act4<ACT>(x), L.livem[ct]));
                if (l > 0) { spill_st4(spill_e, img_bytes, Ly.spill_e_tm ? sb_tm : sb, mask4(e, L.livem[ct]), sys); emx = absmax4(emx, mask4(e, L.livem[ct])); }
                else if (e0_in_regs) e0acc[ct] = e0acc[ct] + e;
                else gst4s(spill_e, rowb[ct] + tb, gld4s(spill_e, rowb[ct] + tb) + e);
            }
            if (rec != nullptr && L.livem[ct]) st_unpadded(rec, (int)L.chain[ct], Ly.n, 16 * tile + 4 * L.q, x);
            const f32x4 dd = d * d;
            esum += L.livem[ct] ? 0.5f * ecoef * (dd.x + dd.y + dd.z + dd.w) : 0.f;
        }
    }
    if (slot >= 0) {
        spill_track(lds + P.lds_spillmax, spill_id_a(l), amx, L.c + 16 * L.q);
        if (l > 0) spill_track(lds + P.lds_spillmax, spill_id_e(l), emx, L.c + 16 * L.q);
    }
    if (CTT == 1 && rx != nullptr && ph.o_row >= 0) rowexp_track(rx, ph.o_row, L.c, rmx, row_gen);
    return esum;
}

template <int CTT>
__device__ __forceinline__ void lean_load_e0(const KParams& P, int kk, const LeanLane<CTT>& L, f32x4 (&e0acc)[CTT]) {
    const KLayer& Ly = P.layer[0];
    if (kk >= Ly.ntiles) return;
    const uint32_t npad4 = 4u * (uint32_t)Ly.npad;
#pragma unroll
    for (int ct = 0; ct < CTT; ++ct) e0acc[ct] = gld4s(Ly.spill_e, mul24(L.chain[ct], npad4) + 16u * L.q + 64u * (uint32_t)kk);
}
template <int CTT>
__device__ __forceinline__ void lean_flush_e0(const KParams& P, int kk, const LeanLane<CTT>& L, const f32x4 (&e0acc)[CTT]) {
    const KLayer& Ly = P.layer[0];
    if (kk >= Ly.ntiles) return;
    const uint32_t npad4 = 4u * (uint32_t)Ly.npad;
#pragma unroll
    for (int ct = 0; ct < CTT; ++ct) gst4s(Ly.spill_e, mul24(L.chain[ct], npad4) + 16u * L.q + 64u * (uint32_t)kk, e0acc[ct]);
}

template <int CTT, int NW>
__device__ __forceinline__ void lean_store_x(const KParams& P, const float* lds, int kk, const LeanLane<CTT>& L) {
    for (int l = 0; l < P.L; ++l) {
        const KLayer& Ly = P.layer[l];
        const uint32_t npad4 = 4u * (uint32_t)Ly.npad;
        for (int tile = kk; tile < Ly.ntiles; tile += NW) {
#pragma unroll
            for (int ct = 0; ct < CTT; ++ct) {
                const uint32_t lb = mul24(L.lrow[ct], 4u * (uint32_t)Ly.ld) + 16u * L.q + 64u * (uint32_t)tile;
                gst4s(Ly.x, mul24(L.chain[ct], npad4) + 16u * L.q + 64u * (uint32_t)tile,
                      *reinterpret_cast<const f32x4*>(reinterpret_cast<const char*>(lds + Ly.lds_x) + lb));
            }
        }
    }
}

template <int CTT, int NW, int NTW, int ACT, bool NOISE, bool ADAM = false, bool XL = false, bool REG = false>
__device__ __forceinline__ void lean_bwd(const KParams& P, const KPhase& ph, float* lds, int nt, int kk, const LeanLane<CTT>& L,
                                         int t, const int* prog_g, int need, int* err, int& dead, int s_tab = 0, float* rx = nullptr,
                                         unsigned row_gen = 0u, const f32x4 (*racc)[CTT] = nullptr) {
    static_assert(!(NOISE && ADAM), "Adam with the fused kick takes the generic epilogue");
    if (nt <= 0) return;
    const int tstep = REG ? ph.rot : NW;
    const KLayer& Ly = P.layer[ph.layer];
    const int l = ph.layer, n = Ly.n;
    const bool from_g = ((ph.flags & PHF_WS_GEMM) && ph.nkb > 0) || (ph.flags & PHF_WS2_HANDOFF);
    const uint32_t npad4 = 4u * (uint32_t)Ly.npad;
    uint32_t rowb[CTT], lrowb[CTT], orowb[CTT];
#pragma unroll
    for (int ct = 0; ct < CTT; ++ct) {
        rowb[ct] = mul24(L.chain[ct], npad4) + 16u * L.q;
        lrowb[ct] = mul24(L.lrow[ct], 4u * (uint32_t)Ly.ld) + 16u * L.q;
        orowb[ct] = mul24(L.lrow[ct], 4u * (uint32_t)ph.out_ld) + 16u * L.q;
    }
    const float ecoef = Ly.ecoef;
    f32x4 xv[NTW][CTT], ev[NTW][CTT];
    f32x4 mv[ADAM ? NTW : 1][CTT], vv[ADAM ? NTW : 1][CTT];
    const char* const e_lds = reinterpret_cast<const char*>(lds + Ly.lds_e);
#pragma unroll
    for (int i = 0; i < NTW; ++i) {
        const uint32_t tb = 64u * (uint32_t)(ph.tile0 + kk + tstep * (i < nt ? i : 0));
#pragma unroll
        for (int ct = 0; ct < CTT; ++ct) {
            if constexpr (XL) {
                xv[i][ct] = *reinterpret_cast<const f32x4*>(reinterpret_cast<const char*>(lds + Ly.lds_x) + lrowb[ct] + tb);
            } else {
#if defined(MCPC_EXP_NOX) || defined(MCPC_EXP_NOELOAD)
            xv[i][ct] = splat(0.5f);
#else
            xv[i][ct] = gld4s(Ly.x, rowb[ct] + tb);
#endif
            }
            if constexpr (ADAM) {
                const uint32_t mb = (mul24(L.chain[ct] >> 4, (uint32_t)Ly.ntiles) + (uint32_t)(ph.tile0 + kk + tstep * (i < nt ? i : 0))) * 1024u + 16u * (uint32_t)(L.c + 16 * L.q);
                mv[i][ct] = gld4s(Ly.m, mb);
                vv[i][ct] = gld4s(Ly.v, mb);
            }
#ifdef MCPC_EXP_NOELOAD
            if (l == 0) ev[i][ct] = (xv[i][ct] - splat(0.25f)) * ecoef;
#else
            if (l == 0) {
                if constexpr (XL) ev[i][ct] = (xv[i][ct] - *reinterpret_cast<const f32x4*>(reinterpret_cast<const char*>(lds + Ly.lds_bias) + lrowb[ct] + tb)) * ecoef;
                else ev[i][ct] = (xv[i][ct] - gld4(P.mu1, rowb[ct] + tb)) * ecoef;
            }
#endif
            else if constexpr (!ADAM) ev[i][ct] = *reinterpret_cast<const f32x4*>(e_lds + lrowb[ct] + tb);
        }
    }
    f32x4 av[NTW][CTT];
    if constexpr (REG) {
#pragma unroll
        for (int i = 0; i < NTW; ++i)
#pragma unroll
            for (int ct = 0; ct < CTT; ++ct) av[i][ct] = racc[i][ct];
        (void)from_g; (void)prog_g; (void)need; (void)err; (void)dead; (void)orowb;
    } else if (from_g) {
        ws_wait_one(prog_g, need, err, dead);
        const char* const src = reinterpret_cast<const char*>(lds + ph.out_lds);
#pragma unroll
        for (int i = 0; i < NTW; ++i) {
            const uint32_t tb = 64u * (uint32_t)(ph.tile0 + kk + tstep * (i < nt ? i : 0));
#pragma unroll
            for (int ct = 0; ct < CTT; ++ct) av[i][ct] = *reinterpret_cast<const f32x4*>(src + orowb[ct] + tb);
        }
    } else {
#pragma unroll
        for (int i = 0; i < NTW; ++i)
#pragma unroll
            for (int ct = 0; ct < CTT; ++ct) av[i][ct] = splat(0.f);
    }
    const float sign = ph.sign, lr = P.lr, nscale = P.noise_scale;
    const uint64_t seed = P.seed, step = P.step_base + (uint64_t)t, chain_base = P.chain_base;
    char* const fx_lds = reinterpret_cast<char*>(lds + Ly.lds_a);
    float rmx = 0.f;
#pragma unroll
    for (int i = 0; i < NTW; ++i) {
        if (i >= nt) continue;
        const int tile = ph.tile0 + kk + tstep * i;
        const uint32_t tb = 64u * (uint32_t)tile;
        const bool pad_tile = 16 * tile + 16 > n;
#pragma unroll
        for (int ct = 0; ct < CTT; ++ct) {
            const f32x4 x = xv[i][ct], back = av[i][ct];
            f32x4 e;
            if constexpr (ADAM) {
                if (l == 0) e = ev[i][ct];
                else e = *reinterpret_cast<const f32x4*>(e_lds + lrowb[ct] + tb);
            } else {
                e = ev[i][ct];
            }
            f32x4 g;
            g.x = e.x + sign * actd<ACT>(x.x, actf<ACT>(x.x)) * back.x;
            g.y = e.y + sign * actd<ACT>(x.y, actf<ACT>(x.y)) * back.y;
            g.z = e.z + sign * actd<ACT>(x.z, actf<ACT>(x.z)) * back.z;
            g.w = e.w + sign * actd<ACT>(x.w, actf<ACT>(x.w)) * back.w;
            f32x4 xn;
            if constexpr (ADAM) {
                f32x4 m = mv[i][ct], v = vv[i][ct];
                m.x = adam_m(m.x, g.x, P.omb1); m.y = adam_m(m.y, g.y, P.omb1); m.z = adam_m(m.z, g.z, P.omb1); m.w = adam_m(m.w, g.w, P.omb1);
                v.x = adam_v(v.x, g.x, P.beta2, P.omb2); v.y = adam_v(v.y, g.y, P.beta2, P.omb2); v.z = adam_v(v.z, g.z, P.beta2, P.omb2); v.w = adam_v(v.w, g.w, P.beta2, P.omb2);
                const uint32_t mb = (mul24(L.chain[ct] >> 4, (uint32_t)Ly.ntiles) + (uint32_t)tile) * 1024u + 16u * (uint32_t)(L.c + 16 * L.q);
                gst4s(Ly.m, mb, m);
                gst4s(Ly.v, mb, v);
                const float nss = P.adam_coef[2 * s_tab], bc2s = P.adam_coef[2 * s_tab + 1], eps = P.eps;
                xn.x = adam_x(x.x, m.x, v.x, nss, bc2s, eps);
                xn.y = adam_x(x.y, m.y, v.y, nss, bc2s, eps);
                xn.z = adam_x(x.z, m.z, v.z, nss, bc2s, eps);
                xn.w = adam_x(x.w, m.w, v.w, nss, bc2s, eps);
            } else {
                xn = x - g * lr;
            }
            if constexpr (NOISE)
                xn = xn + normals4(seed, step, (uint32_t)l, (uint32_t)(chain_base + (uint64_t)L.chain[ct]), (uint32_t)(4 * tile + L.q)) * nscale;
            if (pad_tile) {
                const int u0 = 16 * tile + 4 * L.q;
                if (u0 + 0 >= n) xn.x = 0.f;
                if (u0 + 1 >= n) xn.y = 0.f;
                if (u0 + 2 >= n) xn.z = 0.f;
                if (u0 + 3 >= n) xn.w = 0.f;
            }
            if constexpr (XL) {
                *reinterpret_cast<f32x4*>(reinterpret_cast<char*>(lds + Ly.lds_x) + lrowb[ct] + tb) = xn;
            } else {
#ifndef MCPC_EXP_NOX
            gst4s(Ly.x, rowb[ct] + tb, xn);
#endif
            }
            const f32x4 fxn = act4<ACT>(xn);
            *reinterpret_cast<f32x4*>(fx_lds + lrowb[ct] + tb) = fxn;
            rmx = absmax4(rmx, fxn);
        }
    }
    if (CTT == 1 && rx != nullptr && ph.o_row >= 0) rowexp_track(rx, ph.o_row, L.c, rmx, row_gen);
}

template <int CTT, int NW, int NTW, bool XL = false, bool YB = false, bool REG = false, bool YWG = false>
__device__ __forceinline__ float lean_headf(const KParams& P, const KPhase& ph, float* lds, int nt, int kk, const LeanLane<CTT>& L,
                                            int slot, int rec_idx, bool do_energy, const int* prog_g, int need, int* err, int& dead,
                                            bool ybin, float* rx = nullptr, const f32x4 (*racc)[CTT] = nullptr, unsigned row_gen = 0u,
                                            bool planes_ok = false, const uint32_t* ywreg = nullptr) {
    if (nt <= 0) return 0.f;
    const int tstep = REG ? ph.rot : NW;
    const KHead& H = P.head;
    const bool planes = REG && planes_ok;
    const int kind = H.loss_kind, n = H.n, mask_start = H.mask_start;
    const uint32_t npad4 = 4u * (uint32_t)H.npad;
    uint32_t rowb[CTT], orowb[CTT];
#pragma unroll
    for (int ct = 0; ct < CTT; ++ct) {
        rowb[ct] = mul24(L.chain[ct], npad4) + 16u * L.q;
        orowb[ct] = mul24(L.lrow[ct], 4u * (uint32_t)ph.out_ld) + 16u * L.q;
    }
    f32x4 yv[NTW][CTT], bv[NTW];
    uint32_t yw[NTW][CTT];
    const uint32_t wrow4 = 4u * (uint32_t)H.ywords;
#pragma unroll
    for (int i = 0; i < NTW; ++i) {
        const int tile = ph.tile0 + kk + tstep * (i < nt ? i : 0);
        const uint32_t tb = 64u * (uint32_t)tile;
        if constexpr (XL) {
            bv[i] = *reinterpret_cast<const f32x4*>(reinterpret_cast<const char*>(lds + H.lds_bias) + 16u * L.q + tb);
        } else {
#ifdef MCPC_EXP_NOELOAD
        bv[i] = splat(0.25f);
#else
        bv[i] = gld4(H.bias, 16u * L.q + tb);
#endif
        }
#pragma unroll
        for (int ct = 0; ct < CTT; ++ct) {
            if constexpr (XL && YB && YWG) {
                yv[i][ct] = splat(0.f);
                yw[i][ct] = ywreg[i];
            } else if constexpr (XL && YB) {
                yv[i][ct] = splat(0.f);
                yw[i][ct] = *reinterpret_cast<const uint32_t*>(reinterpret_cast<const char*>(lds + H.lds_yw) + mul24(L.lrow[ct], wrow4) + 4u * (uint32_t)(tile >> 1));
            } else if constexpr (XL) {
                const bool has_y = kind != MCPC_LOSS_NONE;
                yv[i][ct] = gld4s(has_y ? H.ytile : H.bias,
                                  has_y ? (mul24(L.chain[ct] >> 4, (uint32_t)H.ntiles) + (uint32_t)tile) * 1024u + 16u * (uint32_t)(L.c + 16 * L.q) : 16u * L.q + tb);
                yw[i][ct] = 0u;
            } else {
#if defined(MCPC_EXP_NOY) || defined(MCPC_EXP_NOELOAD)
            yv[i][ct] = splat(0.f); yw[i][ct] = 0u;
#else
            const bool fp32_y = kind != MCPC_LOSS_NONE && !ybin;
            yv[i][ct] = gld4s(fp32_y ? H.y : H.bias, fp32_y ? rowb[ct] + tb : 16u * L.q + tb);
            yw[i][ct] = *reinterpret_cast<const __attribute__((address_space(1))) uint32_t*>(
                (gbytes_t)H.ybits + mul24(L.chain[ct], wrow4) + 4u * (uint32_t)(tile >> 1));
#endif
            }
        }
    }
    char* const eo = reinterpret_cast<char*>(lds + ph.out_lds);
    f32x4 av[NTW][CTT];
    if constexpr (REG) {
#pragma unroll
        for (int i = 0; i < NTW; ++i)
#pragma unroll
            for (int ct = 0; ct < CTT; ++ct) av[i][ct] = racc[i][ct];
        (void)prog_g; (void)err; (void)dead;
    } else {
        ws_wait_one(prog_g, need, err, dead);
#pragma unroll
        for (int i = 0; i < NTW; ++i) {
            const uint32_t cb = 64u * (uint32_t)(kk + tstep * (i < nt ? i : 0));
#pragma unroll
            for (int ct = 0; ct < CTT; ++ct) av[i][ct] = *reinterpret_cast<const f32x4*>(eo + orowb[ct] + cb);
        }
    }
    const float inv_var = H.inv_var;
    float* const spill = slot >= 0 ? H.spill_e + (size_t)slot * P.Bpad * H.npad : nullptr;
    float* const rec = (rec_idx >= 0 && H.rec_out != nullptr) ? H.rec_out + (size_t)rec_idx * P.B * H.n : nullptr;
    float lsum = 0.f;
    float omx = 0.f;
    float rmx = 0.f;
#pragma unroll
    for (int i = 0; i < NTW; ++i) {
        if (i >= nt) continue;
        const int tile = ph.tile0 + kk + tstep * i;
        const uint32_t tb = 64u * (uint32_t)tile, cb = 64u * (uint32_t)(kk + tstep * i);
        const bool inside = 16 * tile >= mask_start && 16 * tile + 16 <= n;
#pragma unroll
        for (int ct = 0; ct < CTT; ++ct) {
            const f32x4 o = av[i][ct] + bv[i];
            f32x4 e = splat(0.f);
            if (kind != MCPC_LOSS_NONE) {
                f32x4 y = yv[i][ct];
                if (ybin) {
                    const uint32_t nib = yw[i][ct] >> (16u * (uint32_t)(tile & 1) + 4u * (uint32_t)L.q);
                    y.x = (float)(nib & 1u); y.y = (float)((nib >> 1) & 1u); y.z = (float)((nib >> 2) & 1u); y.w = (float)((nib >> 3) & 1u);
                }
                const float ov[4] = {o.x, o.y, o.z, o.w}, yy[4] = {y.x, y.y, y.z, y.w};
                float ev[4];
                const int u0 = 16 * tile + 4 * L.q;
                if (kind == MCPC_LOSS_GAUSSIAN) {
#pragma unroll
                    for (int r = 0; r < 4; ++r) {
                        const bool on = inside || ((u0 + r) >= mask_start && (u0 + r) < n);
                        const float dlt = ov[r] - yy[r];
                        ev[r] = on ? inv_var * dlt : 0.f;
                        lsum += (on && L.livem[ct]) ? 0.5f * inv_var * dlt * dlt : 0.f;
                    }
                } else if (do_energy) {
                    if (inside) {
#pragma unroll
                        for (int r = 0; r < 4; ++r) {
                            float sg, bc;
                            sigmoid_bce_f(ov[r], yy[r], sg, bc);
                            ev[r] = sg - yy[r];
                            lsum += L.livem[ct] ? bc : 0.f;
                        }
                    } else {
#pragma unroll
                        for (int r = 0; r < 4; ++r) {
                            const bool on = (u0 + r) >= mask_start && (u0 + r) < n;
                            float sg, bc;
                            sigmoid_bce_f(ov[r], yy[r], sg, bc);
                            ev[r] = on ? sg - yy[r] : 0.f;
                            lsum += (on && L.livem[ct]) ? bc : 0.f;
                        }
                    }
                } else {
#pragma unroll
                    for (int r = 0; r < 4; ++r) {
                        const bool on = inside || ((u0 + r) >= mask_start && (u0 + r) < n);
                        ev[r] = on ? sigmoid_f(ov[r]) - yy[r] : 0.f;
                    }
                }
                e.x = ev[0]; e.y = ev[1]; e.z = ev[2]; e.w = ev[3];
            }
            if (REG && planes) {
                unsigned h0, m0, h1, m1;
                const float sc = pow2i(headb_fixed_exp(MCPC_LOSS_BERNOULLI, true));
                split2_pair(f32x2{e.x, e.y}, sc, h0, m0);
                split2_pair(f32x2{e.z, e.w}, sc, h1, m1);
                char* const gp = eo + (orowb[ct] - 16u * L.q) + cb + 32u * (uint32_t)(L.q >> 1) + 8u * (uint32_t)(L.q & 1);
                *reinterpret_cast<uint2*>(gp) = make_uint2(h0, h1);
                *reinterpret_cast<uint2*>(gp + 16) = make_uint2(m0, m1);
            } else {
                *reinterpret_cast<f32x4*>(eo + orowb[ct] + cb) = e;
            }
            rmx = absmax4(rmx, e);
#ifdef MCPC_EXP_SPILL_LINEAR
            if (slot >= 0) spill_st4(spill, (uint32_t)P.Bpad * npad4, mul24(L.chain[ct] - (uint32_t)L.c, npad4) + 1024u * (uint32_t)tile + 16u * (uint32_t)(L.c + 16 * L.q), mask4(e, L.livem[ct]), P.spill_sys != 0);
#else
            if (slot >= 0) {
                spill_st4(spill, (uint32_t)P.Bpad * npad4,
                          H.spill_tm ? mul24(L.chain[ct] - (uint32_t)L.c, npad4) + 1024u * (uint32_t)tile + 16u * (uint32_t)(L.c + 16 * L.q) : rowb[ct] + tb,
                          mask4(e, L.livem[ct]), P.spill_sys != 0);
                omx = absmax4(omx, mask4(e, L.livem[ct]));
            }
#endif
            if (rec != nullptr && L.livem[ct]) st_unpadded(rec, (int)L.chain[ct], H.n, 16 * tile + 4 * L.q, o);
        }
    }
    if (slot >= 0) spill_track(lds + P.lds_spillmax, kSpillIdEo, omx, L.c + 16 * L.q);
    if (CTT == 1 && rx != nullptr && ph.o_row >= 0) rowexp_track(rx, ph.o_row, L.c, rmx, REG ? row_gen : (unsigned)need);
    return lsum;
}

}
```

Baseline: 17820.

## Add compile-time specialized ws2 step kernels selected from host-side target flags

Introduces a Ws2Mode template that fixes the update rule, XL, row-exponent tracking, spill mode, Bernoulli-bits head and ReLU activation at compile time. Three specialized ws2 kernels (hot, hot+spill, map) are instantiated alongside the generic one. The host copies the target-binary flags to pinned memory asynchronously and picks a specialized kernel only when the run matches. This is meant to remove runtime branches and dynamic loads in the hot step loop. In exchange it adds code size, an extra D2H copy with an event check, and a fallback to the generic kernel if the flags are not yet ready.

```diff
diff --git a/montecarlopredictivecoding_amd/csrc/mcpc_api.hip b/montecarlopredictivecoding_amd/csrc/mcpc_api.hip
--- a/montecarlopredictivecoding_amd/csrc/mcpc_api.hip
+++ b/montecarlopredictivecoding_amd/csrc/mcpc_api.hip
@@ -39,6 +39,9 @@
     int* y_binary = nullptr;
     int ywords = 0;
     bool target_bound = false;
+    int* y_flags_host = nullptr;
+    hipEvent_t y_flags_ev = nullptr;
+    bool y_flags_pending = false;
     const float* inputs = nullptr;
     hipStream_t aux = nullptr;
     hipEvent_t ev_steps[kMaxRingParts] = {}, ev_flush[kMaxRingParts] = {};
@@ -130,6 +133,8 @@
     if (e->spacer) { (void)hipStreamDestroy(e->spacer); e->spacer = nullptr; }
     if (e->ev_fork) { (void)hipEventDestroy(e->ev_fork); e->ev_fork = nullptr; }
     if (e->ev_join) { (void)hipEventDestroy(e->ev_join); e->ev_join = nullptr; }
+    if (e->y_flags_ev) { (void)hipEventDestroy(e->y_flags_ev); e->y_flags_ev = nullptr; }
+    if (e->y_flags_host) { (void)hipHostFree(e->y_flags_host); e->y_flags_host = nullptr; }
     F(e->rr_tab);
     for (auto& q : e->retired) { (void)hipFree(q.p); if (q.ev) (void)hipEventDestroy(q.ev); }
     e->retired.clear();
@@ -201,7 +206,8 @@
 hipError_t allow_lds(const void* fn, int bytes) { return hipFuncSetAttribute(fn, hipFuncAttributeMaxDynamicSharedMemorySize, bytes); }
 int upload_rounds(mcpc_engine* e) {
     if (const int rc = upload(e->rr_tab, e->rr_host, "the round-schedule tables")) return rc;
-    if (allow_lds((const void*)mcpc_steps_ws2_kernel<1, true>, e->main.lds_bytes) != hipSuccess) return fail(MCPC_EHIP, "hipFuncSetAttribute failed for the round schedule");
+    for (const Ws2SpecEntry& sp : kWs2Specs)
+        if (sp.fn[1] && allow_lds(sp.fn[1], e->main.lds_bytes) != hipSuccess) return fail(MCPC_EHIP, "hipFuncSetAttribute failed for the round schedule");
     return 0;
 }
 
@@ -289,6 +295,11 @@
         if ((rc = zeroed(e->ypad, (size_t)e->Bpad * e->out_pad)) || (rc = dmalloc(e->ytile, (size_t)e->Bpad * e->out_pad))) return bail(rc);
         e->ywords = (e->out_pad + 31) / 32;
         if ((rc = dmalloc(e->ybits, (size_t)e->Bpad * e->ywords)) || (rc = zeroed(e->y_binary, 3))) return bail(rc);
+        if (e->ws == 2 && !e->lw && !e->u.prefer && e->knobs.spec) {
+            if (hipHostMalloc((void**)&e->y_flags_host, 3 * sizeof(int), hipHostMallocDefault) != hipSuccess || hipEventCreateWithFlags(&e->y_flags_ev, hipEventDisableTiming) != hipSuccess)
+                return bail(fail(MCPC_EHIP, "pinned copy of the target flags: allocation failed"));
+            e->y_flags_host[0] = e->y_flags_host[1] = e->y_flags_host[2] = 0;
+        }
     }
     const int nlin = e->L + (e->has_head ? 1 : 0);
     for (int j = 0; j < nlin; ++j) {
@@ -317,7 +328,9 @@
         (rc = zeroed(e->clk, 2)) || (rc = zeroed(e->dummy, 1024)))
         return bail(rc);
     const void* kfn = e->ws == 2 ? (const void*)mcpc_steps_ws2_kernel<1> : (const void*)mcpc_steps_kernel<1, 4>;
-    const hipError_t herr = e->lw ? hipSuccess : allow_lds(kfn, e->main.lds_bytes);
+    hipError_t herr = e->lw ? hipSuccess : allow_lds(kfn, e->main.lds_bytes);
+    for (int i = WS2_SPEC_GENERIC + 1; i < WS2_SPEC_COUNT && herr == hipSuccess && e->ws == 2 && !e->lw; ++i)
+        if (kWs2Specs[i].fn[0]) herr = allow_lds(kWs2Specs[i].fn[0], e->main.lds_bytes);
     if (herr != hipSuccess) return bail(fail(MCPC_EHIP, "hipFuncSetAttribute(%d bytes LDS) failed: %s", e->main.lds_bytes, hipGetErrorString(herr)));
     if (e->rr && (rc = upload_rounds(e))) return bail(rc);
     if (e->u.on && (allow_lds((const void*)mcpc_steps_u_kernel<false>, e->u.plan.lds_bytes) != hipSuccess ||
@@ -386,6 +399,11 @@
     hipLaunchKernelGGL(mcpc_pack_target_bits_kernel, dim3(grid_for((size_t)e->Bpad * e->ywords)), dim3(256), 0, (hipStream_t)stream_,
                        e->ypad, e->ybits, e->y_binary, e->Bpad, e->out_pad, e->ywords);
     HIP_TRY(hipGetLastError());
+    if (e->y_flags_host && e->y_flags_ev) {
+        HIP_TRY(hipMemcpyAsync(e->y_flags_host, e->y_binary, 3 * sizeof(int), hipMemcpyDeviceToHost, (hipStream_t)stream_));
+        HIP_TRY(hipEventRecord(e->y_flags_ev, (hipStream_t)stream_));
+        e->y_flags_pending = true;
+    }
     e->target_bound = true;
     return MCPC_OK;
 }
@@ -847,6 +865,46 @@
     return P;
 }
 
+bool ws2_spec_candidate(const mcpc_engine* e, const KParams& P) {
+#ifdef MCPC_EXP_NOLEAN
+    return false;
+#endif
+    if (!e->y_flags_host || e->ws != 2 || e->lw) return false;
+    const bool kick = P.update_x && P.xopt == MCPC_XOPT_SGD && P.noise_mode == MCPC_NOISE_PHILOX;
+    const bool map = P.update_x && P.xopt == MCPC_XOPT_ADAM && P.noise_mode == MCPC_NOISE_NONE;
+    if (!kick && !map) return false;
+    if (!P.lean_ok || !P.xl) return false;
+    for (int l = 0; l < e->L; ++l)
+        if (P.layer[l].act != MCPC_ACT_RELU) return false;
+    return P.has_head && P.head.loss_kind == MCPC_LOSS_BERNOULLI && e->target_bound;
+}
+
+int target_flags_on_host(mcpc_engine* e, const KParams& P, int run_steps, bool& hot) {
+    hot = false;
+    if (e->y_flags_pending) {
+        if (run_steps >= e->knobs.spec_wait) {
+            HIP_TRY(hipEventSynchronize(e->y_flags_ev));
+        } else {
+            const hipError_t q = hipEventQuery(e->y_flags_ev);
+            if (q == hipErrorNotReady) return 0;
+            HIP_TRY(q);
+        }
+        e->y_flags_pending = false;
+    }
+    const int* const yf = e->y_flags_host;
+    hot = yf[P.head.y_binary - e->y_binary] != 0 && yf[2] != 0;
+    return 0;
+}
+
+int ws2_select_mode(const KParams& P, bool hot, bool accumulating, bool mix) {
+    if (!hot) return WS2_SPEC_GENERIC;
+    const bool map = P.xopt == MCPC_XOPT_ADAM;
+    if (map && accumulating) return WS2_SPEC_GENERIC;
+    if (accumulating && !P.spill_sys) return WS2_SPEC_GENERIC;
+    const int spec = map ? WS2_SPEC_MAP : !accumulating ? WS2_SPEC_HOT : WS2_SPEC_HOT_SPILL;
+    return kWs2Specs[spec].fn[mix ? 1 : 0] ? spec : WS2_SPEC_GENERIC;
+}
+
 #ifdef MCPC_STAMPS
 int report_stamps(mcpc_engine* e, bool use_u, int t, int n, hipStream_t stream) {
     static const char* names_ws2[16] = {"G top", "G wait deps", "G HEADB gemm", "G gemm", "G prefetch next", "G store+publish",
@@ -949,7 +1007,18 @@
     rr_ok = false;
 #endif
     unsigned launched = 0;
-    auto run_round_cycle = [&](const KParams& base, int t0, int q) -> int {
+    unsigned specs_rr = 0, specs_plain = 0;
+    bool hot = false;
+    if (!use_u && ws2_spec_candidate(e, P))
+        if (const int rc = target_flags_on_host(e, P, r->n_steps, hot)) return rc;
+    auto launch_ws2 = [&](KParams& K, bool mix, int nblocks, bool accumulating) -> int {
+        const int spec = ws2_select_mode(K, hot, accumulating, mix);
+        (mix ? specs_rr : specs_plain) |= 1u << spec;
+        void* args[] = {&K};
+        HIP_TRY(hipLaunchKernel(kWs2Specs[spec].fn[mix ? 1 : 0], dim3(nblocks), dim3(kWs2Threads), args, sp.lds_bytes, stream));
+        return 0;
+    };
+    auto run_round_cycle = [&](const KParams& base, int t0, int q, bool accumulating) -> int {
         launched |= 2u;
         KParams Q = base;
         set_window(e, r, Q, t0, q);
@@ -958,7 +1027,7 @@
             Q.wg_list = e->rr_tab + e->rr_off[i]; Q.wg_rel = Q.wg_list + e->rr_count[i];
             { const int rc = prof_begin(); if (rc) return rc; }
             if (use_u) hipLaunchKernelGGL((mcpc_steps_u_kernel<true>), dim3(e->rr_count[i]), dim3(kUThreads), sp.lds_bytes, stream, Q);
-            else hipLaunchKernelGGL((mcpc_steps_ws2_kernel<1, true>), dim3(e->rr_count[i]), dim3(kWs2Threads), sp.lds_bytes, stream, Q);
+            else if (const int rc = launch_ws2(Q, true, e->rr_count[i], accumulating)) return rc;
             { const int rc = prof_end((double)q * e->rr_count[i] / e->nwg_live); if (rc) return rc; }
         }
         HIP_TRY(hipGetLastError());
@@ -982,7 +1051,7 @@
         } else if (rr_ok) {
             while (n >= e->rr_m) {
                 const int q = std::min(std::max(1, e->knobs.rr_qmax), n / e->rr_m);
-                const int rc = run_round_cycle(P, t, q);
+                const int rc = run_round_cycle(P, t, q, false);
                 if (rc) return rc;
                 t += q * e->rr_m; n -= q * e->rr_m;
             }
@@ -1005,14 +1074,14 @@
             P.spillmax = nullptr;
         }
         if (rr_q >= 1) {
-            const int rc = run_round_cycle(P, t, rr_q);
+            const int rc = run_round_cycle(P, t, rr_q, in_acc);
             if (rc) return rc;
         } else {
             { const int rc = prof_begin(); if (rc) return rc; }
             launched |= 1u;
             if (e->lw) { const int rc = launch_lw_steps(e, r, P, t, n, stream); if (rc) return rc; }
             else if (use_u) hipLaunchKernelGGL((mcpc_steps_u_kernel<false>), dim3(e->nwg_live), dim3(kUThreads), sp.lds_bytes, stream, P);
-            else if (e->ws == 2) hipLaunchKernelGGL((mcpc_steps_ws2_kernel<1>), dim3(e->nwg_live), dim3(kWs2Threads), sp.lds_bytes, stream, P);
+            else if (e->ws == 2) { const int rc = launch_ws2(P, false, e->nwg_live, in_acc); if (rc) return rc; }
             else hipLaunchKernelGGL((mcpc_steps_kernel<1, 4>), dim3(e->nwg), dim3(256), sp.lds_bytes, stream, P);
             { const int rc = prof_end((double)n); if (rc) return rc; }
         }
@@ -1037,11 +1106,18 @@
         t += n;
     }
     {
+        auto spec_tag = [](unsigned specs) -> std::string {
+            if (!(specs & ~(1u << WS2_SPEC_GENERIC))) return "";
+            std::string tag;
+            for (int i = 0; i < WS2_SPEC_COUNT; ++i)
+                if (specs & (1u << i)) tag += (tag.empty() ? "" : ", ") + std::string(kWs2Specs[i].tag);
+            return " [mcpc_steps_ws2_spec_kernel: " + tag + "]";
+        };
         std::string name;
-        if (launched & 2u) name = use_u ? e->u_rr_name : e->rr_name;
+        if (launched & 2u) name = (use_u ? e->u_rr_name : e->rr_name) + spec_tag(specs_rr);
         if (launched & 1u) {
             if (!name.empty()) name += " + ";
-            name += plain_kernel_name(*e, use_u);
+            name += plain_kernel_name(*e, use_u) + spec_tag(specs_plain);
         }
         e->last_step = name;
     }
diff --git a/montecarlopredictivecoding_amd/csrc/mcpc_plan.h b/montecarlopredictivecoding_amd/csrc/mcpc_plan.h
--- a/montecarlopredictivecoding_amd/csrc/mcpc_plan.h
+++ b/montecarlopredictivecoding_amd/csrc/mcpc_plan.h
@@ -67,6 +67,8 @@
     int rr_qmax = 100;
     int heb171 = 0;
     int heb_fp32 = 0;
+    int spec = 1;
+    int spec_wait = 0;
     int u_row = 5000;
     int u_gemm0 = 1200;
     int u_kb = 200;
@@ -92,7 +94,7 @@
         struct { const char* name; int* dst; } table[] = {
             {"ws", &k.ws}, {"wide", &k.wide}, {"no_overlap", &k.no_overlap},
             {"slot_cap", &k.slot_cap}, {"spill_gb", &k.spill_gb}, {"cu_slack", &k.cu_slack}, {"ring_parts", &k.ring_parts}, {"flush_tail", &k.flush_tail}, {"flush_streams", &k.flush_streams}, {"dw_ksplit", &k.dw_ksplit},
-            {"ws_prio", &k.ws_prio}, {"stagger", &k.stagger}, {"no_lean", &k.no_lean}, {"no_ybits", &k.no_ybits}, {"overlay16", &k.overlay16}, {"heb_fp32", &k.heb_fp32}, {"heb171", &k.heb171}, {"rr", &k.rr}, {"rr_qmax", &k.rr_qmax}, {"no_xl", &k.no_xl},
+            {"ws_prio", &k.ws_prio}, {"stagger", &k.stagger}, {"no_lean", &k.no_lean}, {"no_ybits", &k.no_ybits}, {"overlay16", &k.overlay16}, {"heb_fp32", &k.heb_fp32}, {"heb171", &k.heb171}, {"rr", &k.rr}, {"rr_qmax", &k.rr_qmax}, {"no_xl", &k.no_xl}, {"spec", &k.spec}, {"spec_wait", &k.spec_wait},
             {"u_row", &k.u_row}, {"u_gemm0", &k.u_gemm0}, {"u_kb", &k.u_kb}, {"u_kbt", &k.u_kbt}, {"u_eh", &k.u_eh}, {"u_eb", &k.u_eb}, {"u_ef", &k.u_ef}};
         bool found = false;
         for (auto& t : table)
diff --git a/montecarlopredictivecoding_amd/csrc/mcpc_steps_ws2.h b/montecarlopredictivecoding_amd/csrc/mcpc_steps_ws2.h
--- a/montecarlopredictivecoding_amd/csrc/mcpc_steps_ws2.h
+++ b/montecarlopredictivecoding_amd/csrc/mcpc_steps_ws2.h
@@ -212,14 +212,29 @@
     return lsum;
 }
 
-template <int CTT, bool MIX = false>
-__global__ __launch_bounds__(kWs2Threads, MCPC_WS2_WAVES_PER_EU) void mcpc_steps_ws2_kernel(const KParams P) {
-    extern __shared__ __attribute__((aligned(16))) float lds[];
-#define WS2_BLOCK blockIdx.x
-#define WS2_NBLOCKS gridDim.x
-#include "mcpc_steps_ws2_body.inc"
-#undef WS2_BLOCK
-#undef WS2_NBLOCKS
-}
-
-}
+#define WS2_KERNEL_TEMPLATE template <int CTT, bool MIX = false>
+#define WS2_KERNEL_NAME mcpc_steps_ws2_kernel
+#define WS2_MODE Ws2Generic
+#include "mcpc_steps_ws2_kernel.inc"
+#define WS2_KERNEL_TEMPLATE template <class MODE, int CTT, bool MIX = false>
+#define WS2_KERNEL_NAME mcpc_steps_ws2_spec_kernel
+#define WS2_MODE MODE
+#include "mcpc_steps_ws2_kernel.inc"
+
+template <int SPILL> using Ws2HotMode = Ws2Mode<WS2_UPD_SGD_PHILOX, 1, 1, SPILL, WS2_HEAD_BERNOULLI_BITS, MCPC_ACT_RELU>;
+using Ws2MapMode = Ws2Mode<WS2_UPD_ADAM, 1, 1, WS2_SPILL_OFF, WS2_HEAD_BERNOULLI_BITS, MCPC_ACT_RELU>;
+enum Ws2Spec { WS2_SPEC_GENERIC = 0, WS2_SPEC_HOT, WS2_SPEC_HOT_SPILL, WS2_SPEC_MAP, WS2_SPEC_COUNT };
+struct Ws2SpecEntry { const void* fn[2]; const char* tag; };
+#ifndef MCPC_EXP_NOLEAN
+static const Ws2SpecEntry kWs2Specs[WS2_SPEC_COUNT] = {
+    {{(const void*)mcpc_steps_ws2_kernel<1, false>, (const void*)mcpc_steps_ws2_kernel<1, true>}, "generic"},
+    {{(const void*)mcpc_steps_ws2_spec_kernel<Ws2HotMode<WS2_SPILL_OFF>, 1, false>, (const void*)mcpc_steps_ws2_spec_kernel<Ws2HotMode<WS2_SPILL_OFF>, 1, true>}, "hot"},
+    {{(const void*)mcpc_steps_ws2_spec_kernel<Ws2HotMode<WS2_SPILL_SYS>, 1, false>, (const void*)mcpc_steps_ws2_spec_kernel<Ws2HotMode<WS2_SPILL_SYS>, 1, true>}, "hot+spill"},
+    {{(const void*)mcpc_steps_ws2_spec_kernel<Ws2MapMode, 1, false>, (const void*)mcpc_steps_ws2_spec_kernel<Ws2MapMode, 1, true>}, "map"},
+};
+#else
+static const Ws2SpecEntry kWs2Specs[WS2_SPEC_COUNT] = {
+    {{(const void*)mcpc_steps_ws2_kernel<1, false>, (const void*)mcpc_steps_ws2_kernel<1, true>}, "generic"}, {{nullptr, nullptr}, ""}, {{nullptr, nullptr}, ""}, {{nullptr, nullptr}, ""}};
+#endif
+
+}
diff --git a/montecarlopredictivecoding_amd/csrc/mcpc_steps_ws2_body.inc b/montecarlopredictivecoding_amd/csrc/mcpc_steps_ws2_body.inc
--- a/montecarlopredictivecoding_amd/csrc/mcpc_steps_ws2_body.inc
+++ b/montecarlopredictivecoding_amd/csrc/mcpc_steps_ws2_body.inc
@@ -1,3 +1,4 @@
+    using M = WS2_MODE;
     constexpr int NW = kWs2Pairs, NTW = ws2_nt<CTT>();
     const int tid = threadIdx.x;
     const int lane = tid & 63;
@@ -15,21 +16,22 @@
     for (int i = tid; i < P.lds_floats / 4; i += kWs2Threads) st4(lds + 4 * i, splat(0.f));
     __syncthreads();
     if (tid < 2 * kWs2Pairs) reinterpret_cast<int*>(sync)[tid] = 0;
-    const int upd_mode = (P.update_x && P.xopt == MCPC_XOPT_SGD)
+    const int upd_mode = M::UPD != kModeDyn ? (M::UPD == WS2_UPD_SGD_PHILOX ? 2 : (M::UPD == WS2_UPD_SGD ? 1 : 0))
+                         : (P.update_x && P.xopt == MCPC_XOPT_SGD)
                              ? (P.noise_mode == MCPC_NOISE_PHILOX ? 2 : (P.noise_mode == MCPC_NOISE_NONE ? 1 : 0)) : 0;
-    const bool lean_adam = P.update_x && P.xopt == MCPC_XOPT_ADAM && P.noise_mode == MCPC_NOISE_NONE;
-    const bool lean = (upd_mode != 0 || lean_adam) && chain0 < P.B && P.lean_ok;
-    const bool xl = CTT == 1 && lean && P.xl != 0;
+    const bool lean_adam = M::UPD != kModeDyn ? M::UPD == WS2_UPD_ADAM : P.update_x && P.xopt == MCPC_XOPT_ADAM && P.noise_mode == MCPC_NOISE_NONE;
+    const bool lean = M::UPD != kModeDyn || ((upd_mode != 0 || lean_adam) && chain0 < P.B && P.lean_ok);
+    const bool xl = M::XL != kModeDyn ? M::XL != 0 : CTT == 1 && lean && P.xl != 0;
 #ifdef MCPC_EXP_NOLEAN
     const bool rowexp = false;
 #else
-    const bool rowexp = CTT == 1 && lean;
+    const bool rowexp = M::ROWEXP != kModeDyn ? M::ROWEXP != 0 : CTT == 1 && lean;
 #endif
     float* const rx = rowexp ? lds + P.lds_rowexp : nullptr;
     for (int l = 0; l < L; ++l) {
         const KLayer& Ly = P.layer[l];
-        if (Ly.act == MCPC_ACT_RELU) ws2_fill_fx<MCPC_ACT_RELU>(Ly, lds, chain0, tid, 16 * CTT, xl, rx, rowexp_fx(l));
-        else if (Ly.act == MCPC_ACT_TANH) ws2_fill_fx<MCPC_ACT_TANH>(Ly, lds, chain0, tid, 16 * CTT, xl, rx, rowexp_fx(l));
+        if (M::act(Ly.act) == MCPC_ACT_RELU) ws2_fill_fx<MCPC_ACT_RELU>(Ly, lds, chain0, tid, 16 * CTT, xl, rx, rowexp_fx(l));
+        else if (M::act(Ly.act) == MCPC_ACT_TANH) ws2_fill_fx<MCPC_ACT_TANH>(Ly, lds, chain0, tid, 16 * CTT, xl, rx, rowexp_fx(l));
         else ws2_fill_fx<MCPC_ACT_IDENTITY>(Ly, lds, chain0, tid, 16 * CTT, xl, rx, rowexp_fx(l));
     }
     if (xl) ws2_fill_constants(P, lds, chain0, tid, 16 * CTT);
@@ -39,7 +41,7 @@
         if (P.ws_prio == 2) __builtin_amdgcn_s_setprio(2);
         int p = P.g_first;
         if (p < 0) return;
-        const bool y_bounded = P.has_head && *P.head.y_bounded != 0;
+        const bool y_bounded = M::HEAD != kModeDyn ? M::HEAD == WS2_HEAD_BERNOULLI_BITS : P.has_head && *P.head.y_bounded != 0;
         KPhase ph_next = load_phase(P.phases, p);
         int nt_next, aoff[NTW];
         frag_t pre0[NTW];
@@ -88,7 +90,7 @@
                     STAMP(1);
                     if (is_headb) {
                         if (nt > 0 MCPC_EXP_GEMM_GATE) {
-                            const int hb_exp = headb_fixed_exp(P.head.loss_kind, y_bounded);
+                            const int hb_exp = headb_fixed_exp(M::loss_kind(P.head), y_bounded);
                             const bool hb_word = hb_exp == kScaleAuto && rowexp && ph.b_row >= 0;
                             const int fixed_b = hb_word ? rowexp_read(rx, ph.b_row, c) : hb_exp;
                             GemmScale gs{load_wexp(P.wexp, ph.a_lin), GS_ACCUM, fixed_b, accb_run,
@@ -171,20 +173,20 @@
         const bool live = chain0 + 16 * ct + c < P.B;
         LL.livem[ct] = live ? ~0u : 0u;
     }
-    const bool ybin = lean && P.has_head && *P.head.y_binary != 0;
+    const bool ybin = M::HEAD != kModeDyn ? M::HEAD == WS2_HEAD_BERNOULLI_BITS : lean && P.has_head && *P.head.y_binary != 0;
     const bool e0_in_regs = lean && P.layer[0].ntiles <= NW;
     bool e0_dirty = false;
     f32x4 e0acc[CTT];
 #pragma unroll
     for (int ct = 0; ct < CTT; ++ct) e0acc[ct] = splat(0.f);
-    if (e0_in_regs && t_first + P.n_steps > P.acc_begin && t_first < P.acc_end) lean_load_e0<CTT>(P, k, LL, e0acc);
+    if (e0_in_regs && (M::SPILL != kModeDyn ? M::SPILL != WS2_SPILL_OFF : t_first + P.n_steps > P.acc_begin && t_first < P.acc_end)) lean_load_e0<CTT>(P, k, LL, e0acc);
     STAMP_DECL
     for (int s = 0; s < P.n_steps; ++s) {
         const int t = t_first + s;
         const int s_tab = MIX ? t - P.t0 : s;
         const int base = s * n_ent;
         const bool do_energy = (P.energy_mode == MCPC_ENERGY_ALL) || (P.energy_mode == MCPC_ENERGY_LAST && t == P.T - 1);
-        const int slot = (t >= P.acc_begin && t < P.acc_end) ? (t - P.spill_t0) : -1;
+        const int slot = M::SPILL == WS2_SPILL_OFF ? -1 : (M::SPILL != kModeDyn || (t >= P.acc_begin && t < P.acc_end)) ? (t - P.spill_t0) : -1;
         int rec_idx = -1;
         if (P.rec_count > 0 && t >= P.rec_begin) {
             const int kk = (t - P.rec_begin) / P.rec_stride;
@@ -228,7 +230,7 @@
             nt = nt < 0 ? 0 : (nt > NTW ? NTW : nt);
 #ifndef MCPC_EXP_NOLEAN
             if (lean) {
-                const int act = P.layer[ph.layer].act;
+                const int act = M::act(P.layer[ph.layer].act);
                 const int* const pg = &sync->prog_g[k];
                 const int need = base + p + 1;
 #ifdef MCPC_STAMPS_ENTRY
@@ -243,18 +245,18 @@
 #endif
                 if (ph.type == PH_FWD) {
                     float esum;
-                    if (ph.layer == 0 && slot >= 0) e0_dirty = true;
+                    if (ph.layer == 0 && M::spills(slot)) e0_dirty = true;
                     if constexpr (CTT == 1) {
                         if (xl) {
-                            if (act == MCPC_ACT_RELU) esum = lean_fwd<CTT, NW, NTW, MCPC_ACT_RELU, true>(P, ph, lds, nt, kk, LL, slot, rec_idx, pg, need, P.err, dead, e0acc, e0_in_regs, rx, (unsigned)(s + 1));
-                            else if (act == MCPC_ACT_TANH) esum = lean_fwd<CTT, NW, NTW, MCPC_ACT_TANH, true>(P, ph, lds, nt, kk, LL, slot, rec_idx, pg, need, P.err, dead, e0acc, e0_in_regs, rx, (unsigned)(s + 1));
-                            else esum = lean_fwd<CTT, NW, NTW, MCPC_ACT_IDENTITY, true>(P, ph, lds, nt, kk, LL, slot, rec_idx, pg, need, P.err, dead, e0acc, e0_in_regs, rx, (unsigned)(s + 1));
+                            if (act == MCPC_ACT_RELU) esum = lean_fwd<CTT, NW, NTW, MCPC_ACT_RELU, true, false, M>(P, ph, lds, nt, kk, LL, slot, rec_idx, pg, need, P.err, dead, e0acc, e0_in_regs, rx, (unsigned)(s + 1));
+                            else if (act == MCPC_ACT_TANH) esum = lean_fwd<CTT, NW, NTW, MCPC_ACT_TANH, true, false, M>(P, ph, lds, nt, kk, LL, slot, rec_idx, pg, need, P.err, dead, e0acc, e0_in_regs, rx, (unsigned)(s + 1));
+                            else esum = lean_fwd<CTT, NW, NTW, MCPC_ACT_IDENTITY, true, false, M>(P, ph, lds, nt, kk, LL, slot, rec_idx, pg, need, P.err, dead, e0acc, e0_in_regs, rx, (unsigned)(s + 1));
                         }
                     }
                     if (!xl) {
-                    if (act == MCPC_ACT_RELU) esum = lean_fwd<CTT, NW, NTW, MCPC_ACT_RELU>(P, ph, lds, nt, kk, LL, slot, rec_idx, pg, need, P.err, dead, e0acc, e0_in_regs, rx, (unsigned)(s + 1));
-                    else if (act == MCPC_ACT_TANH) esum = lean_fwd<CTT, NW, NTW, MCPC_ACT_TANH>(P, ph, lds, nt, kk, LL, slot, rec_idx, pg, need, P.err, dead, e0acc, e0_in_regs, rx, (unsigned)(s + 1));
-                    else esum = lean_fwd<CTT, NW, NTW, MCPC_ACT_IDENTITY>(P, ph, lds, nt, kk, LL, slot, rec_idx, pg, need, P.err, dead, e0acc, e0_in_regs, rx, (unsigned)(s + 1));
+                    if (act == MCPC_ACT_RELU) esum = lean_fwd<CTT, NW, NTW, MCPC_ACT_RELU, false, false, M>(P, ph, lds, nt, kk, LL, slot, rec_idx, pg, need, P.err, dead, e0acc, e0_in_regs, rx, (unsigned)(s + 1));
+                    else if (act == MCPC_ACT_TANH) esum = lean_fwd<CTT, NW, NTW, MCPC_ACT_TANH, false, false, M>(P, ph, lds, nt, kk, LL, slot, rec_idx, pg, need, P.err, dead, e0acc, e0_in_regs, rx, (unsigned)(s + 1));
+                    else esum = lean_fwd<CTT, NW, NTW, MCPC_ACT_IDENTITY, false, false, M>(P, ph, lds, nt, kk, LL, slot, rec_idx, pg, need, P.err, dead, e0acc, e0_in_regs, rx, (unsigned)(s + 1));
                     }
                     if (do_energy) { esum = wave_sum(esum); if (lane == ph.layer) en_acc += esum; }
                 } else if (ph.type == PH_HEADF) {
@@ -262,12 +264,12 @@
                     bool done = false;
                     if constexpr (CTT == 1) {
                         if (xl) {
-                            if (ybin) lsum = lean_headf<CTT, NW, NTW, true, true>(P, ph, lds, nt, kk, LL, slot, rec_idx, do_energy, pg, need, P.err, dead, true, rx);
-                            else lsum = lean_headf<CTT, NW, NTW, true, false>(P, ph, lds, nt, kk, LL, slot, rec_idx, do_energy, pg, need, P.err, dead, false, rx);
+                            if (ybin) lsum = lean_headf<CTT, NW, NTW, true, true, false, false, M>(P, ph, lds, nt, kk, LL, slot, rec_idx, do_energy, pg, need, P.err, dead, true, rx);
+                            else lsum = lean_headf<CTT, NW, NTW, true, false, false, false, M>(P, ph, lds, nt, kk, LL, slot, rec_idx, do_energy, pg, need, P.err, dead, false, rx);
                             done = true;
                         }
                     }
-                    if (!done) lsum = lean_headf<CTT, NW, NTW>(P, ph, lds, nt, kk, LL, slot, rec_idx, do_energy, pg, need, P.err, dead, ybin, rx);
+                    if (!done) lsum = lean_headf<CTT, NW, NTW, false, false, false, false, M>(P, ph, lds, nt, kk, LL, slot, rec_idx, do_energy, pg, need, P.err, dead, ybin, rx);
                     if (do_energy) { lsum = wave_sum(lsum); if (lane == kMaxLatent) en_acc += lsum; }
                 } else if (ph.type == PH_BWD) {
                     bool done = false;
@@ -275,33 +277,33 @@
                         if (xl) {
                             done = true;
                             if (lean_adam) {
-                                if (act == MCPC_ACT_RELU) lean_bwd<CTT, NW, NTW, MCPC_ACT_RELU, false, true, true>(P, ph, lds, nt, kk, LL, t, pg, need, P.err, dead, s_tab, rx, (unsigned)(s + 1));
-                                else if (act == MCPC_ACT_TANH) lean_bwd<CTT, NW, NTW, MCPC_ACT_TANH, false, true, true>(P, ph, lds, nt, kk, LL, t, pg, need, P.err, dead, s_tab, rx, (unsigned)(s + 1));
-                                else lean_bwd<CTT, NW, NTW, MCPC_ACT_IDENTITY, false, true, true>(P, ph, lds, nt, kk, LL, t, pg, need, P.err, dead, s_tab, rx, (unsigned)(s + 1));
+                                if (act == MCPC_ACT_RELU) lean_bwd<CTT, NW, NTW, MCPC_ACT_RELU, false, true, true, false, M>(P, ph, lds, nt, kk, LL, t, pg, need, P.err, dead, s_tab, rx, (unsigned)(s + 1));
+                                else if (act == MCPC_ACT_TANH) lean_bwd<CTT, NW, NTW, MCPC_ACT_TANH, false, true, true, false, M>(P, ph, lds, nt, kk, LL, t, pg, need, P.err, dead, s_tab, rx, (unsigned)(s + 1));
+                                else lean_bwd<CTT, NW, NTW, MCPC_ACT_IDENTITY, false, true, true, false, M>(P, ph, lds, nt, kk, LL, t, pg, need, P.err, dead, s_tab, rx, (unsigned)(s + 1));
                             } else if (upd_mode == 2) {
-                                if (act == MCPC_ACT_RELU) lean_bwd<CTT, NW, NTW, MCPC_ACT_RELU, true, false, true>(P, ph, lds, nt, kk, LL, t, pg, need, P.err, dead, 0, rx, (unsigned)(s + 1));
-                                else if (act == MCPC_ACT_TANH) lean_bwd<CTT, NW, NTW, MCPC_ACT_TANH, true, false, true>(P, ph, lds, nt, kk, LL, t, pg, need, P.err, dead, 0, rx, (unsigned)(s + 1));
-                                else lean_bwd<CTT, NW, NTW, MCPC_ACT_IDENTITY, true, false, true>(P, ph, lds, nt, kk, LL, t, pg, need, P.err, dead, 0, rx, (unsigned)(s + 1));
+                                if (act == MCPC_ACT_RELU) lean_bwd<CTT, NW, NTW, MCPC_ACT_RELU, true, false, true, false, M>(P, ph, lds, nt, kk, LL, t, pg, need, P.err, dead, 0, rx, (unsigned)(s + 1));
+                                else if (act == MCPC_ACT_TANH) lean_bwd<CTT, NW, NTW, MCPC_ACT_TANH, true, false, true, false, M>(P, ph, lds, nt, kk, LL, t, pg, need, P.err, dead, 0, rx, (unsigned)(s + 1));
+                                else lean_bwd<CTT, NW, NTW, MCPC_ACT_IDENTITY, true, false, true, false, M>(P, ph, lds, nt, kk, LL, t, pg, need, P.err, dead, 0, rx, (unsigned)(s + 1));
                             } else {
-                                if (act == MCPC_ACT_RELU) lean_bwd<CTT, NW, NTW, MCPC_ACT_RELU, false, false, true>(P, ph, lds, nt, kk, LL, t, pg, need, P.err, dead, 0, rx, (unsigned)(s + 1));
-                                else if (act == MCPC_ACT_TANH) lean_bwd<CTT, NW, NTW, MCPC_ACT_TANH, false, false, true>(P, ph, lds, nt, kk, LL, t, pg, need, P.err, dead, 0, rx, (unsigned)(s + 1));
-                                else lean_bwd<CTT, NW, NTW, MCPC_ACT_IDENTITY, false, false, true>(P, ph, lds, nt, kk, LL, t, pg, need, P.err, dead, 0, rx, (unsigned)(s + 1));
+                                if (act == MCPC_ACT_RELU) lean_bwd<CTT, NW, NTW, MCPC_ACT_RELU, false, false, true, false, M>(P, ph, lds, nt, kk, LL, t, pg, need, P.err, dead, 0, rx, (unsigned)(s + 1));
+                                else if (act == MCPC_ACT_TANH) lean_bwd<CTT, NW, NTW, MCPC_ACT_TANH, false, false, true, false, M>(P, ph, lds, nt, kk, LL, t, pg, need, P.err, dead, 0, rx, (unsigned)(s + 1));
+                                else lean_bwd<CTT, NW, NTW, MCPC_ACT_IDENTITY, false, false, true, false, M>(P, ph, lds, nt, kk, LL, t, pg, need, P.err, dead, 0, rx, (unsigned)(s + 1));
                             }
                         }
                     }
                     if (done) {
                     } else if (lean_adam) {
-                        if (act == MCPC_ACT_RELU) lean_bwd<CTT, NW, NTW, MCPC_ACT_RELU, false, true>(P, ph, lds, nt, kk, LL, t, pg, need, P.err, dead, s_tab, rx, (unsigned)(s + 1));
-                        else if (act == MCPC_ACT_TANH) lean_bwd<CTT, NW, NTW, MCPC_ACT_TANH, false, true>(P, ph, lds, nt, kk, LL, t, pg, need, P.err, dead, s_tab, rx, (unsigned)(s + 1));
-                        else lean_bwd<CTT, NW, NTW, MCPC_ACT_IDENTITY, false, true>(P, ph, lds, nt, kk, LL, t, pg, need, P.err, dead, s_tab, rx, (unsigned)(s + 1));
+                        if (act == MCPC_ACT_RELU) lean_bwd<CTT, NW, NTW, MCPC_ACT_RELU, false, true, false, false, M>(P, ph, lds, nt, kk, LL, t, pg, need, P.err, dead, s_tab, rx, (unsigned)(s + 1));
+                        else if (act == MCPC_ACT_TANH) lean_bwd<CTT, NW, NTW, MCPC_ACT_TANH, false, true, false, false, M>(P, ph, lds, nt, kk, LL, t, pg, need, P.err, dead, s_tab, rx, (unsigned)(s + 1));
+                        else lean_bwd<CTT, NW, NTW, MCPC_ACT_IDENTITY, false, true, false, false, M>(P, ph, lds, nt, kk, LL, t, pg, need, P.err, dead, s_tab, rx, (unsigned)(s + 1));
                     } else if (upd_mode == 2) {
-                        if (act == MCPC_ACT_RELU) lean_bwd<CTT, NW, NTW, MCPC_ACT_RELU, true>(P, ph, lds, nt, kk, LL, t, pg, need, P.err, dead, 0, rx, (unsigned)(s + 1));
-                        else if (act == MCPC_ACT_TANH) lean_bwd<CTT, NW, NTW, MCPC_ACT_TANH, true>(P, ph, lds, nt, kk, LL, t, pg, need, P.err, dead, 0, rx, (unsigned)(s + 1));
-                        else lean_bwd<CTT, NW, NTW, MCPC_ACT_IDENTITY, true>(P, ph, lds, nt, kk, LL, t, pg, need, P.err, dead, 0, rx, (unsigned)(s + 1));
+                        if (act == MCPC_ACT_RELU) lean_bwd<CTT, NW, NTW, MCPC_ACT_RELU, true, false, false, false, M>(P, ph, lds, nt, kk, LL, t, pg, need, P.err, dead, 0, rx, (unsigned)(s + 1));
+                        else if (act == MCPC_ACT_TANH) lean_bwd<CTT, NW, NTW, MCPC_ACT_TANH, true, false, false, false, M>(P, ph, lds, nt, kk, LL, t, pg, need, P.err, dead, 0, rx, (unsigned)(s + 1));
+                        else lean_bwd<CTT, NW, NTW, MCPC_ACT_IDENTITY, true, false, false, false, M>(P, ph, lds, nt, kk, LL, t, pg, need, P.err, dead, 0, rx, (unsigned)(s + 1));
                     } else {
-                        if (act == MCPC_ACT_RELU) lean_bwd<CTT, NW, NTW, MCPC_ACT_RELU, false>(P, ph, lds, nt, kk, LL, t, pg, need, P.err, dead, 0, rx, (unsigned)(s + 1));
-                        else if (act == MCPC_ACT_TANH) lean_bwd<CTT, NW, NTW, MCPC_ACT_TANH, false>(P, ph, lds, nt, kk, LL, t, pg, need, P.err, dead, 0, rx, (unsigned)(s + 1));
-                        else lean_bwd<CTT, NW, NTW, MCPC_ACT_IDENTITY, false>(P, ph, lds, nt, kk, LL, t, pg, need, P.err, dead, 0, rx, (unsigned)(s + 1));
+                        if (act == MCPC_ACT_RELU) lean_bwd<CTT, NW, NTW, MCPC_ACT_RELU, false, false, false, false, M>(P, ph, lds, nt, kk, LL, t, pg, need, P.err, dead, 0, rx, (unsigned)(s + 1));
+                        else if (act == MCPC_ACT_TANH) lean_bwd<CTT, NW, NTW, MCPC_ACT_TANH, false, false, false, false, M>(P, ph, lds, nt, kk, LL, t, pg, need, P.err, dead, 0, rx, (unsigned)(s + 1));
+                        else lean_bwd<CTT, NW, NTW, MCPC_ACT_IDENTITY, false, false, false, false, M>(P, ph, lds, nt, kk, LL, t, pg, need, P.err, dead, 0, rx, (unsigned)(s + 1));
                     }
                 }
                 if (lane == 0) ws_publish(&sync->prog_e[k], base + p + 1);
@@ -368,7 +370,7 @@
     if constexpr (CTT == 1) {
         if (xl) lean_store_x<CTT, NW>(P, lds, k, LL);
     }
-    spill_max_publish(P.spillmax, lds + P.lds_spillmax, lane);
+    if constexpr (M::SPILL != WS2_SPILL_OFF) spill_max_publish(P.spillmax, lds + P.lds_spillmax, lane);
     if (clk_wave && lane == 0) {
         atomicAdd(P.clk, __builtin_amdgcn_s_memtime() - clk_c0);
         atomicAdd(P.clk + 1, __builtin_amdgcn_s_memrealtime() - clk_w0);
diff --git a/montecarlopredictivecoding_amd/csrc/mcpc_steps_ws2_kernel.inc b/montecarlopredictivecoding_amd/csrc/mcpc_steps_ws2_kernel.inc
--- /dev/null
+++ b/montecarlopredictivecoding_amd/csrc/mcpc_steps_ws2_kernel.inc
@@ -0,0 +1,12 @@
+WS2_KERNEL_TEMPLATE
+__global__ __launch_bounds__(kWs2Threads, MCPC_WS2_WAVES_PER_EU) void WS2_KERNEL_NAME(const KParams P) {
+    extern __shared__ __attribute__((aligned(16))) float lds[];
+#define WS2_BLOCK blockIdx.x
+#define WS2_NBLOCKS gridDim.x
+#include "mcpc_steps_ws2_body.inc"
+#undef WS2_BLOCK
+#undef WS2_NBLOCKS
+}
+#undef WS2_KERNEL_TEMPLATE
+#undef WS2_KERNEL_NAME
+#undef WS2_MODE
diff --git a/montecarlopredictivecoding_amd/csrc/mcpc_ws2_lean.h b/montecarlopredictivecoding_amd/csrc/mcpc_ws2_lean.h
--- a/montecarlopredictivecoding_amd/csrc/mcpc_ws2_lean.h
+++ b/montecarlopredictivecoding_amd/csrc/mcpc_ws2_lean.h
@@ -36,6 +36,26 @@
     else __builtin_amdgcn_raw_buffer_store_b128(__builtin_bit_cast(u32x4_t, v), rsrc, (int)boff, 0, 0);
 #endif
 }
+
+constexpr int kModeDyn = -1;
+enum { WS2_UPD_SGD = 1, WS2_UPD_SGD_PHILOX = 2, WS2_UPD_ADAM = 3 };
+enum { WS2_SPILL_OFF = 0, WS2_SPILL_SYS = 1 };
+enum { WS2_HEAD_NONE = 0, WS2_HEAD_BERNOULLI_BITS = 1 };
+template <int UPD_ = kModeDyn, int XL_ = kModeDyn, int ROWEXP_ = kModeDyn, int SPILL_ = kModeDyn, int HEAD_ = kModeDyn, int ACT_ = kModeDyn>
+struct Ws2Mode {
+    static constexpr int UPD = UPD_, XL = XL_, ROWEXP = ROWEXP_, SPILL = SPILL_, HEAD = HEAD_, ACT = ACT_;
+    static constexpr bool generic = UPD == kModeDyn && XL == kModeDyn && ROWEXP == kModeDyn && SPILL == kModeDyn && HEAD == kModeDyn && ACT == kModeDyn;
+    static_assert(XL == kModeDyn || UPD != kModeDyn, "XL is a property of the lean epilogues");
+    static_assert(ROWEXP == kModeDyn || UPD != kModeDyn, "row words are kept by the lean epilogues");
+    static __device__ __forceinline__ bool spills(int slot) { if constexpr (SPILL == kModeDyn) return slot >= 0; else return SPILL != WS2_SPILL_OFF; }
+    static __device__ __forceinline__ bool spill_sys(const KParams& P) { if constexpr (SPILL == kModeDyn) return P.spill_sys != 0; else return SPILL == WS2_SPILL_SYS; }
+    static __device__ __forceinline__ int loss_kind(const KHead& H) {
+        if constexpr (HEAD == kModeDyn) return H.loss_kind; else return HEAD == WS2_HEAD_BERNOULLI_BITS ? MCPC_LOSS_BERNOULLI : MCPC_LOSS_NONE;
+    }
+    static __device__ __forceinline__ int act(int a) { if constexpr (ACT == kModeDyn) return a; else return ACT; }
+    static __device__ __forceinline__ bool has_rx(const float* rx) { if constexpr (ROWEXP == kModeDyn) return rx != nullptr; else return ROWEXP != 0; }
+};
+using Ws2Generic = Ws2Mode<>;
 
 template <int CTT>
 struct LeanLane {
@@ -57,7 +77,7 @@
     return r;
 }
 
-template <int CTT, int NW, int NTW, int ACT, bool XL = false, bool REG = false>
+template <int CTT, int NW, int NTW, int ACT, bool XL = false, bool REG = false, class M = Ws2Generic>
 __device__ __forceinline__ float lean_fwd(const KParams& P, const KPhase& ph, float* lds, int nt, int kk, const LeanLane<CTT>& L,
                                           int slot, int rec_idx, const int* prog_g, int need, int* err, int& dead,
                                           f32x4 (&e0acc)[CTT], bool e0_in_regs, float* rx = nullptr, unsigned row_gen = 0u,
@@ -124,11 +144,11 @@
     }
     const float ecoef = Ly.ecoef;
     char* const e_lds = reinterpret_cast<char*>(lds + Ly.lds_e);
-    float* const spill_a = slot >= 0 ? Ly.spill_a + (size_t)slot * P.Bpad * Ly.npad : nullptr;
-    float* const spill_e = slot >= 0 ? (l > 0 ? Ly.spill_e + (size_t)slot * P.Bpad * Ly.npad : Ly.spill_e) : nullptr;
+    float* const spill_a = M::spills(slot) ? Ly.spill_a + (size_t)slot * P.Bpad * Ly.npad : nullptr;
+    float* const spill_e = M::spills(slot) ? (l > 0 ? Ly.spill_e + (size_t)slot * P.Bpad * Ly.npad : Ly.spill_e) : nullptr;
     float* const rec = (rec_idx >= 0 && Ly.rec != nullptr) ? Ly.rec + (size_t)rec_idx * P.B * Ly.n : nullptr;
     const uint32_t img_bytes = (uint32_t)P.Bpad * npad4;
-    const bool sys = P.spill_sys != 0;
+    const bool sys = M::spill_sys(P);
     float esum = 0.f;
     float amx = 0.f, emx = 0.f;
     float rmx = 0.f;
@@ -143,7 +163,7 @@
             const f32x4 d = x - (av[i][ct] + bv[i][ct]);
             const f32x4 e = d * ecoef;
             if (l > 0) { *reinterpret_cast<f32x4*>(e_lds + lrowb[ct] + tb) = e; rmx = absmax4(rmx, e); }
-            if (slot >= 0) {
+            if (M::spills(slot)) {
 #ifdef MCPC_EXP_SPILL_LINEAR
                 const uint32_t sb = mul24(L.chain[ct] - (uint32_t)L.c, npad4) + 1024u * (uint32_t)tile + 16u * (uint32_t)(L.c + 16 * L.q);
 #else
@@ -161,11 +181,11 @@
             esum += L.livem[ct] ? 0.5f * ecoef * (dd.x + dd.y + dd.z + dd.w) : 0.f;
         }
     }
-    if (slot >= 0) {
+    if (M::spills(slot)) {
         spill_track(lds + P.lds_spillmax, spill_id_a(l), amx, L.c + 16 * L.q);
         if (l > 0) spill_track(lds + P.lds_spillmax, spill_id_e(l), emx, L.c + 16 * L.q);
     }
-    if (CTT == 1 && rx != nullptr && ph.o_row >= 0) rowexp_track(rx, ph.o_row, L.c, rmx, row_gen);
+    if (CTT == 1 && M::has_rx(rx) && ph.o_row >= 0) rowexp_track(rx, ph.o_row, L.c, rmx, row_gen);
     return esum;
 }
 
@@ -202,7 +222,7 @@
     }
 }
 
-template <int CTT, int NW, int NTW, int ACT, bool NOISE, bool ADAM = false, bool XL = false, bool REG = false>
+template <int CTT, int NW, int NTW, int ACT, bool NOISE, bool ADAM = false, bool XL = false, bool REG = false, class M = Ws2Generic>
 __device__ __forceinline__ void lean_bwd(const KParams& P, const KPhase& ph, float* lds, int nt, int kk, const LeanLane<CTT>& L,
                                          int t, const int* prog_g, int need, int* err, int& dead, int s_tab = 0, float* rx = nullptr,
                                          unsigned row_gen = 0u, const f32x4 (*racc)[CTT] = nullptr) {
@@ -338,10 +358,10 @@
             rmx = absmax4(rmx, fxn);
         }
     }
-    if (CTT == 1 && rx != nullptr && ph.o_row >= 0) rowexp_track(rx, ph.o_row, L.c, rmx, row_gen);
-}
-
-template <int CTT, int NW, int NTW, bool XL = false, bool YB = false, bool REG = false, bool YWG = false>
+    if (CTT == 1 && M::has_rx(rx) && ph.o_row >= 0) rowexp_track(rx, ph.o_row, L.c, rmx, row_gen);
+}
+
+template <int CTT, int NW, int NTW, bool XL = false, bool YB = false, bool REG = false, bool YWG = false, class M = Ws2Generic>
 __device__ __forceinline__ float lean_headf(const KParams& P, const KPhase& ph, float* lds, int nt, int kk, const LeanLane<CTT>& L,
                                             int slot, int rec_idx, bool do_energy, const int* prog_g, int need, int* err, int& dead,
                                             bool ybin, float* rx = nullptr, const f32x4 (*racc)[CTT] = nullptr, unsigned row_gen = 0u,
@@ -350,7 +370,7 @@
     const int tstep = REG ? ph.rot : NW;
     const KHead& H = P.head;
     const bool planes = REG && planes_ok;
-    const int kind = H.loss_kind, n = H.n, mask_start = H.mask_start;
+    const int kind = M::loss_kind(H), n = H.n, mask_start = H.mask_start;
     const uint32_t npad4 = 4u * (uint32_t)H.npad;
     uint32_t rowb[CTT], orowb[CTT];
 #pragma unroll
@@ -417,7 +437,7 @@
         }
     }
     const float inv_var = H.inv_var;
-    float* const spill = slot >= 0 ? H.spill_e + (size_t)slot * P.Bpad * H.npad : nullptr;
+    float* const spill = M::spills(slot) ? H.spill_e + (size_t)slot * P.Bpad * H.npad : nullptr;
     float* const rec = (rec_idx >= 0 && H.rec_out != nullptr) ? H.rec_out + (size_t)rec_idx * P.B * H.n : nullptr;
     float lsum = 0.f;
     float omx = 0.f;
@@ -490,20 +510,20 @@
             }
             rmx = absmax4(rmx, e);
 #ifdef MCPC_EXP_SPILL_LINEAR
-            if (slot >= 0) spill_st4(spill, (uint32_t)P.Bpad * npad4, mul24(L.chain[ct] - (uint32_t)L.c, npad4) + 1024u * (uint32_t)tile + 16u * (uint32_t)(L.c + 16 * L.q), mask4(e, L.livem[ct]), P.spill_sys != 0);
-#else
-            if (slot >= 0) {
+            if (M::spills(slot)) spill_st4(spill, (uint32_t)P.Bpad * npad4, mul24(L.chain[ct] - (uint32_t)L.c, npad4) + 1024u * (uint32_t)tile + 16u * (uint32_t)(L.c + 16 * L.q), mask4(e, L.livem[ct]), M::spill_sys(P));
+#else
+            if (M::spills(slot)) {
                 spill_st4(spill, (uint32_t)P.Bpad * npad4,
                           H.spill_tm ? mul24(L.chain[ct] - (uint32_t)L.c, npad4) + 1024u * (uint32_t)tile + 16u * (uint32_t)(L.c + 16 * L.q) : rowb[ct] + tb,
-                          mask4(e, L.livem[ct]), P.spill_sys != 0);
+                          mask4(e, L.livem[ct]), M::spill_sys(P));
                 omx = absmax4(omx, mask4(e, L.livem[ct]));
             }
 #endif
             if (rec != nullptr && L.livem[ct]) st_unpadded(rec, (int)L.chain[ct], H.n, 16 * tile + 4 * L.q, o);
         }
     }
-    if (slot >= 0) spill_track(lds + P.lds_spillmax, kSpillIdEo, omx, L.c + 16 * L.q);
-    if (CTT == 1 && rx != nullptr && ph.o_row >= 0) rowexp_track(rx, ph.o_row, L.c, rmx, REG ? row_gen : (unsigned)need);
+    if (M::spills(slot)) spill_track(lds + P.lds_spillmax, kSpillIdEo, omx, L.c + 16 * L.q);
+    if (CTT == 1 && M::has_rx(rx) && ph.o_row >= 0) rowexp_track(rx, ph.o_row, L.c, rmx, REG ? row_gen : (unsigned)need);
     return lsum;
 }
 
```

Measured after the change: 18640, median of 6. 1.05x the previous value.
